# test-time-training/ttt-video-dit

Measured on AMD Instinct MI355X. Metric: DiT+TTT fwd/bwd video-tokens/sec, higher is better.
Workload: dtype bf16

## Files before the change

include/ttt_hip.h:

```cpp
#ifndef TTT_HIP_H
#define TTT_HIP_H

#include <stddef.h>
#include <stdint.h>

#ifdef __cplusplus
extern "C" {
#endif

#define TTT_HIP_ABI_VERSION 5

enum { TTT_DTYPE_BF16 = 0, TTT_DTYPE_F32 = 1 };
enum { TTT_IMPL_AUTO = 0, TTT_IMPL_GENERIC = 1, TTT_IMPL_MFMA = 2 };

typedef struct ttt_dims {
    int32_t B, NH, NC, CS, F, G;
    int32_t act_dtype;
    int32_t impl;
    float   eps;
} ttt_dims;

typedef struct ttt_mlp_fwd_args {
    const void*  XQ;
    const void*  XK;
    const void*  XV;
    const void*  last_eta;
    const float* ttt_norm_weight;
    const float* ttt_norm_bias;
    const float* W1_init;
    const float* b1_init;
    const float* W2_init;
    const float* b2_init;
    float* W1_checkpoints;
    float* b1_checkpoints;
    float* W2_checkpoints;
    float* b2_checkpoints;
    void*  XQW;
} ttt_mlp_fwd_args;

typedef struct ttt_mlp_bwd_args {
    const void*  XQ; const void* XK; const void* XV; const void* last_eta;
    const float* ttt_norm_weight; const float* ttt_norm_bias;
    const float* W1_checkpoints; const float* b1_checkpoints;
    const float* W2_checkpoints; const float* b2_checkpoints;
    const void*  XQW;
    float* W1_init_group; float* b1_init_group; float* W2_init_group; float* b2_init_group;
    void*  x_hat_ln_group;
    float* std_ln_group;
    void*  X2_group;
    void*  Z1_group;
    void*  Z1_bar_group;
    void*  X2_bar_group;
    void*  grad_l_wrt_Z2_group;
    void*  grad_l_wrt_Z1_group;
    void*  x_hat_fused_group;
    void*  grad_x_hat_fused_group;
    void*  grad_output_fused_group;
    float* std_fused_group;
    const float* grad_L_W1_last; const float* grad_L_b1_last;
    const float* grad_L_W2_last; const float* grad_L_b2_last;
    const void*  grad_L_XQW;
    float* grad_L_ttt_norm_weight;
    float* grad_L_ttt_norm_bias;
    float* grad_L_W1_init; float* grad_L_b1_init; float* grad_L_W2_init; float* grad_L_b2_init;
    void*  grad_L_last_eta;
    void*  grad_L_XQ; void* grad_L_XK; void* grad_L_XV;
} ttt_mlp_bwd_args;

typedef struct ttt_linear_fwd_args {
    const void*  XQ; const void* XK; const void* XV; const void* last_eta;
    const float* ttt_norm_weight; const float* ttt_norm_bias;
    const float* W1_init;
    const float* b1_init;
    float* W1_checkpoints;
    float* b1_checkpoints;
    void*  XQW;
} ttt_linear_fwd_args;

typedef struct ttt_linear_bwd_args {
    const void*  XQ; const void* XK; const void* XV; const void* last_eta;
    const float* ttt_norm_weight; const float* ttt_norm_bias;
    const float* W1_checkpoints; const float* b1_checkpoints;
    const float* grad_L_W1_last; const float* grad_L_b1_last;
    const void*  grad_L_XQW;
    float* W1_init_group;
    float* b1_init_group;
    float* grad_L_ttt_norm_weight; float* grad_L_ttt_norm_bias;
    float* grad_L_W1_init; float* grad_L_b1_init;
    void*  grad_L_last_eta;
    void*  grad_L_XQ; void* grad_L_XK; void* grad_L_XV;
} ttt_linear_bwd_args;

size_t ttt_hip_mlp_forward_workspace(const ttt_dims* d);
size_t ttt_hip_mlp_backward_workspace(const ttt_dims* d);
size_t ttt_hip_linear_forward_workspace(const ttt_dims* d);
size_t ttt_hip_linear_backward_workspace(const ttt_dims* d);

int ttt_hip_mlp_forward(const ttt_dims* d, const ttt_mlp_fwd_args* a, void* workspace, size_t workspace_bytes, void* stream);
int ttt_hip_mlp_backward(const ttt_dims* d, const ttt_mlp_bwd_args* a, void* workspace, size_t workspace_bytes, void* stream);
int ttt_hip_mlp_forward_chunk(const ttt_dims* d, const ttt_mlp_fwd_args* a, int step0, int nsteps, float* W1_final, float* b1_final,
                              float* W2_final, float* b2_final, void* workspace, size_t workspace_bytes, void* stream);
int ttt_hip_linear_forward(const ttt_dims* d, const ttt_linear_fwd_args* a, void* workspace, size_t workspace_bytes, void* stream);
int ttt_hip_linear_backward(const ttt_dims* d, const ttt_linear_bwd_args* a, void* workspace, size_t workspace_bytes, void* stream);

int ttt_hip_pre_forward(int B, int L, int NH, int F, const void* XQ_raw, const void* XK_raw, const void* XV_raw,
                        const float* rope , const int32_t* src, const int32_t* pos,
                        const float* ln_w, const float* ln_b , void* XQ, void* XK, void* XV, void* stream);
int ttt_hip_pre_forward_range(int B, int L, int NH, int F, const void* XQ_raw, const void* XK_raw, const void* XV_raw,
                              const float* rope, const int32_t* src, const int32_t* pos, const float* ln_w, const float* ln_b,
                              void* XQ, void* XK, void* XV, int t0, int tn, void* stream);
int ttt_hip_pre_backward_partials(int NH);
int ttt_hip_pre_backward(int B, int L, int NH, int F, const void* XQ_raw, const void* XK_raw, const void* XV_raw,
                         const float* rope, const int32_t* src, const int32_t* pos, const float* ln_w,
                         const void* dXQ, const void* dXK, const void* dXV, void* dXQ_raw, void* dXK_raw, void* dXV_raw,
                         float* dlnw_part, float* dlnb_part , void* stream);
int ttt_hip_pre_backward_ld(int B, int L, int NH, int F, const void* XQ_raw, const void* XK_raw, const void* XV_raw,
                            const float* rope, const int32_t* src, const int32_t* pos, const float* ln_w,
                            const void* dXQ, const void* dXK, const void* dXV, void* dXQ_raw, void* dXK_raw, void* dXV_raw, int64_t ld_out,
                            float* dlnw_part, float* dlnb_part, void* stream);
int ttt_hip_post_partials(int B, int L);
int ttt_hip_post_forward(int B, int L, int NH, int F, float eps, const void* Y, const int32_t* src, const float* w, const float* b,
                         void* out, void* stream);
int ttt_hip_post_forward_range(int B, int L, int NH, int F, float eps, const void* Y, const int32_t* src, const float* w, const float* b,
                               void* out, int t0, int tn, void* stream);
int ttt_hip_post_backward(int B, int L, int NH, int F, float eps, const void* Y, const void* dOut, const int32_t* src, const float* w,
                          void* dY, float* dw_part, float* db_part , void* stream);
int ttt_hip_gate_forward(int B, int L, int D, int n_text, const void* res, const void* y, const float* tanh_text,
                         const float* tanh_video, void* out, void* stream);
int ttt_hip_gate_backward_partials(int D);
int ttt_hip_gate_backward(int B, int L, int D, int n_text, const void* g, const void* y, const float* tanh_text,
                          const float* tanh_video, void* dy, float* dtanh_part , void* stream);

typedef struct ttt_attn_tensor {
    void*   ptr;
    int64_t stride_b, stride_h, stride_s;
} ttt_attn_tensor;
typedef struct ttt_attn_fwd_args {
    ttt_attn_tensor Q, K, V, O;
    float*  LSE;
    int32_t B, NH, S, D;
    float   scale;
} ttt_attn_fwd_args;
typedef struct ttt_attn_bwd_args {
    ttt_attn_tensor Q, K, V, O, dO;
    ttt_attn_tensor dQ, dK, dV;
    const float* LSE;
    float*  Delta;
    int32_t B, NH, S, D;
    float   scale;
} ttt_attn_bwd_args;
int ttt_hip_attn_forward(const ttt_attn_fwd_args* a, void* stream);
int ttt_hip_attn_backward(const ttt_attn_bwd_args* a, void* stream);

int ttt_hip_attn_pre_forward(int B, int S, int NH, int n_text, float eps, const void* q_raw, const void* k_raw,
                             const float* wq, const float* bq, const float* wk, const float* bk,
                             const float* cos_table, const float* sin_table, void* q, void* k, void* stream);
int ttt_hip_attn_pre_partials(int B, int S, int NH);
int ttt_hip_attn_pre_backward(int B, int S, int NH, int n_text, float eps, const void* q_raw, const void* k_raw,
                              const ttt_attn_tensor* dq, const ttt_attn_tensor* dk, const float* wq, const float* wk,
                              const float* cos_table, const float* sin_table, void* dq_raw, void* dk_raw, float* part,
                              void* stream);
int ttt_hip_attn_pre_backward_ld(int B, int S, int NH, int n_text, float eps, const void* q_raw, const void* k_raw,
                                 const ttt_attn_tensor* dq, const ttt_attn_tensor* dk, const float* wq, const float* wk,
                                 const float* cos_table, const float* sin_table, void* dq_raw, void* dk_raw, int64_t ld_out, float* part,
                                 void* stream);

int ttt_hip_adaln_forward(int B, int Lt, int Lv, int D, float eps, const void* vid, const void* text, const float* w, const float* b,
                          const float* shift, const float* scale1p, void* out, void* stream);
int ttt_hip_adaln_backward_partials(void);
int ttt_hip_adaln_backward(int B, int Lt, int Lv, int D, float eps, const void* vid, const void* text, const void* dout,
                           const float* w, const float* b, const float* scale1p, void* dvid, void* dtext, float* part, void* stream);
int ttt_hip_resgate_forward(int B, int Lt, int Lv, int D, const void* vid, const void* text, const void* y, const float* gate,
                            void* ovid, void* otext, void* stream);
int ttt_hip_resgate_backward_partials(int D);
int ttt_hip_resgate_backward(int B, int Lt, int Lv, int D, const void* dvid, const void* dtext, const void* y, const float* gate,
                             void* dy, float* dgate_part, void* stream);

int ttt_hip_resolve_impl(const ttt_dims* d, int is_mlp, int is_backward);

void        ttt_hip_debug_timing(void* device_buffer);
void        ttt_hip_debug_groups_per_chunk(int groups);
int         ttt_hip_debug_option(const char* name, int value);
unsigned    ttt_hip_debug_sweep_error(void);
void        ttt_hip_sweep_error_clear(void);
int         ttt_hip_debug_occupy_cus(int workgroups, int lds_bytes, int microseconds, void* stream);
void        ttt_hip_debug_dump(float* device_buffer);
int         ttt_hip_stream_create_masked(const unsigned* cu_mask, int mask_words, void** stream);
int         ttt_hip_stream_destroy(void* stream);
int         ttt_hip_debug_placement_probe(unsigned* device_out, int workgroups, int lds_bytes, int microseconds, void* stream);

int         ttt_hip_abi_version(void);
const char* ttt_hip_last_error(void);

#ifdef __cplusplus
}
#endif
#endif
```

ttt-video-dit_amd/csrc/attn.h:

```cpp
#pragma once
#include <hip/hip_runtime.h>
#include <stdint.h>
#include "attn_types.h"

namespace ttt {
namespace attn {

struct PreParams {
    const __bf16 *q_raw, *k_raw;
    const float *wq, *bq, *wk, *bk;
    const float *cos, *sin;
    __bf16 *q, *k;
    int B, S, NH, n_text;
    float eps;
};
struct PreBwdParams {
    const __bf16 *q_raw, *k_raw, *dq, *dk;
    long dq_sb, dq_sh, dq_ss, dk_sb, dk_sh, dk_ss;
    const float *wq, *wk, *cos, *sin;
    __bf16 *dq_raw, *dk_raw;
    long ld_out;
    float* part;
    int B, S, NH, n_text;
    float eps;
};
int  pre_blocks(long rows);
void launch_pre_forward(const PreParams& a, hipStream_t s);
void launch_pre_backward(const PreBwdParams& a, hipStream_t s);

void launch_forward(const FwdParams& p, hipStream_t s);
void launch_backward(const BwdParams& p, hipStream_t s);

void launch_dq_v2(const BwdParams& p, hipStream_t s);
void launch_dkdv_v2(const BwdParams& p, hipStream_t s);
void set_debug_attn_variant(int v);

}
}
```

ttt-video-dit_amd/csrc/attn_body.h:

```cpp
#pragma once
#include <math.h>

#include "attn_types.h"
#include "ttt_wave_types.h"

#ifndef TTT_BODY_FN
#if defined(__HIP_DEVICE_COMPILE__) || defined(__HIPCC__)
#define TTT_BODY_FN __device__ __forceinline__
#else
#define TTT_BODY_FN inline
#endif
#endif

namespace ttt {
namespace attnb {
using namespace ttt::wv;
using attn::BwdParams;
using attn::FwdParams;

constexpr int QB = 256, KB = 64;
constexpr int AS = 72;
constexpr int VS = 96;
constexpr int KT_ELEMS = 64 * AS, VT_ELEMS = 64 * VS;
constexpr int FWD_BUF_ELEMS = KT_ELEMS + VT_ELEMS, LDS_FWD = 2 * FWD_BUF_ELEMS * 2;
constexpr int DQ_BUF_ELEMS = 2 * KT_ELEMS, LDS_DQ = 2 * DQ_BUF_ELEMS * 2;
constexpr float LOG2E = 1.4426950408889634f;

#if defined(__HIP_DEVICE_COMPILE__)
#define TTT_PIN_IN_BRANCH(x) asm volatile("" : "+v"(x))
#else
#define TTT_PIN_IN_BRANCH(x) ((void)0)
#endif

TTT_BODY_FN int row_of(int r, int h) { return (r & 3) + 8 * (r >> 2) + 4 * h; }
TTT_BODY_FN f32x16 zero16() {
    f32x16 z;
#pragma unroll
    for (int i = 0; i < 16; ++i) z[i] = 0.f;
    return z;
}
TTT_BODY_FN bf16x8 pack(const f32x16& t, int s) {
    bf16x8 r;
#pragma unroll
    for (int e = 0; e < 8; ++e) r[e] = (__bf16)t[8 * s + e];
    return r;
}
TTT_BODY_FN bf16x8 zero_frag() {
    bf16x8 r;
#pragma unroll
    for (int e = 0; e < 8; ++e) r[e] = (__bf16)0.0f;
    return r;
}
template <class BK>
TTT_BODY_FN bf16x8 row_frag(BK& bk, typename BK::tile_t img, int stride, int row0, int col0, int l) {
    return bk.template ld<bf16x8>(img + ((row0 + (l & 31)) * stride + col0 + 8 * (l >> 5)));
}
template <class BK>
TTT_BODY_FN bf16x8 tr_frag(BK& bk, typename BK::tile_t img, int stride, int r0, int r1, int col0, int l) {
    const int i = l & 15, g1 = (l >> 4) & 1;
    const int off = (i >> 2) * stride + col0 + 16 * g1 + 4 * (i & 3);
    const bf16x4 lo = bk.tr(img + (r0 * stride + off));
    const bf16x4 hi = bk.tr(img + (r1 * stride + off));
    return __builtin_shufflevector(lo, hi, 0, 1, 2, 3, 4, 5, 6, 7);
}
template <class BK>
TTT_BODY_FN bf16x8 tr_frag_pi(BK& bk, typename BK::tile_t img, int stride, int row0, int s, int col0, int l) {
    const int h = l >> 5;
    return tr_frag(bk, img, stride, row0 + 16 * s + 4 * h, row0 + 16 * s + 8 + 4 * h, col0, l);
}

TTT_BODY_FN int swz_g(int r) { return (((r >> 1) & 1) << 2) | ((r >> 2) & 3); }
template <bool SWZ>
TTT_BODY_FN int tile_off(int r, int col) {
    return SWZ ? r * 64 + ((((col >> 3) ^ swz_g(r)) << 3) | (col & 7)) : r * AS + col;
}
template <bool SWZ, class BK>
TTT_BODY_FN bf16x8 row_frag_s(BK& bk, typename BK::tile_t img, int row0, int col0, int l) {
    return bk.template ld<bf16x8>(img + tile_off<SWZ>(row0 + (l & 31), col0 + 8 * (l >> 5)));
}
template <bool SWZ, class BK>
TTT_BODY_FN bf16x8 tr_frag_pi_s(BK& bk, typename BK::tile_t img, int row0, int s, int col0, int l) {
    const int h = l >> 5, i = l & 15, g1 = (l >> 4) & 1;
    const int r0 = row0 + 16 * s + 4 * h + (i >> 2), col = col0 + 16 * g1 + 4 * (i & 3);
    const bf16x4 lo = bk.tr(img + tile_off<SWZ>(r0, col));
    const bf16x4 hi = bk.tr(img + tile_off<SWZ>(r0 + 8, col));
    return __builtin_shufflevector(lo, hi, 0, 1, 2, 3, 4, 5, 6, 7);
}

struct KVStage {
    u32x4 k, v;
};
TTT_BODY_FN u32x4 zero_u4() {
    u32x4 z = {0u, 0u, 0u, 0u};
    return z;
}
TTT_BODY_FN void kv_issue(KVStage& st, const __bf16* Kp, const __bf16* Vp, long k_ss, long v_ss, int kv0, int S, int tid) {
    const int row = tid >> 3, col = (tid & 7) * 8;
    const int key = kv0 + row;
    if (key < S) {
        st.k = *reinterpret_cast<const u32x4*>(Kp + (long)key * k_ss + col);
        st.v = *reinterpret_cast<const u32x4*>(Vp + (long)key * v_ss + col);
    } else {
        st.k = zero_u4();
        st.v = zero_u4();
    }
}
template <class BK>
TTT_BODY_FN void kv_park(BK& bk, const KVStage& st, typename BK::tile_t k_img, typename BK::tile_t v_img, int v_stride, int tid) {
    const int row = tid >> 3, col = (tid & 7) * 8;
    bk.st(k_img + (row * AS + col), st.k);
    bk.st(v_img + (row * v_stride + col), st.v);
}

template <bool SWZ, class BK>
TTT_BODY_FN void kv_park_s(BK& bk, const KVStage& st, typename BK::tile_t k_img, typename BK::tile_t v_img, int tid) {
    const int row = tid >> 3, col = (tid & 7) * 8;
    bk.st(k_img + tile_off<SWZ>(row, col), st.k);
    bk.st(v_img + tile_off<SWZ>(row, col), st.v);
}

TTT_BODY_FN void head_of_block(int b, int nblk, int nbh, int& bh, int& blk) {
    if ((nbh & 7) == 0) {
        const int xcd = b & 7, idx = b >> 3;
        bh = xcd + 8 * (idx / nblk);
        blk = idx % nblk;
    } else {
        bh = b / nblk;
        blk = b % nblk;
    }
}

template <class BK>
TTT_BODY_FN void forward(BK& bk, const FwdParams& p, int bh, int qb) {
    const int tid = bk.thread(), wv = bk.wave(), l = bk.lane(), h = l >> 5, c = l & 31;
    const int bb = bh / p.NH, hh = bh % p.NH;
    const __bf16* Qp = p.Q + (long)bb * p.q_sb + (long)hh * p.q_sh;
    const __bf16* Kp = p.K + (long)bb * p.k_sb + (long)hh * p.k_sh;
    const __bf16* Vp = p.V + (long)bb * p.v_sb + (long)hh * p.v_sh;
    __bf16* Op = p.O + (long)bb * p.o_sb + (long)hh * p.o_sh;

    const int qrow = qb * QB + 32 * wv + c;
    const bool qvalid = qrow < p.S;
    bf16x8 Qf[4];
#pragma unroll
    for (int kk = 0; kk < 4; ++kk)
        Qf[kk] = qvalid ? *reinterpret_cast<const bf16x8*>(Qp + (long)qrow * p.q_ss + 16 * kk + 8 * h) : zero_frag();

    f32x16 O[2] = {zero16(), zero16()};
    float m = -1e30f, lsum = 0.f;
    const float sc = p.scale * LOG2E;
    const int nt = (p.S + KB - 1) / KB;
    KVStage st;

    const typename BK::tile_t lds = bk.lds_base();
    kv_issue(st, Kp, Vp, p.k_ss, p.v_ss, 0, p.S, tid);
    kv_park(bk, st, lds, lds + KT_ELEMS, VS, tid);
    bk.barrier();
    for (int j = 0; j < nt; ++j) {
        const typename BK::tile_t Kt = lds + (j & 1) * FWD_BUF_ELEMS, Vt = Kt + KT_ELEMS;
        const bool more = j + 1 < nt;
        if (more) kv_issue(st, Kp, Vp, p.k_ss, p.v_ss, (j + 1) * KB, p.S, tid);
        f32x16 Sc[2];
#pragma unroll
        for (int kb = 0; kb < 2; ++kb) {
            f32x16 acc = zero16();
#pragma unroll
            for (int kk = 0; kk < 4; ++kk) acc = bk.mma3216(row_frag(bk, Kt, AS, 32 * kb, 16 * kk, l), Qf[kk], acc);
            Sc[kb] = acc;
        }
        if (!more && (p.S & (KB - 1))) {
            const int kv0 = j * KB;
#pragma unroll
            for (int kb = 0; kb < 2; ++kb)
#pragma unroll
                for (int r = 0; r < 16; ++r) {
                    float v = Sc[kb][r];
                    if (kv0 + 32 * kb + row_of(r, h) >= p.S) v = -1e30f;
                    TTT_PIN_IN_BRANCH(v);
                    Sc[kb][r] = v;
                }
        }
        float mt = Sc[0][0];
#pragma unroll
        for (int r = 1; r < 16; ++r) mt = fmaxf(mt, Sc[0][r]);
#pragma unroll
        for (int r = 0; r < 16; ++r) mt = fmaxf(mt, Sc[1][r]);
        mt = fmaxf(mt, bk.xor_read(mt, 32));
        if (bk.any(mt > m)) {
            const float mn = fmaxf(m, mt);
            const float alpha = bk.exp2((m - mn) * sc);
            m = mn;
            lsum *= alpha;
#pragma unroll
            for (int db = 0; db < 2; ++db)
#pragma unroll
                for (int r = 0; r < 16; ++r) O[db][r] *= alpha;
        }
        const float msc = m * sc;
        float ps = 0.f;
#pragma unroll
        for (int kb = 0; kb < 2; ++kb)
#pragma unroll
            for (int r = 0; r < 16; ++r) {
                const float e = bk.exp2(__builtin_fmaf(Sc[kb][r], sc, -msc));
                Sc[kb][r] = e;
                ps += e;
            }
        lsum += ps;
#pragma unroll
        for (int kb = 0; kb < 2; ++kb)
#pragma unroll
            for (int s = 0; s < 2; ++s) {
                const bf16x8 pf = pack(Sc[kb], s);
                O[0] = bk.mma3216(tr_frag_pi(bk, Vt, VS, 32 * kb, s, 0, l), pf, O[0]);
                O[1] = bk.mma3216(tr_frag_pi(bk, Vt, VS, 32 * kb, s, 32, l), pf, O[1]);
            }
        if (more) {
            const typename BK::tile_t Kn = lds + ((j + 1) & 1) * FWD_BUF_ELEMS;
            kv_park(bk, st, Kn, Kn + KT_ELEMS, VS, tid);
        }
        bk.barrier();
    }

    const float ltot = lsum + bk.xor_read(lsum, 32);
    const float inv = 1.0f / ltot;
    if (qvalid) {
        __bf16* orow = Op + (long)qrow * p.o_ss;
#pragma unroll
        for (int db = 0; db < 2; ++db)
#pragma unroll
            for (int g = 0; g < 4; ++g) {
                bf16x4 v;
#pragma unroll
                for (int e = 0; e < 4; ++e) v[e] = (__bf16)(O[db][4 * g + e] * inv);
                *reinterpret_cast<bf16x4*>(orow + 32 * db + 8 * g + 4 * h) = v;
            }
        if (h == 0 && p.LSE) p.LSE[(long)bh * p.S + qrow] = m * p.scale + bk.log(ltot);
    }
}


template <class BK>
TTT_BODY_FN void dq(BK& bk, const BwdParams& p, int bh, int qb) {
    const int tid = bk.thread(), wv = bk.wave(), l = bk.lane(), h = l >> 5, c = l & 31;
    const int bb = bh / p.NH, hh = bh % p.NH;
    const __bf16* Qp = p.Q + (long)bb * p.q_sb + (long)hh * p.q_sh;
    const __bf16* Kp = p.K + (long)bb * p.k_sb + (long)hh * p.k_sh;
    const __bf16* Vp = p.V + (long)bb * p.v_sb + (long)hh * p.v_sh;
    const __bf16* dOp = p.dO + (long)bb * p.do_sb + (long)hh * p.do_sh;

    const int qrow = qb * QB + 32 * wv + c;
    const bool qvalid = qrow < p.S;
    bf16x8 Qf[4], Df[4];
#pragma unroll
    for (int kk = 0; kk < 4; ++kk) {
        Qf[kk] = qvalid ? *reinterpret_cast<const bf16x8*>(Qp + (long)qrow * p.q_ss + 16 * kk + 8 * h) : zero_frag();
        Df[kk] = qvalid ? *reinterpret_cast<const bf16x8*>(dOp + (long)qrow * p.do_ss + 16 * kk + 8 * h) : zero_frag();
    }
    const float lse2 = qvalid ? p.LSE[(long)bh * p.S + qrow] * LOG2E : 1e30f;
// ... 5 lines not shown

    const typename BK::tile_t lds = bk.lds_base();
    kv_issue(st, Kp, Vp, p.k_ss, p.v_ss, 0, p.S, tid);
    kv_park(bk, st, lds, lds + KT_ELEMS, AS, tid);
    bk.barrier();
    for (int j = 0; j < nt; ++j) {
        const typename BK::tile_t Kt = lds + (j & 1) * DQ_BUF_ELEMS, Vt = Kt + KT_ELEMS;
        const bool more = j + 1 < nt;
        if (more) kv_issue(st, Kp, Vp, p.k_ss, p.v_ss, (j + 1) * KB, p.S, tid);
        const bool ragged = !more && (p.S & (KB - 1));
#pragma unroll
        for (int kb = 0; kb < 2; ++kb) {
            f32x16 Sc = zero16(), dP = zero16();
#pragma unroll
            for (int kk = 0; kk < 4; ++kk) {
                Sc = bk.mma3216(row_frag(bk, Kt, AS, 32 * kb, 16 * kk, l), Qf[kk], Sc);
                dP = bk.mma3216(row_frag(bk, Vt, AS, 32 * kb, 16 * kk, l), Df[kk], dP);
            }
            if (ragged) {
#pragma unroll
                for (int r = 0; r < 16; ++r) {
                    float v = Sc[r];
                    if (j * KB + 32 * kb + row_of(r, h) >= p.S) v = -1e30f;
                    TTT_PIN_IN_BRANCH(v);
                    Sc[r] = v;
                }
            }
#pragma unroll
            for (int r = 0; r < 16; ++r) {
                const float pr = bk.exp2(__builtin_fmaf(Sc[r], sc, -lse2));
                dP[r] = pr * (dP[r] - delta);
            }
#pragma unroll
            for (int s = 0; s < 2; ++s) {
                const bf16x8 df = pack(dP, s);
                dQ[0] = bk.mma3216(tr_frag_pi(bk, Kt, AS, 32 * kb, s, 0, l), df, dQ[0]);
                dQ[1] = bk.mma3216(tr_frag_pi(bk, Kt, AS, 32 * kb, s, 32, l), df, dQ[1]);
            }
        }
        if (more) {
            const typename BK::tile_t Kn = lds + ((j + 1) & 1) * DQ_BUF_ELEMS;
            kv_park(bk, st, Kn, Kn + KT_ELEMS, AS, tid);
        }
        bk.barrier();
    }

    if (qvalid) {
        __bf16* row = p.dQ + (long)bb * p.dq_sb + (long)hh * p.dq_sh + (long)qrow * p.dq_ss;
#pragma unroll
        for (int db = 0; db < 2; ++db)
#pragma unroll
            for (int g = 0; g < 4; ++g) {
                bf16x4 v;
#pragma unroll
                for (int e = 0; e < 4; ++e) v[e] = (__bf16)(dQ[db][4 * g + e] * p.scale);
                *reinterpret_cast<bf16x4*>(row + 32 * db + 8 * g + 4 * h) = v;
            }
    }
}

template <int NSUB, bool SWZ = false, class BK>
TTT_BODY_FN void dq_staged(BK& bk, const BwdParams& p, int bh, int qb) {
    const int tid = bk.thread(), wv = bk.wave(), l = bk.lane(), h = l >> 5, c = l & 31;
    const int bb = bh / p.NH, hh = bh % p.NH;
    const __bf16* Qp = p.Q + (long)bb * p.q_sb + (long)hh * p.q_sh;
    const __bf16* Kp = p.K + (long)bb * p.k_sb + (long)hh * p.k_sh;
    const __bf16* Vp = p.V + (long)bb * p.v_sb + (long)hh * p.v_sh;
    const __bf16* dOp = p.dO + (long)bb * p.do_sb + (long)hh * p.do_sh;

    const int qrow = qb * QB + 32 * wv + c;
    const bool qvalid = qrow < p.S;
    bf16x8 Qf[4], Df[4];
#pragma unroll
    for (int kk = 0; kk < 4; ++kk) {
        Qf[kk] = qvalid ? *reinterpret_cast<const bf16x8*>(Qp + (long)qrow * p.q_ss + 16 * kk + 8 * h) : zero_frag();
        Df[kk] = qvalid ? *reinterpret_cast<const bf16x8*>(dOp + (long)qrow * p.do_ss + 16 * kk + 8 * h) : zero_frag();
    }
    const float lse2 = qvalid ? p.LSE[(long)bh * p.S + qrow] * LOG2E : 1e30f;
    const float delta = qvalid ? p.Delta[(long)bh * p.S + qrow] : 0.f;
    const float sc = p.scale * LOG2E;
    f32x16 dQ[2] = {zero16(), zero16()};
    const int nt = (p.S + KB - 1) / KB;
    const int ns = (nt + NSUB - 1) / NSUB;
    constexpr int STAGE_ELEMS = NSUB * DQ_BUF_ELEMS;
    KVStage st;

    const typename BK::tile_t lds = bk.lds_base();
#pragma unroll
    for (int u = 0; u < NSUB; ++u) {
        kv_issue(st, Kp, Vp, p.k_ss, p.v_ss, u * KB, p.S, tid);
        kv_park_s<SWZ>(bk, st, lds + u * DQ_BUF_ELEMS, lds + u * DQ_BUF_ELEMS + KT_ELEMS, tid);
    }
    bk.barrier();
    for (int j = 0; j < ns; ++j) {
        const typename BK::tile_t stage = lds + (j & 1) * STAGE_ELEMS;
        const typename BK::tile_t nxt = lds + ((j + 1) & 1) * STAGE_ELEMS;
        const bool more = j + 1 < ns;
#pragma unroll
        for (int u = 0; u < NSUB; ++u) {
            const int jt = j * NSUB + u;
            if (more) kv_issue(st, Kp, Vp, p.k_ss, p.v_ss, ((j + 1) * NSUB + u) * KB, p.S, tid);
            if (jt < nt) {
            const typename BK::tile_t Kt = stage + u * DQ_BUF_ELEMS, Vt = Kt + KT_ELEMS;
            const bool ragged = jt + 1 == nt && (p.S & (KB - 1));
#pragma unroll
            for (int kb = 0; kb < 2; ++kb) {
                f32x16 Sc = zero16(), dP = zero16();
#pragma unroll
                for (int kk = 0; kk < 4; ++kk) {
                    Sc = bk.mma3216(row_frag_s<SWZ>(bk, Kt, 32 * kb, 16 * kk, l), Qf[kk], Sc);
                    dP = bk.mma3216(row_frag_s<SWZ>(bk, Vt, 32 * kb, 16 * kk, l), Df[kk], dP);
                }
                if (ragged) {
#pragma unroll
                    for (int r = 0; r < 16; ++r) {
                        float v = Sc[r];
                        if (jt * KB + 32 * kb + row_of(r, h) >= p.S) v = -1e30f;
                        TTT_PIN_IN_BRANCH(v);
                        Sc[r] = v;
                    }
                }
#pragma unroll
                for (int r = 0; r < 16; ++r) {
                    const float pr = bk.exp2(__builtin_fmaf(Sc[r], sc, -lse2));
                    dP[r] = pr * (dP[r] - delta);
                }
#pragma unroll
                for (int s = 0; s < 2; ++s) {
                    const bf16x8 df = pack(dP, s);
                    dQ[0] = bk.mma3216(tr_frag_pi_s<SWZ>(bk, Kt, 32 * kb, s, 0, l), df, dQ[0]);
                    dQ[1] = bk.mma3216(tr_frag_pi_s<SWZ>(bk, Kt, 32 * kb, s, 32, l), df, dQ[1]);
                }
            }
            }
            if (more) kv_park_s<SWZ>(bk, st, nxt + u * DQ_BUF_ELEMS, nxt + u * DQ_BUF_ELEMS + KT_ELEMS, tid);
        }
        bk.barrier();
    }

    if (qvalid) {
        __bf16* row = p.dQ + (long)bb * p.dq_sb + (long)hh * p.dq_sh + (long)qrow * p.dq_ss;
#pragma unroll
        for (int db = 0; db < 2; ++db)
#pragma unroll
            for (int g = 0; g < 4; ++g) {
                bf16x4 v;
#pragma unroll
                for (int e = 0; e < 4; ++e) v[e] = (__bf16)(dQ[db][4 * g + e] * p.scale);
                *reinterpret_cast<bf16x4*>(row + 32 * db + 8 * g + 4 * h) = v;
            }
    }
}

template <int NSUB, int NQ, class BK>
TTT_BODY_FN void dq_wide(BK& bk, const BwdParams& p, int bh, int qb) {
    const int tid = bk.thread(), wv = bk.wave(), l = bk.lane(), h = l >> 5, c = l & 31;
    const int bb = bh / p.NH, hh = bh % p.NH;
    const __bf16* Qp = p.Q + (long)bb * p.q_sb + (long)hh * p.q_sh;
    const __bf16* Kp = p.K + (long)bb * p.k_sb + (long)hh * p.k_sh;
    const __bf16* Vp = p.V + (long)bb * p.v_sb + (long)hh * p.v_sh;
    const __bf16* dOp = p.dO + (long)bb * p.do_sb + (long)hh * p.do_sh;

    int qrow[NQ];
    bool qvalid[NQ];
    bf16x8 Qf[NQ][4], Df[NQ][4];
    float lse2[NQ], delta[NQ];
    f32x16 dQ[NQ][2];
#pragma unroll
    for (int qi = 0; qi < NQ; ++qi) {
        qrow[qi] = qb * (QB * NQ) + 32 * NQ * wv + 32 * qi + c;
        qvalid[qi] = qrow[qi] < p.S;
#pragma unroll
        for (int kk = 0; kk < 4; ++kk) {
            Qf[qi][kk] = qvalid[qi] ? *reinterpret_cast<const bf16x8*>(Qp + (long)qrow[qi] * p.q_ss + 16 * kk + 8 * h) : zero_frag();
            Df[qi][kk] = qvalid[qi] ? *reinterpret_cast<const bf16x8*>(dOp + (long)qrow[qi] * p.do_ss + 16 * kk + 8 * h) : zero_frag();
        }
        lse2[qi] = qvalid[qi] ? p.LSE[(long)bh * p.S + qrow[qi]] * LOG2E : 1e30f;
        delta[qi] = qvalid[qi] ? p.Delta[(long)bh * p.S + qrow[qi]] : 0.f;
        dQ[qi][0] = zero16();
        dQ[qi][1] = zero16();
    }
    const float sc = p.scale * LOG2E;
    const int nt = (p.S + KB - 1) / KB;
    const int ns = (nt + NSUB - 1) / NSUB;
    constexpr int STAGE_ELEMS = NSUB * DQ_BUF_ELEMS;
    KVStage st;

    const typename BK::tile_t lds = bk.lds_base();
#pragma unroll
    for (int u = 0; u < NSUB; ++u) {
        kv_issue(st, Kp, Vp, p.k_ss, p.v_ss, u * KB, p.S, tid);
        kv_park_s<false>(bk, st, lds + u * DQ_BUF_ELEMS, lds + u * DQ_BUF_ELEMS + KT_ELEMS, tid);
    }
    bk.barrier();
    for (int j = 0; j < ns; ++j) {
        const typename BK::tile_t stage = lds + (j & 1) * STAGE_ELEMS;
        const typename BK::tile_t nxt = lds + ((j + 1) & 1) * STAGE_ELEMS;
        const bool more = j + 1 < ns;
#pragma unroll
        for (int u = 0; u < NSUB; ++u) {
            const int jt = j * NSUB + u;
            if (more) kv_issue(st, Kp, Vp, p.k_ss, p.v_ss, ((j + 1) * NSUB + u) * KB, p.S, tid);
            if (jt < nt) {
            const typename BK::tile_t Kt = stage + u * DQ_BUF_ELEMS, Vt = Kt + KT_ELEMS;
            const bool ragged = jt + 1 == nt && (p.S & (KB - 1));
#pragma unroll
            for (int kb = 0; kb < 2; ++kb) {
                f32x16 Sc[NQ], dP[NQ];
#pragma unroll
                for (int qi = 0; qi < NQ; ++qi) { Sc[qi] = zero16(); dP[qi] = zero16(); }
#pragma unroll
                for (int kk = 0; kk < 4; ++kk) {
                    const bf16x8 kf = row_frag_s<false>(bk, Kt, 32 * kb, 16 * kk, l), vf = row_frag_s<false>(bk, Vt, 32 * kb, 16 * kk, l);
#pragma unroll
                    for (int qi = 0; qi < NQ; ++qi) {
                        Sc[qi] = bk.mma3216(kf, Qf[qi][kk], Sc[qi]);
                        dP[qi] = bk.mma3216(vf, Df[qi][kk], dP[qi]);
                    }
                }
                if (ragged) {
#pragma unroll
                    for (int qi = 0; qi < NQ; ++qi)
#pragma unroll
                        for (int r = 0; r < 16; ++r) {
                            float v = Sc[qi][r];
                            if (jt * KB + 32 * kb + row_of(r, h) >= p.S) v = -1e30f;
                            TTT_PIN_IN_BRANCH(v);
                            Sc[qi][r] = v;
                        }
                }
#pragma unroll
                for (int qi = 0; qi < NQ; ++qi)
#pragma unroll
                    for (int r = 0; r < 16; ++r) {
                        const float pr = bk.exp2(__builtin_fmaf(Sc[qi][r], sc, -lse2[qi]));
                        dP[qi][r] = pr * (dP[qi][r] - delta[qi]);
                    }
                if constexpr (BK::kPrio) bk.setprio(1);
#pragma unroll
                for (int s = 0; s < 2; ++s) {
                    const bf16x8 k0 = tr_frag_pi_s<false>(bk, Kt, 32 * kb, s, 0, l), k1 = tr_frag_pi_s<false>(bk, Kt, 32 * kb, s, 32, l);
#pragma unroll
                    for (int qi = 0; qi < NQ; ++qi) {
                        const bf16x8 df = pack(dP[qi], s);
                        dQ[qi][0] = bk.mma3216(k0, df, dQ[qi][0]);
                        dQ[qi][1] = bk.mma3216(k1, df, dQ[qi][1]);
                    }
                }
                if constexpr (BK::kPrio) bk.setprio(0);
            }
            }
            if (more) kv_park_s<false>(bk, st, nxt + u * DQ_BUF_ELEMS, nxt + u * DQ_BUF_ELEMS + KT_ELEMS, tid);
        }
        bk.barrier();
    }

#pragma unroll
    for (int qi = 0; qi < NQ; ++qi)
        if (qvalid[qi]) {
            __bf16* row = p.dQ + (long)bb * p.dq_sb + (long)hh * p.dq_sh + (long)qrow[qi] * p.dq_ss;
#pragma unroll
            for (int db = 0; db < 2; ++db)
#pragma unroll
                for (int g = 0; g < 4; ++g) {
                    bf16x4 v;
#pragma unroll
                    for (int e = 0; e < 4; ++e) v[e] = (__bf16)(dQ[qi][db][4 * g + e] * p.scale);
                    *reinterpret_cast<bf16x4*>(row + 32 * db + 8 * g + 4 * h) = v;
                }
        }
}

constexpr int DKV_BUF_ELEMS = 2 * KT_ELEMS + 2 * 64 * 2;
constexpr int LDS_DKV = 2 * DKV_BUF_ELEMS * 2;

struct QStage {
    u32x4 q, d;
    float lse, del;
};
template <bool ACC_INIT>
TTT_BODY_FN void qstage_issue(QStage& st, const BwdParams& p, const __bf16* Qp, const __bf16* dOp, const float* lse, const float* del,
                              float inv_scale, int q0, int tid) {
    if (tid < 512) {
        const int row = tid >> 3, col = (tid & 7) * 8;
        const int q = q0 + row;
        if (q < p.S) {
            st.q = *reinterpret_cast<const u32x4*>(Qp + (long)q * p.q_ss + col);
            st.d = *reinterpret_cast<const u32x4*>(dOp + (long)q * p.do_ss + col);
        } else {
            st.q = zero_u4();
            st.d = zero_u4();
        }
    }
    if (tid < 64) {
        const int qq = q0 + tid;
        if (ACC_INIT) {
            st.lse = qq < p.S ? -lse[qq] * inv_scale : -1e30f;
            st.del = qq < p.S ? -del[qq] : 0.f;
        } else {
            st.lse = qq < p.S ? lse[qq] * LOG2E : 1e30f;
            st.del = qq < p.S ? del[qq] : 0.f;
        }
    }
}
template <class BK>
TTT_BODY_FN void qstage_park(BK& bk, const QStage& st, typename BK::tile_t buf, int tid) {
    if (tid < 512) {
        const int row = tid >> 3, col = (tid & 7) * 8;
        bk.st(buf + (row * AS + col), st.q);
        bk.st(buf + (KT_ELEMS + row * AS + col), st.d);
    }
    if (tid < 64) {
        bk.st(buf + (2 * KT_ELEMS + 2 * tid), st.lse);
        bk.st(buf + (2 * KT_ELEMS + 2 * (64 + tid)), st.del);
    }
}
template <bool SWZ, class BK>
TTT_BODY_FN void qstage_park_s(BK& bk, const QStage& st, typename BK::tile_t buf, int tid) {
    if (tid < 512) {
        const int row = tid >> 3, col = (tid & 7) * 8;
        bk.st(buf + tile_off<SWZ>(row, col), st.q);
        bk.st(buf + (KT_ELEMS + tile_off<SWZ>(row, col)), st.d);
    }
    if (tid < 64) {
        bk.st(buf + (2 * KT_ELEMS + 2 * tid), st.lse);
        bk.st(buf + (2 * KT_ELEMS + 2 * (64 + tid)), st.del);
    }
}
template <class BK>
TTT_BODY_FN f32x16 rows_from_lds(BK& bk, typename BK::tile_t buf, int which, int base, int h) {
    f32x4 v[4];
#pragma unroll
    for (int q = 0; q < 4; ++q) v[q] = bk.template ld<f32x4>(buf + (2 * KT_ELEMS + 2 * (64 * which + base + 8 * q + 4 * h)));
    typedef float f32x8 __attribute__((ext_vector_type(8)));
    const f32x8 lo = __builtin_shufflevector(v[0], v[1], 0, 1, 2, 3, 4, 5, 6, 7);
    const f32x8 hi = __builtin_shufflevector(v[2], v[3], 0, 1, 2, 3, 4, 5, 6, 7);
    return __builtin_shufflevector(lo, hi, 0, 1, 2, 3, 4, 5, 6, 7, 8, 9, 10, 11, 12, 13, 14, 15);
}

template <int NW, bool ACC_INIT, class BK>
TTT_BODY_FN void dkdv(BK& bk, const BwdParams& p, int bh, int kvb) {
    const int tid = bk.thread(), wv = bk.wave(), l = bk.lane(), h = l >> 5, c = l & 31;
    const int bb = bh / p.NH, hh = bh % p.NH;
    const __bf16* Qp = p.Q + (long)bb * p.q_sb + (long)hh * p.q_sh;
    const __bf16* Kp = p.K + (long)bb * p.k_sb + (long)hh * p.k_sh;
    const __bf16* Vp = p.V + (long)bb * p.v_sb + (long)hh * p.v_sh;
    const __bf16* dOp = p.dO + (long)bb * p.do_sb + (long)hh * p.do_sh;
    const float* lse = p.LSE + (long)bh * p.S;
    const float* del = p.Delta + (long)bh * p.S;

    const int key0 = kvb * (32 * NW) + 32 * wv;
    const int krow = key0 + c;
    bf16x8 Kf[4], Vf[4];
#pragma unroll
    for (int kk = 0; kk < 4; ++kk) {
        Kf[kk] = krow < p.S ? *reinterpret_cast<const bf16x8*>(Kp + (long)krow * p.k_ss + 16 * kk + 8 * h) : zero_frag();
        Vf[kk] = krow < p.S ? *reinterpret_cast<const bf16x8*>(Vp + (long)krow * p.v_ss + 16 * kk + 8 * h) : zero_frag();
    }
    f32x16 dK[2] = {zero16(), zero16()}, dV[2] = {zero16(), zero16()};
    const float sc = p.scale * LOG2E, inv_scale = 1.0f / p.scale;

    const int nt = (p.S + 63) / 64;
    const typename BK::tile_t lds = bk.lds_base();
    QStage st;
    qstage_issue<ACC_INIT>(st, p, Qp, dOp, lse, del, inv_scale, 0, tid);
    qstage_park(bk, st, lds, tid);
    bk.barrier();

    for (int j = 0; j < nt; ++j) {
        const typename BK::tile_t buf = lds + (j & 1) * DKV_BUF_ELEMS;
        const typename BK::tile_t Qt = buf, Dt = buf + KT_ELEMS;
        const bool more = j + 1 < nt;
        if (more) qstage_issue<ACC_INIT>(st, p, Qp, dOp, lse, del, inv_scale, (j + 1) * 64, tid);
#pragma unroll
        for (int qb = 0; qb < 2; ++qb) {
            f32x16 Sc, dP;
            if (ACC_INIT) {
                Sc = rows_from_lds(bk, buf, 0, 32 * qb, h);
                dP = rows_from_lds(bk, buf, 1, 32 * qb, h);
            } else {
                Sc = zero16();
                dP = zero16();
            }
#pragma unroll
            for (int kk = 0; kk < 4; ++kk) {
                Sc = bk.mma3216(row_frag(bk, Qt, AS, 32 * qb, 16 * kk, l), Kf[kk], Sc);
                dP = bk.mma3216(row_frag(bk, Dt, AS, 32 * qb, 16 * kk, l), Vf[kk], dP);
            }
            if (ACC_INIT) {
#pragma unroll
                for (int r = 0; r < 16; ++r) {
                    float pr = bk.exp2(Sc[r] * sc);
                    TTT_PIN_IN_BRANCH(pr);
                    Sc[r] = pr;
                    float ds = pr * dP[r];
                    TTT_PIN_IN_BRANCH(ds);
                    dP[r] = ds;
                }
            } else {
                const f32x16 lseR = rows_from_lds(bk, buf, 0, 32 * qb, h);
                const f32x16 delR = rows_from_lds(bk, buf, 1, 32 * qb, h);
#pragma unroll
                for (int r = 0; r < 16; ++r) {
                    const float pr = bk.exp2(__builtin_fmaf(Sc[r], sc, -lseR[r]));
                    Sc[r] = pr;
                    dP[r] = pr * (dP[r] - delR[r]);
                }
            }
#pragma unroll
            for (int s = 0; s < 2; ++s) {
                const bf16x8 pf = pack(Sc, s), df = pack(dP, s);
#pragma unroll
                for (int db = 0; db < 2; ++db) {
                    dV[db] = bk.mma3216(pf, tr_frag_pi(bk, Dt, AS, 32 * qb, s, 32 * db, l), dV[db]);
                    dK[db] = bk.mma3216(df, tr_frag_pi(bk, Qt, AS, 32 * qb, s, 32 * db, l), dK[db]);
                }
            }
        }
        if (more) qstage_park(bk, st, lds + ((j + 1) & 1) * DKV_BUF_ELEMS, tid);
        bk.barrier();
    }

    __bf16* dKp = p.dK + (long)bb * p.dk_sb + (long)hh * p.dk_sh;
    __bf16* dVp = p.dV + (long)bb * p.dv_sb + (long)hh * p.dv_sh;
#pragma unroll
    for (int db = 0; db < 2; ++db)
#pragma unroll
        for (int r = 0; r < 16; ++r) {
            const int key = key0 + row_of(r, h);
            if (key < p.S) {
                dKp[(long)key * p.dk_ss + 32 * db + c] = (__bf16)(dK[db][r] * p.scale);
                dVp[(long)key * p.dv_ss + 32 * db + c] = (__bf16)dV[db][r];
            }
        }
}

template <int NW, bool ACC_INIT, int NSUB, bool SWZ = false, class BK>
TTT_BODY_FN void dkdv_staged(BK& bk, const BwdParams& p, int bh, int kvb) {
    const int tid = bk.thread(), wv = bk.wave(), l = bk.lane(), h = l >> 5, c = l & 31;
    const int bb = bh / p.NH, hh = bh % p.NH;
    const __bf16* Qp = p.Q + (long)bb * p.q_sb + (long)hh * p.q_sh;
    const __bf16* Kp = p.K + (long)bb * p.k_sb + (long)hh * p.k_sh;
    const __bf16* Vp = p.V + (long)bb * p.v_sb + (long)hh * p.v_sh;
    const __bf16* dOp = p.dO + (long)bb * p.do_sb + (long)hh * p.do_sh;
    const float* lse = p.LSE + (long)bh * p.S;
    const float* del = p.Delta + (long)bh * p.S;

    const int key0 = kvb * (32 * NW) + 32 * wv;
    const int krow = key0 + c;
    bf16x8 Kf[4], Vf[4];
#pragma unroll
    for (int kk = 0; kk < 4; ++kk) {
        Kf[kk] = krow < p.S ? *reinterpret_cast<const bf16x8*>(Kp + (long)krow * p.k_ss + 16 * kk + 8 * h) : zero_frag();
        Vf[kk] = krow < p.S ? *reinterpret_cast<const bf16x8*>(Vp + (long)krow * p.v_ss + 16 * kk + 8 * h) : zero_frag();
    }
    f32x16 dK[2] = {zero16(), zero16()}, dV[2] = {zero16(), zero16()};
    const float sc = p.scale * LOG2E, inv_scale = 1.0f / p.scale;

    const int nt = (p.S + 63) / 64;
    const int ns = (nt + NSUB - 1) / NSUB;
    constexpr int STAGE_ELEMS = NSUB * DKV_BUF_ELEMS;
    const typename BK::tile_t lds = bk.lds_base();
    QStage st;
#pragma unroll
    for (int u = 0; u < NSUB; ++u) {
        qstage_issue<ACC_INIT>(st, p, Qp, dOp, lse, del, inv_scale, u * 64, tid);
        qstage_park_s<SWZ>(bk, st, lds + u * DKV_BUF_ELEMS, tid);
    }
    bk.barrier();

    for (int j = 0; j < ns; ++j) {
        const typename BK::tile_t stage = lds + (j & 1) * STAGE_ELEMS;
        const typename BK::tile_t nxt = lds + ((j + 1) & 1) * STAGE_ELEMS;
        const bool more = j + 1 < ns;
#pragma unroll
        for (int u = 0; u < NSUB; ++u) {
        if (more) qstage_issue<ACC_INIT>(st, p, Qp, dOp, lse, del, inv_scale, ((j + 1) * NSUB + u) * 64, tid);
        if (j * NSUB + u < nt) {
        const typename BK::tile_t buf = stage + u * DKV_BUF_ELEMS;
        const typename BK::tile_t Qt = buf, Dt = buf + KT_ELEMS;
#pragma unroll
        for (int qb = 0; qb < 2; ++qb) {
            f32x16 Sc, dP;
            if (ACC_INIT) {
                Sc = rows_from_lds(bk, buf, 0, 32 * qb, h);
                dP = rows_from_lds(bk, buf, 1, 32 * qb, h);
            } else {
                Sc = zero16();
                dP = zero16();
            }
            if constexpr (BK::kPrio) bk.setprio(1);
#pragma unroll
            for (int kk = 0; kk < 4; ++kk) {
                Sc = bk.mma3216(row_frag_s<SWZ>(bk, Qt, 32 * qb, 16 * kk, l), Kf[kk], Sc);
                dP = bk.mma3216(row_frag_s<SWZ>(bk, Dt, 32 * qb, 16 * kk, l), Vf[kk], dP);
            }
            if constexpr (BK::kPrio) bk.setprio(0);
            if (ACC_INIT) {
#pragma unroll
                for (int r = 0; r < 16; ++r) {
                    float pr = bk.exp2(Sc[r] * sc);
                    TTT_PIN_IN_BRANCH(pr);
                    Sc[r] = pr;
                    float ds = pr * dP[r];
                    TTT_PIN_IN_BRANCH(ds);
                    dP[r] = ds;
                }
            } else {
                const f32x16 lseR = rows_from_lds(bk, buf, 0, 32 * qb, h);
                const f32x16 delR = rows_from_lds(bk, buf, 1, 32 * qb, h);
#pragma unroll
                for (int r = 0; r < 16; ++r) {
                    const float pr = bk.exp2(__builtin_fmaf(Sc[r], sc, -lseR[r]));
                    Sc[r] = pr;
                    dP[r] = pr * (dP[r] - delR[r]);
                }
            }
#pragma unroll
            for (int s = 0; s < 2; ++s) {
                const bf16x8 pf = pack(Sc, s), df = pack(dP, s);
#pragma unroll
                for (int db = 0; db < 2; ++db) {
                    dV[db] = bk.mma3216(pf, tr_frag_pi_s<SWZ>(bk, Dt, 32 * qb, s, 32 * db, l), dV[db]);
                    dK[db] = bk.mma3216(df, tr_frag_pi_s<SWZ>(bk, Qt, 32 * qb, s, 32 * db, l), dK[db]);
                }
            }

        }
        }
        if (more) qstage_park_s<SWZ>(bk, st, nxt + u * DKV_BUF_ELEMS, tid);
        }
        bk.barrier();
    }

    __bf16* dKp = p.dK + (long)bb * p.dk_sb + (long)hh * p.dk_sh;
    __bf16* dVp = p.dV + (long)bb * p.dv_sb + (long)hh * p.dv_sh;
#pragma unroll
    for (int db = 0; db < 2; ++db)
#pragma unroll
        for (int r = 0; r < 16; ++r) {
            const int key = key0 + row_of(r, h);
            if (key < p.S) {
                dKp[(long)key * p.dk_ss + 32 * db + c] = (__bf16)(dK[db][r] * p.scale);
                dVp[(long)key * p.dv_ss + 32 * db + c] = (__bf16)dV[db][r];
            }
        }
}

}
}
```

ttt-video-dit_amd/csrc/attn_bwd.hip:

```cpp
#include <hip/hip_runtime.h>
#include <stdlib.h>
#include "../../include/ttt_hip.h"
#include "attn.h"
#include "attn_dev.h"

namespace ttt {
namespace attn {

__global__ __launch_bounds__(256) void attn_delta_kernel(BwdParams p) {
    const long rows = (long)p.B * p.NH * p.S;
    for (long idx = (long)blockIdx.x * blockDim.x + threadIdx.x; idx < rows * 8; idx += (long)gridDim.x * blockDim.x) {
        const long row = idx >> 3;
        const int o = idx & 7;
        const int s = row % p.S;
        const int bh = row / p.S;
        const int b = bh / p.NH, h = bh % p.NH;
        const bf16x8 a = *reinterpret_cast<const bf16x8*>(p.dO + (long)b * p.do_sb + (long)h * p.do_sh + (long)s * p.do_ss + 8 * o);
        const bf16x8 c = *reinterpret_cast<const bf16x8*>(p.O + (long)b * p.o_sb + (long)h * p.o_sh + (long)s * p.o_ss + 8 * o);
        float acc = 0.f;
#pragma unroll
        for (int e = 0; e < 8; ++e) acc += (float)a[e] * (float)c[e];
        acc += __shfl_xor(acc, 1, 64);
        acc += __shfl_xor(acc, 2, 64);
        acc += __shfl_xor(acc, 4, 64);
        if (o == 0) p.Delta[row] = acc;
    }
}

void launch_backward(const BwdParams& p, hipStream_t s) {
    const long rows = (long)p.B * p.NH * p.S;
    const int dgrid = (int)((rows * 8 + 255) / 256 < 65536 ? (rows * 8 + 255) / 256 : 65536);
    hipLaunchKernelGGL(attn_delta_kernel, dim3(dgrid), dim3(256), 0, s, p);
    launch_dkdv_v2(p, s);
    launch_dq_v2(p, s);
}

}
}
```

ttt-video-dit_amd/csrc/attn_fwd.hip:

```cpp
#include <hip/hip_runtime.h>
#include "../../include/ttt_hip.h"
#include "attn.h"
#include "attn_dev.h"
#include "once_per_device.h"

namespace ttt {
namespace attn {

constexpr int QB = 256;
constexpr int KB = 64;
constexpr int NTF = 512;
constexpr int VS = 96;
constexpr int KT_ELEMS = ATILE, VT_ELEMS = 64 * VS, BUF_ELEMS = KT_ELEMS + VT_ELEMS;
constexpr int LDS_FWD = 2 * BUF_ELEMS * 2;

struct KVStage {
    uint4 k, v;
};

__device__ __forceinline__ void stage_issue(KVStage& st, const __bf16* Kp, const __bf16* Vp, long k_ss, long v_ss, int kv0, int S, int tid) {
    const int row = tid >> 3, col = (tid & 7) * 8;
    const int key = kv0 + row;
    if (key < S) {
        st.k = *reinterpret_cast<const uint4*>(Kp + (long)key * k_ss + col);
        st.v = *reinterpret_cast<const uint4*>(Vp + (long)key * v_ss + col);
    } else {
        st.k = make_uint4(0, 0, 0, 0);
        st.v = make_uint4(0, 0, 0, 0);
    }
}
__device__ __forceinline__ void stage_park(const KVStage& st, __bf16* Kt, __bf16* Vt, int tid) {
    const int row = tid >> 3, col = (tid & 7) * 8;
    *reinterpret_cast<uint4*>(Kt + row * AS + col) = st.k;
    *reinterpret_cast<uint4*>(Vt + row * VS + col) = st.v;
}

__global__ __launch_bounds__(NTF) void attn_fwd_kernel(FwdParams p) {
    extern __shared__ __attribute__((aligned(16))) char smem[];
    __bf16* lds = reinterpret_cast<__bf16*>(smem);

    const int tid = threadIdx.x;
    const int wv = __builtin_amdgcn_readfirstlane(tid >> 6);
    const int l = tid & 63, h = l >> 5, c = l & 31;

    const int nqb = (p.S + QB - 1) / QB;
    int bh, qb;
    {
        const int nbh = p.B * p.NH;
        const int b = blockIdx.x;
        if ((nbh & 7) == 0) {
            const int xcd = b & 7, idx = b >> 3;
            bh = xcd + 8 * (idx / nqb);
            qb = idx % nqb;
        } else {
            bh = b / nqb;
            qb = b % nqb;
        }
    }
    const int bb = bh / p.NH, hh = bh % p.NH;
    const __bf16* Qp = p.Q + (long)bb * p.q_sb + (long)hh * p.q_sh;
    const __bf16* Kp = p.K + (long)bb * p.k_sb + (long)hh * p.k_sh;
    const __bf16* Vp = p.V + (long)bb * p.v_sb + (long)hh * p.v_sh;
    __bf16* Op = p.O + (long)bb * p.o_sb + (long)hh * p.o_sh;

    const int q0 = qb * QB + 32 * wv;
    const int qrow = q0 + c;
    const bool qvalid = qrow < p.S;

    bf16x8 Qf[4];
#pragma unroll
    for (int kk = 0; kk < 4; ++kk) {
        if (qvalid) Qf[kk] = *reinterpret_cast<const bf16x8*>(Qp + (long)qrow * p.q_ss + 16 * kk + 8 * h);
        else {
#pragma unroll
            for (int e = 0; e < 8; ++e) Qf[kk][e] = (__bf16)0.0f;
        }
    }

    f32x16 O[2] = {zero16(), zero16()};
    float m = -1e30f, lsum = 0.f;
    const float sc = p.scale * 1.4426950408889634f;

    const int nt = (p.S + KB - 1) / KB;
    KVStage st;
    stage_issue(st, Kp, Vp, p.k_ss, p.v_ss, 0, p.S, tid);
    stage_park(st, lds, lds + KT_ELEMS, tid);
    __syncthreads();

    for (int j = 0; j < nt; ++j) {
        const __bf16* Kt = lds + (j & 1) * BUF_ELEMS;
        const __bf16* Vt = Kt + KT_ELEMS;
        const bool more = j + 1 < nt;
        if (more) stage_issue(st, Kp, Vp, p.k_ss, p.v_ss, (j + 1) * KB, p.S, tid);

        f32x16 Sc[2];
#pragma unroll
        for (int kb = 0; kb < 2; ++kb) {
            f32x16 acc = zero16();
#pragma unroll
            for (int kk = 0; kk < 4; ++kk) acc = mma(row_frag(Kt, AS, 32 * kb, 16 * kk, l), Qf[kk], acc);
            Sc[kb] = acc;
        }
        if (!more && (p.S & (KB - 1))) {
            const int kv0 = j * KB;
#pragma unroll
            for (int kb = 0; kb < 2; ++kb)
#pragma unroll
                for (int r = 0; r < 16; ++r)
                    if (kv0 + 32 * kb + row_of(r, h) >= p.S) Sc[kb][r] = -1e30f;
        }
        float mt = Sc[0][0];
#pragma unroll
        for (int r = 1; r < 16; ++r) mt = fmaxf(mt, Sc[0][r]);
#pragma unroll
        for (int r = 0; r < 16; ++r) mt = fmaxf(mt, Sc[1][r]);
        mt = fmaxf(mt, half_swap(mt));
        if (__builtin_amdgcn_ballot_w64(mt > m) != 0) {
            const float mn = fmaxf(m, mt);
            const float alpha = __builtin_amdgcn_exp2f((m - mn) * sc);
            m = mn;
            lsum *= alpha;
#pragma unroll
            for (int db = 0; db < 2; ++db)
#pragma unroll
                for (int r = 0; r < 16; ++r) O[db][r] *= alpha;
        }
        const float msc = m * sc;
        float ps = 0.f;
#pragma unroll
        for (int kb = 0; kb < 2; ++kb)
#pragma unroll
            for (int r = 0; r < 16; ++r) {
                const float e = __builtin_amdgcn_exp2f(__builtin_fmaf(Sc[kb][r], sc, -msc));
                Sc[kb][r] = e;
                ps += e;
            }
        lsum += ps;
#pragma unroll
        for (int kb = 0; kb < 2; ++kb)
#pragma unroll
            for (int s = 0; s < 2; ++s) {
                const bf16x8 pf = pack(Sc[kb], s);
                O[0] = mma(tr_frag_pi(Vt, VS, 32 * kb, s, 0, l), pf, O[0]);
                O[1] = mma(tr_frag_pi(Vt, VS, 32 * kb, s, 32, l), pf, O[1]);
            }
        if (more) {
            __bf16* Kn = lds + ((j + 1) & 1) * BUF_ELEMS;
            stage_park(st, Kn, Kn + KT_ELEMS, tid);
        }
        __syncthreads();
    }

    const float ltot = lsum + half_swap(lsum);
    const float inv = 1.0f / ltot;
    if (qvalid) {
        __bf16* orow = Op + (long)qrow * p.o_ss;
#pragma unroll
        for (int db = 0; db < 2; ++db)
#pragma unroll
            for (int g = 0; g < 4; ++g) {
                bf16x4 v;
#pragma unroll
                for (int e = 0; e < 4; ++e) v[e] = (__bf16)(O[db][4 * g + e] * inv);
                *reinterpret_cast<bf16x4*>(orow + 32 * db + 8 * g + 4 * h) = v;
            }
        if (h == 0 && p.LSE) p.LSE[(long)bh * p.S + qrow] = m * p.scale + __logf(ltot);
    }
}

void launch_forward(const FwdParams& p, hipStream_t s) {
    static ttt::OncePerDevice attr;
    attr.run([&] {
        (void)hipFuncSetAttribute((const void*)attn_fwd_kernel, hipFuncAttributeMaxDynamicSharedMemorySize, LDS_FWD);
    });
    const int nqb = (p.S + QB - 1) / QB;
    hipLaunchKernelGGL(attn_fwd_kernel, dim3(p.B * p.NH * nqb), dim3(NTF), LDS_FWD, s, p);
}

}
}
```

ttt-video-dit_amd/csrc/attn_pre.hip:

```cpp
#include <hip/hip_runtime.h>
#include <stdint.h>
#include "../../include/ttt_hip.h"
#include "attn.h"
#include "ttt_dpp.h"

namespace ttt {
namespace attn {

typedef __bf16 bf16x8 __attribute__((ext_vector_type(8)));
typedef float f32x4 __attribute__((ext_vector_type(4)));

__device__ __forceinline__ void ld8(const __bf16* p, float (&o)[8]) {
    const bf16x8 a = *reinterpret_cast<const bf16x8*>(p);
#pragma unroll
    for (int j = 0; j < 8; ++j) o[j] = (float)a[j];
}
__device__ __forceinline__ void st8(__bf16* p, const float (&v)[8]) {
    bf16x8 a;
#pragma unroll
    for (int j = 0; j < 8; ++j) a[j] = (__bf16)v[j];
    *reinterpret_cast<bf16x8*>(p) = a;
}
__device__ __forceinline__ void ldf8(const float* p, float (&o)[8]) {
    const f32x4 a = *reinterpret_cast<const f32x4*>(p), b = *reinterpret_cast<const f32x4*>(p + 4);
    o[0] = a[0]; o[1] = a[1]; o[2] = a[2]; o[3] = a[3]; o[4] = b[0]; o[5] = b[1]; o[6] = b[2]; o[7] = b[3];
}
__device__ __forceinline__ float rb(float x) { return (float)(__bf16)x; }

__device__ __forceinline__ void ln_rope(const float (&x)[8], const float (&w)[8], const float (&b)[8], float eps,
                                        const float* cosr, const float* sinr, float (&out)[8], float (&xh)[8], float& rstd) {
    float s = 0.f;
#pragma unroll
    for (int j = 0; j < 8; ++j) s += x[j];
    const float mean = sum8(s) * (1.0f / 64.0f);
    float vs = 0.f;
#pragma unroll
    for (int j = 0; j < 8; ++j) { xh[j] = x[j] - mean; vs += xh[j] * xh[j]; }
    rstd = 1.0f / sqrtf(sum8(vs) * (1.0f / 64.0f) + eps);
#pragma unroll
    for (int j = 0; j < 8; ++j) { xh[j] *= rstd; out[j] = rb(xh[j] * w[j] + b[j]); }
    if (cosr) {
        float c8[8], s8[8];
        ldf8(cosr, c8);
        ldf8(sinr, s8);
#pragma unroll
        for (int q = 0; q < 4; ++q) {
            const float a = out[2 * q], bb = out[2 * q + 1];
            out[2 * q] = rb(rb(a * rb(c8[2 * q])) + rb(-bb * rb(s8[2 * q])));
            out[2 * q + 1] = rb(rb(bb * rb(c8[2 * q + 1])) + rb(a * rb(s8[2 * q + 1])));
        }
    }
}

__global__ __launch_bounds__(256) void attn_pre_fwd_kernel(PreParams a) {
    const long total = (long)a.B * a.S * a.NH * 8;
    const int o = threadIdx.x & 7;
    float wq[8], bq[8], wk[8], bk[8];
    ldf8(a.wq + 8 * o, wq); ldf8(a.bq + 8 * o, bq); ldf8(a.wk + 8 * o, wk); ldf8(a.bk + 8 * o, bk);
    for (long idx = (long)blockIdx.x * blockDim.x + threadIdx.x; idx < total; idx += (long)gridDim.x * blockDim.x) {
        const int s = ((idx >> 3) / a.NH) % a.S;
        const int pos = s - a.n_text;
        const float* cosr = pos >= 0 ? a.cos + (long)pos * 64 + 8 * o : nullptr;
        const float* sinr = pos >= 0 ? a.sin + (long)pos * 64 + 8 * o : nullptr;
        float x[8], y[8], xh[8], rstd;
        ld8(a.q_raw + idx * 8, x);
        ln_rope(x, wq, bq, a.eps, cosr, sinr, y, xh, rstd);
        st8(a.q + idx * 8, y);
        ld8(a.k_raw + idx * 8, x);
        ln_rope(x, wk, bk, a.eps, cosr, sinr, y, xh, rstd);
        st8(a.k + idx * 8, y);
    }
}

__device__ __forceinline__ void ln_rope_bwd(const float (&x)[8], const float (&w)[8], float eps, const float* cosr, const float* sinr,
                                            float (&g)[8], float (&dx)[8], float (&dw)[8], float (&db)[8]) {
    if (cosr) {
        float c8[8], s8[8];
        ldf8(cosr, c8);
        ldf8(sinr, s8);
#pragma unroll
        for (int q = 0; q < 4; ++q) {
            const float ga = g[2 * q], gb = g[2 * q + 1];
            g[2 * q] = ga * rb(c8[2 * q]) + gb * rb(s8[2 * q + 1]);
            g[2 * q + 1] = gb * rb(c8[2 * q + 1]) - ga * rb(s8[2 * q]);
        }
    }
    float s = 0.f;
#pragma unroll
    for (int j = 0; j < 8; ++j) s += x[j];
    const float mean = sum8(s) * (1.0f / 64.0f);
    float vs = 0.f, xh[8];
#pragma unroll
    for (int j = 0; j < 8; ++j) { xh[j] = x[j] - mean; vs += xh[j] * xh[j]; }
    const float rstd = 1.0f / sqrtf(sum8(vs) * (1.0f / 64.0f) + eps);
    float s1 = 0.f, s2 = 0.f;
#pragma unroll
    for (int j = 0; j < 8; ++j) {
        xh[j] *= rstd;
        dw[j] += g[j] * xh[j];
        db[j] += g[j];
        g[j] *= w[j];
        s1 += g[j];
        s2 += g[j] * xh[j];
    }
    s1 = sum8(s1) * (1.0f / 64.0f);
    s2 = sum8(s2) * (1.0f / 64.0f);
#pragma unroll
    for (int j = 0; j < 8; ++j) dx[j] = (g[j] - s1 - xh[j] * s2) * rstd;
}

__global__ __launch_bounds__(256) void attn_pre_bwd_kernel(PreBwdParams a) {
    __shared__ float red[4][256][8 + 1];
    const long total = (long)a.B * a.S * a.NH * 8;
    const int o = threadIdx.x & 7;
    float wq[8], wk[8], dwq[8], dbq[8], dwk[8], dbk[8];
    ldf8(a.wq + 8 * o, wq); ldf8(a.wk + 8 * o, wk);
#pragma unroll
    for (int j = 0; j < 8; ++j) { dwq[j] = 0.f; dbq[j] = 0.f; dwk[j] = 0.f; dbk[j] = 0.f; }
    for (long idx = (long)blockIdx.x * blockDim.x + threadIdx.x; idx < total; idx += (long)gridDim.x * blockDim.x) {
        const long row = idx >> 3;
        const int hd = row % a.NH;
        const long tok = row / a.NH;
        const int s = tok % a.S;
        const int b = tok / a.S;
        const int pos = s - a.n_text;
        const float* cosr = pos >= 0 ? a.cos + (long)pos * 64 + 8 * o : nullptr;
        const float* sinr = pos >= 0 ? a.sin + (long)pos * 64 + 8 * o : nullptr;
        float x[8], g[8], dx[8];
        ld8(a.q_raw + idx * 8, x);
        ld8(a.dq + (long)b * a.dq_sb + (long)hd * a.dq_sh + (long)s * a.dq_ss + 8 * o, g);
        ln_rope_bwd(x, wq, a.eps, cosr, sinr, g, dx, dwq, dbq);
        const long raw_off = tok * a.ld_out + hd * 64 + 8 * o;
        st8(a.dq_raw + raw_off, dx);
        ld8(a.k_raw + idx * 8, x);
        ld8(a.dk + (long)b * a.dk_sb + (long)hd * a.dk_sh + (long)s * a.dk_ss + 8 * o, g);
        ln_rope_bwd(x, wk, a.eps, cosr, sinr, g, dx, dwk, dbk);
        st8(a.dk_raw + raw_off, dx);
    }
#pragma unroll
    for (int j = 0; j < 8; ++j) {
        red[0][threadIdx.x][j] = dwq[j]; red[1][threadIdx.x][j] = dbq[j];
        red[2][threadIdx.x][j] = dwk[j]; red[3][threadIdx.x][j] = dbk[j];
    }
    __syncthreads();
    {
        const int which = threadIdx.x >> 6, f = threadIdx.x & 63;
        const int oo = f >> 3, j = f & 7;
        float acc = 0.f;
        for (int t = oo; t < 256; t += 8) acc += red[which][t][j];
        a.part[((long)blockIdx.x * 4 + which) * 64 + f] = acc;
    }
}

int pre_blocks(long rows) {
    const long g = (rows * 8 + 255) / 256;
    return (int)(g < 2048 ? g : 2048);
}
void launch_pre_forward(const PreParams& a, hipStream_t s) {
    const long g = ((long)a.B * a.S * a.NH * 8 + 255) / 256;
    hipLaunchKernelGGL(attn_pre_fwd_kernel, dim3((int)(g < 8192 ? g : 8192)), dim3(256), 0, s, a);
}
void launch_pre_backward(const PreBwdParams& a, hipStream_t s) {
    hipLaunchKernelGGL(attn_pre_bwd_kernel, dim3(pre_blocks((long)a.B * a.S * a.NH)), dim3(256), 0, s, a);
}

}
}
```

ttt-video-dit_amd/csrc/attn_types.h:

```cpp
#pragma once
#include <stdint.h>

namespace ttt {
namespace attn {

struct FwdParams {
    const __bf16 *Q, *K, *V;
    __bf16* O;
    float* LSE;
    long q_sb, q_sh, q_ss, k_sb, k_sh, k_ss, v_sb, v_sh, v_ss, o_sb, o_sh, o_ss;
    int B, NH, S;
    float scale;
};
struct BwdParams {
    const __bf16 *Q, *K, *V, *O, *dO;
    const float* LSE;
    float* Delta;
    __bf16 *dQ, *dK, *dV;
    long q_sb, q_sh, q_ss, k_sb, k_sh, k_ss, v_sb, v_sh, v_ss, o_sb, o_sh, o_ss, do_sb, do_sh, do_ss;
    long dq_sb, dq_sh, dq_ss, dk_sb, dk_sh, dk_ss, dv_sb, dv_sh, dv_ss;
    int B, NH, S;
    float scale;
};

}
}
```

ttt-video-dit_amd/csrc/attn_v2.hip:

```cpp
#include <hip/hip_runtime.h>
#include <stdlib.h>
#include "../../include/ttt_hip.h"
#include "attn.h"
#include "attn_body.h"
#include "once_per_device.h"

namespace ttt {
namespace attn {

template <int VAR>
struct AttnDeviceWave {
    static constexpr bool kPrio = VAR != 0;
    __device__ __forceinline__ void setprio(int v) const { if (v) __builtin_amdgcn_s_setprio(1); else __builtin_amdgcn_s_setprio(0); }
    typedef __bf16* tile_t;
    typedef __attribute__((address_space(3))) wv::bf16x4 lds_b4;
    tile_t base;
    __device__ __forceinline__ int lane() const { return threadIdx.x & 63; }
    __device__ __forceinline__ int wave() const { return __builtin_amdgcn_readfirstlane(threadIdx.x >> 6); }
    __device__ __forceinline__ int thread() const { return threadIdx.x; }
    __device__ __forceinline__ void barrier() const { __syncthreads(); }
    __device__ __forceinline__ float exp2(float x) const { return __builtin_amdgcn_exp2f(x); }
    __device__ __forceinline__ float log(float x) const { return __logf(x); }
    __device__ __forceinline__ tile_t lds_base() const { return base; }
    template <class T> __device__ __forceinline__ T ld(const __bf16* p) const { return *reinterpret_cast<const T*>(p); }
    template <class T> __device__ __forceinline__ void st(__bf16* p, T v) const { *reinterpret_cast<T*>(p) = v; }
    __device__ __forceinline__ wv::bf16x4 tr(const __bf16* p) const { return __builtin_amdgcn_ds_read_tr16_b64_v4bf16((lds_b4*)p); }
    __device__ __forceinline__ wv::f32x16 mma3216(wv::bf16x8 a, wv::bf16x8 b, wv::f32x16 c) const {
        return __builtin_amdgcn_mfma_f32_32x32x16_bf16(a, b, c, 0, 0, 0);
    }
    __device__ __forceinline__ float xor_read(float v, int mask) const { return __shfl_xor(v, mask, 64); }
    __device__ __forceinline__ bool any(bool b) const { return __builtin_amdgcn_ballot_w64(b) != 0; }
};

template <int NW, bool ACC_INIT, int MINW, int NSUB, int VAR>
__global__ __launch_bounds__(64 * NW, MINW) void attn_dkdv2s_kernel(BwdParams p) {
    extern __shared__ __attribute__((aligned(16))) char smem[];
    int bh, kvb;
    attnb::head_of_block(blockIdx.x, (p.S + 32 * NW - 1) / (32 * NW), p.B * p.NH, bh, kvb);
    AttnDeviceWave<VAR> bk{reinterpret_cast<__bf16*>(smem)};
    attnb::dkdv_staged<NW, ACC_INIT, NSUB, false>(bk, p, bh, kvb);
}
template <int NSUB, int VAR>
__global__ __launch_bounds__(512, 2) void attn_dq_wide_kernel(BwdParams p) {
    extern __shared__ __attribute__((aligned(16))) char smem[];
    int bh, qb;
    attnb::head_of_block(blockIdx.x, (p.S + 2 * attnb::QB - 1) / (2 * attnb::QB), p.B * p.NH, bh, qb);
    AttnDeviceWave<VAR> bk{reinterpret_cast<__bf16*>(smem)};
    attnb::dq_wide<NSUB, 2>(bk, p, bh, qb);
}

static int g_attn_variant = 1;
void set_debug_attn_variant(int v) { g_attn_variant = v; }

template <int VAR>
static void launch_dq_var(const BwdParams& p, hipStream_t s) {
    constexpr int NSUB = 1;
    static ttt::OncePerDevice attr;
    attr.run([&] {
        (void)hipFuncSetAttribute((const void*)attn_dq_wide_kernel<NSUB, VAR>, hipFuncAttributeMaxDynamicSharedMemorySize, NSUB * attnb::LDS_DQ);
    });
    const int nb = (p.S + 2 * attnb::QB - 1) / (2 * attnb::QB);
    hipLaunchKernelGGL((attn_dq_wide_kernel<NSUB, VAR>), dim3(p.B * p.NH * nb), dim3(512), NSUB * attnb::LDS_DQ, s, p);
}
void launch_dq_v2(const BwdParams& p, hipStream_t s) {
    if (g_attn_variant) launch_dq_var<1>(p, s);
    else launch_dq_var<0>(p, s);
}

template <int VAR>
static void launch_dkdv_var(const BwdParams& p, hipStream_t s) {
    constexpr int NW = 12, NSUB = 2;
    static_assert(NSUB * attnb::LDS_DKV <= 160 * 1024, "LDS budget");
    static ttt::OncePerDevice attr;
    attr.run([&] {
        (void)hipFuncSetAttribute((const void*)attn_dkdv2s_kernel<NW, true, 3, NSUB, VAR>, hipFuncAttributeMaxDynamicSharedMemorySize, NSUB * attnb::LDS_DKV);
    });
    const int nb = (p.S + 32 * NW - 1) / (32 * NW);
    hipLaunchKernelGGL((attn_dkdv2s_kernel<NW, true, 3, NSUB, VAR>), dim3(p.B * p.NH * nb), dim3(64 * NW), NSUB * attnb::LDS_DKV, s, p);
}
void launch_dkdv_v2(const BwdParams& p, hipStream_t s) {
    if (g_attn_variant) launch_dkdv_var<1>(p, s);
    else launch_dkdv_var<0>(p, s);
}

}
}
```

ttt-video-dit_amd/csrc/capi.hip:

```cpp
#include <hip/hip_runtime.h>
#include <stdio.h>
#include <string.h>
#include "../../include/ttt_hip.h"
#include "ttt_generic.h"
#include "ttt_mfma.h"
#include "ttt_prepost.h"
#include "attn.h"
#include "ttt_mfma_int.h"

static thread_local char g_err[512] = "";

static int fail(const char* fmt, const char* what = "") {
    snprintf(g_err, sizeof(g_err), fmt, what);
    return -1;
}

static int check_dims(const ttt_dims* d) {
    if (!d) return fail("ttt_hip: null dims");
    if (d->B <= 0 || d->NH <= 0 || d->NC <= 0 || d->CS <= 0 || d->F <= 0 || d->G <= 0)
        return fail("ttt_hip: non-positive dimension");
    if (d->act_dtype != TTT_DTYPE_BF16 && d->act_dtype != TTT_DTYPE_F32) return fail("ttt_hip: bad act_dtype");
    if (d->impl < TTT_IMPL_AUTO || d->impl > TTT_IMPL_MFMA) return fail("ttt_hip: bad impl");
    if (!(d->eps >= 0.f)) return fail("ttt_hip: bad eps");
    return 0;
// ... 194 lines not shown
    if (wsb < ws_bytes(d, false, true) || (ws_bytes(d, false, true) && !ws)) return fail("ttt_hip: linear_backward: workspace too small");
    if (r == TTT_IMPL_MFMA) ttt::mfma::linear_backward(d, a, ws, (hipStream_t)stream);
    else ttt::generic::linear_backward(d, a, ws, (hipStream_t)stream);
    return post_launch("linear_backward");
}

static int check_pp(int B, int L, int NH, int F) {
    if (B <= 0 || L <= 0 || NH <= 0) return fail("ttt_hip: non-positive dimension");
    if (F != 64) return fail("ttt_hip: fused pre/post kernels need head_dim 64");
    if (NH * 8 > 512) return fail("ttt_hip: too many heads for the post kernels (NH * 64 <= 4096 features)");
    if ((long long)B * L >= (1ll << 31) / 4) return fail("ttt_hip: B * L too large for the pre / post kernels' 32-bit token arithmetic");
    return 0;
}

int ttt_hip_pre_forward(int B, int L, int NH, int F, const void* XQ_raw, const void* XK_raw, const void* XV_raw,
                        const float* rope, const int32_t* src, const int32_t* pos, const float* ln_w, const float* ln_b,
                        void* XQ, void* XK, void* XV, void* stream) {
    return ttt_hip_pre_forward_range(B, L, NH, F, XQ_raw, XK_raw, XV_raw, rope, src, pos, ln_w, ln_b, XQ, XK, XV, 0, L, stream);
}
int ttt_hip_pre_forward_range(int B, int L, int NH, int F, const void* XQ_raw, const void* XK_raw, const void* XV_raw,
                              const float* rope, const int32_t* src, const int32_t* pos, const float* ln_w, const float* ln_b,
                              void* XQ, void* XK, void* XV, int t0, int tn, void* stream) {
    if (check_pp(B, L, NH, F)) return -1;
    if (!XQ_raw || !XK_raw || !XV_raw || !ln_w || !ln_b || !XQ || !XK || !XV) return fail("ttt_hip: pre_forward: null pointer");
    if (pos && !rope) return fail("ttt_hip: pre_forward: positions without a rotation table");
    if (t0 < 0 || tn <= 0 || t0 + tn > L) return fail("ttt_hip: pre_forward: the range of scan positions must lie inside the sequence");
    ttt::prepost::PreArgs a = {(const __bf16*)XQ_raw, (const __bf16*)XK_raw, (const __bf16*)XV_raw, rope, src, pos, ln_w, ln_b,
                               (__bf16*)XQ, (__bf16*)XK, (__bf16*)XV, B, L, NH, t0, tn};
    ttt::prepost::pre_forward(a, (hipStream_t)stream);
    return post_launch("pre_forward");
}
int ttt_hip_pre_backward_partials(int NH) { return ttt::prepost::pre_backward_partials(NH); }
int ttt_hip_pre_backward(int B, int L, int NH, int F, const void* XQ_raw, const void* XK_raw, const void* XV_raw,
                         const float* rope, const int32_t* src, const int32_t* pos, const float* ln_w,
                         const void* dXQ, const void* dXK, const void* dXV, void* dXQ_raw, void* dXK_raw, void* dXV_raw,
                         float* dlnw_part, float* dlnb_part, void* stream) {
    return ttt_hip_pre_backward_ld(B, L, NH, F, XQ_raw, XK_raw, XV_raw, rope, src, pos, ln_w, dXQ, dXK, dXV, dXQ_raw, dXK_raw, dXV_raw,
                                   (int64_t)NH * F, dlnw_part, dlnb_part, stream);
}
int ttt_hip_pre_backward_ld(int B, int L, int NH, int F, const void* XQ_raw, const void* XK_raw, const void* XV_raw,
                            const float* rope, const int32_t* src, const int32_t* pos, const float* ln_w,
                            const void* dXQ, const void* dXK, const void* dXV, void* dXQ_raw, void* dXK_raw, void* dXV_raw, int64_t ld_out,
                            float* dlnw_part, float* dlnb_part, void* stream) {
    if (check_pp(B, L, NH, F)) return -1;
    if (ld_out < (int64_t)NH * F || (ld_out & 7) || ((uintptr_t)dXQ_raw & 15) || ((uintptr_t)dXK_raw & 15) || ((uintptr_t)dXV_raw & 15))
        return fail("ttt_hip: pre_backward: the raw gradients' row stride must be >= NH*F and a multiple of 8 elements, their bases 16-byte aligned");
    if (!XQ_raw || !XK_raw || !XV_raw || !ln_w || !dXQ || !dXK || !dXV || !dXQ_raw || !dXK_raw || !dXV_raw || !dlnw_part || !dlnb_part)
        return fail("ttt_hip: pre_backward: null pointer");
    ttt::prepost::PreBwdArgs a = {(const __bf16*)XQ_raw, (const __bf16*)XK_raw, (const __bf16*)XV_raw, rope, src, pos, ln_w,
                                  (const __bf16*)dXQ, (const __bf16*)dXK, (const __bf16*)dXV,
                                  (__bf16*)dXQ_raw, (__bf16*)dXK_raw, (__bf16*)dXV_raw, dlnw_part, dlnb_part, B, L, NH, (long)ld_out};
    ttt::prepost::pre_backward(a, (hipStream_t)stream);
    return post_launch("pre_backward");
}
int ttt_hip_post_partials(int B, int L) { return ttt::prepost::post_blocks(B, L); }
int ttt_hip_post_forward(int B, int L, int NH, int F, float eps, const void* Y, const int32_t* src, const float* w, const float* b,
                         void* out, void* stream) {
    return ttt_hip_post_forward_range(B, L, NH, F, eps, Y, src, w, b, out, 0, L, stream);
}
int ttt_hip_post_forward_range(int B, int L, int NH, int F, float eps, const void* Y, const int32_t* src, const float* w, const float* b,
                               void* out, int t0, int tn, void* stream) {
    if (check_pp(B, L, NH, F)) return -1;
    if (!Y || !w || !b || !out) return fail("ttt_hip: post_forward: null pointer");
    if (t0 < 0 || tn <= 0 || t0 + tn > L) return fail("ttt_hip: post_forward: the range of scan positions must lie inside the sequence");
    ttt::prepost::PostArgs a = {(const __bf16*)Y, src, w, b, (__bf16*)out, B, L, NH, eps, t0, tn};
    ttt::prepost::post_forward(a, (hipStream_t)stream);
    return post_launch("post_forward");
}
int ttt_hip_post_backward(int B, int L, int NH, int F, float eps, const void* Y, const void* dOut, const int32_t* src, const float* w,
                          void* dY, float* dw_part, float* db_part, void* stream) {
    if (check_pp(B, L, NH, F)) return -1;
    if (!Y || !dOut || !w || !dY || !dw_part || !db_part) return fail("ttt_hip: post_backward: null pointer");
    ttt::prepost::PostBwdArgs a = {(const __bf16*)Y, (const __bf16*)dOut, src, w, (__bf16*)dY, dw_part, db_part, B, L, NH, eps};
    ttt::prepost::post_backward(a, (hipStream_t)stream);
    return post_launch("post_backward");
}
int ttt_hip_gate_forward(int B, int L, int D, int n_text, const void* res, const void* y, const float* tanh_text,
                         const float* tanh_video, void* out, void* stream) {
    if (B <= 0 || L <= 0 || D <= 0 || D % 8) return fail("ttt_hip: gate_forward: bad dimensions");
    if (!res || !y || !tanh_text || !tanh_video || !out) return fail("ttt_hip: gate_forward: null pointer");
    ttt::prepost::GateArgs a = {(const __bf16*)res, (const __bf16*)y, tanh_text, tanh_video, (__bf16*)out, B, L, D, n_text};
    ttt::prepost::gate_forward(a, (hipStream_t)stream);
    return post_launch("gate_forward");
}
int ttt_hip_gate_backward_partials(int D) { return ttt::prepost::gate_backward_partials(D); }
int ttt_hip_gate_backward(int B, int L, int D, int n_text, const void* g, const void* y, const float* tanh_text,
                          const float* tanh_video, void* dy, float* dtanh_part, void* stream) {
    if (B <= 0 || L <= 0 || D <= 0 || D % 8) return fail("ttt_hip: gate_backward: bad dimensions");
    if (!g || !y || !tanh_text || !tanh_video || !dy || !dtanh_part) return fail("ttt_hip: gate_backward: null pointer");
    ttt::prepost::GateBwdArgs a = {(const __bf16*)g, (const __bf16*)y, tanh_text, tanh_video, (__bf16*)dy, dtanh_part, B, L, D, n_text};
    ttt::prepost::gate_backward(a, (hipStream_t)stream);
    return post_launch("gate_backward");
}


static int check_attn_tensor(const ttt_attn_tensor& t, const char* name) {
    if (!t.ptr) return fail("ttt_hip: attention: null tensor %s", name);
    if (((uintptr_t)t.ptr & 15) || (t.stride_b & 7) || (t.stride_h & 7) || (t.stride_s & 7))
        return fail("ttt_hip: attention: tensor %s must be 16-byte aligned with strides that are multiples of 8 elements", name);
    return 0;
}

int ttt_hip_attn_forward(const ttt_attn_fwd_args* a, void* stream) {
    if (!a) return fail("ttt_hip: null args");
    if (a->D != 64) return fail("ttt_hip: attention: head_dim must be 64");
    if (a->B <= 0 || a->NH <= 0 || a->S <= 0) return fail("ttt_hip: attention: non-positive dimension");
    if (check_attn_tensor(a->Q, "Q") || check_attn_tensor(a->K, "K") || check_attn_tensor(a->V, "V") || check_attn_tensor(a->O, "O")) return -1;
    ttt::attn::FwdParams p = {};
    p.Q = (const __bf16*)a->Q.ptr; p.K = (const __bf16*)a->K.ptr; p.V = (const __bf16*)a->V.ptr; p.O = (__bf16*)a->O.ptr;
    p.LSE = a->LSE;
    p.q_sb = a->Q.stride_b; p.q_sh = a->Q.stride_h; p.q_ss = a->Q.stride_s;
    p.k_sb = a->K.stride_b; p.k_sh = a->K.stride_h; p.k_ss = a->K.stride_s;
    p.v_sb = a->V.stride_b; p.v_sh = a->V.stride_h; p.v_ss = a->V.stride_s;
    p.o_sb = a->O.stride_b; p.o_sh = a->O.stride_h; p.o_ss = a->O.stride_s;
    p.B = a->B; p.NH = a->NH; p.S = a->S; p.scale = a->scale;
    ttt::attn::launch_forward(p, (hipStream_t)stream);
    return post_launch("attn_forward");
}

int ttt_hip_attn_backward(const ttt_attn_bwd_args* a, void* stream) {
    if (!a) return fail("ttt_hip: null args");
    if (a->D != 64) return fail("ttt_hip: attention: head_dim must be 64");
    if (a->B <= 0 || a->NH <= 0 || a->S <= 0) return fail("ttt_hip: attention: non-positive dimension");
    if (!a->LSE || !a->Delta) return fail("ttt_hip: attention backward: null LSE / Delta");
    if (check_attn_tensor(a->Q, "Q") || check_attn_tensor(a->K, "K") || check_attn_tensor(a->V, "V") || check_attn_tensor(a->O, "O") ||
        check_attn_tensor(a->dO, "dO") || check_attn_tensor(a->dQ, "dQ") || check_attn_tensor(a->dK, "dK") || check_attn_tensor(a->dV, "dV")) return -1;
    ttt::attn::BwdParams p = {};
    p.Q = (const __bf16*)a->Q.ptr; p.K = (const __bf16*)a->K.ptr; p.V = (const __bf16*)a->V.ptr; p.O = (const __bf16*)a->O.ptr;
    p.dO = (const __bf16*)a->dO.ptr; p.dQ = (__bf16*)a->dQ.ptr; p.dK = (__bf16*)a->dK.ptr; p.dV = (__bf16*)a->dV.ptr;
    p.LSE = a->LSE; p.Delta = a->Delta;
    p.q_sb = a->Q.stride_b; p.q_sh = a->Q.stride_h; p.q_ss = a->Q.stride_s;
    p.k_sb = a->K.stride_b; p.k_sh = a->K.stride_h; p.k_ss = a->K.stride_s;
    p.v_sb = a->V.stride_b; p.v_sh = a->V.stride_h; p.v_ss = a->V.stride_s;
    p.o_sb = a->O.stride_b; p.o_sh = a->O.stride_h; p.o_ss = a->O.stride_s;
    p.do_sb = a->dO.stride_b; p.do_sh = a->dO.stride_h; p.do_ss = a->dO.stride_s;
    p.dq_sb = a->dQ.stride_b; p.dq_sh = a->dQ.stride_h; p.dq_ss = a->dQ.stride_s;
    p.dk_sb = a->dK.stride_b; p.dk_sh = a->dK.stride_h; p.dk_ss = a->dK.stride_s;
    p.dv_sb = a->dV.stride_b; p.dv_sh = a->dV.stride_h; p.dv_ss = a->dV.stride_s;
    p.B = a->B; p.NH = a->NH; p.S = a->S; p.scale = a->scale;
    ttt::attn::launch_backward(p, (hipStream_t)stream);
    return post_launch("attn_backward");
}


int ttt_hip_attn_pre_partials(int B, int S, int NH) { return ttt::attn::pre_blocks((long)B * S * NH); }

int ttt_hip_attn_pre_forward(int B, int S, int NH, int n_text, float eps, const void* q_raw, const void* k_raw,
                             const float* wq, const float* bq, const float* wk, const float* bk,
                             const float* cos_table, const float* sin_table, void* q, void* k, void* stream) {
    if (B <= 0 || S <= 0 || NH <= 0 || n_text < 0) return fail("ttt_hip: attn_pre: bad dimension");
    if (!q_raw || !k_raw || !wq || !bq || !wk || !bk || !q || !k) return fail("ttt_hip: attn_pre_forward: null pointer");
    if (n_text < S && (!cos_table || !sin_table)) return fail("ttt_hip: attn_pre_forward: null rope table");
    ttt::attn::PreParams p = {(const __bf16*)q_raw, (const __bf16*)k_raw, wq, bq, wk, bk, cos_table, sin_table,
                              (__bf16*)q, (__bf16*)k, B, S, NH, n_text, eps};
    ttt::attn::launch_pre_forward(p, (hipStream_t)stream);
    return post_launch("attn_pre_forward");
}

int ttt_hip_attn_pre_backward(int B, int S, int NH, int n_text, float eps, const void* q_raw, const void* k_raw,
                              const ttt_attn_tensor* dq, const ttt_attn_tensor* dk, const float* wq, const float* wk,
                              const float* cos_table, const float* sin_table, void* dq_raw, void* dk_raw, float* part,
                              void* stream) {
    return ttt_hip_attn_pre_backward_ld(B, S, NH, n_text, eps, q_raw, k_raw, dq, dk, wq, wk, cos_table, sin_table, dq_raw, dk_raw,
                                        (int64_t)NH * 64, part, stream);
}
int ttt_hip_attn_pre_backward_ld(int B, int S, int NH, int n_text, float eps, const void* q_raw, const void* k_raw,
                                 const ttt_attn_tensor* dq, const ttt_attn_tensor* dk, const float* wq, const float* wk,
                                 const float* cos_table, const float* sin_table, void* dq_raw, void* dk_raw, int64_t ld_out, float* part,
                                 void* stream) {
    if (ld_out < (int64_t)NH * 64 || (ld_out & 7) || ((uintptr_t)dq_raw & 15) || ((uintptr_t)dk_raw & 15))
        return fail("ttt_hip: attn_pre_backward: the raw gradients' row stride must be >= NH*64 and a multiple of 8 elements, their bases 16-byte aligned");
    if (B <= 0 || S <= 0 || NH <= 0 || n_text < 0) return fail("ttt_hip: attn_pre: bad dimension");
    if (!q_raw || !k_raw || !dq || !dk || !wq || !wk || !dq_raw || !dk_raw || !part) return fail("ttt_hip: attn_pre_backward: null pointer");
    if (n_text < S && (!cos_table || !sin_table)) return fail("ttt_hip: attn_pre_backward: null rope table");
    if (check_attn_tensor(*dq, "dq") || check_attn_tensor(*dk, "dk")) return -1;
    ttt::attn::PreBwdParams p = {};
    p.q_raw = (const __bf16*)q_raw; p.k_raw = (const __bf16*)k_raw; p.dq = (const __bf16*)dq->ptr; p.dk = (const __bf16*)dk->ptr;
    p.dq_sb = dq->stride_b; p.dq_sh = dq->stride_h; p.dq_ss = dq->stride_s;
    p.dk_sb = dk->stride_b; p.dk_sh = dk->stride_h; p.dk_ss = dk->stride_s;
    p.wq = wq; p.wk = wk; p.cos = cos_table; p.sin = sin_table;
    p.dq_raw = (__bf16*)dq_raw; p.dk_raw = (__bf16*)dk_raw; p.part = part; p.ld_out = (long)ld_out;
    p.B = B; p.S = S; p.NH = NH; p.n_text = n_text; p.eps = eps;
    ttt::attn::launch_pre_backward(p, (hipStream_t)stream);
    return post_launch("attn_pre_backward");
}


static int check_glue_dims(int B, int Lt, int Lv, int D) {
    if (B <= 0 || Lt < 0 || Lv < 0 || Lt + Lv <= 0 || D <= 0 || (D & 7)) return fail("ttt_hip: glue kernels: bad dimension (D must be a multiple of 8)");
    if (D > 8 * 512) return fail("ttt_hip: glue kernels: D too large for one block per token (D / 8 <= 512 threads)");
    return 0;
}
int ttt_hip_adaln_backward_partials(void) { return ttt::prepost::adaln_backward_partials(); }
int ttt_hip_adaln_forward(int B, int Lt, int Lv, int D, float eps, const void* vid, const void* text, const float* w, const float* b,
                          const float* shift, const float* scale1p, void* out, void* stream) {
    if (check_glue_dims(B, Lt, Lv, D)) return -1;
    if ((Lv && !vid) || (Lt && !text) || !w || !b || !shift || !scale1p || !out) return fail("ttt_hip: adaln_forward: null pointer");
    ttt::prepost::AdaLNArgs a = {(const __bf16*)vid, (const __bf16*)text, w, b, shift, scale1p, (__bf16*)out, B, Lt, Lv, D, eps};
    ttt::prepost::adaln_forward(a, (hipStream_t)stream);
    return post_launch("adaln_forward");
}
int ttt_hip_adaln_backward(int B, int Lt, int Lv, int D, float eps, const void* vid, const void* text, const void* dout,
                           const float* w, const float* b, const float* scale1p, void* dvid, void* dtext, float* part, void* stream) {
    if (check_glue_dims(B, Lt, Lv, D)) return -1;
    if ((Lv && (!vid || !dvid)) || (Lt && (!text || !dtext)) || !dout || !w || !b || !scale1p || !part) return fail("ttt_hip: adaln_backward: null pointer");
    ttt::prepost::AdaLNBwdArgs a = {(const __bf16*)vid, (const __bf16*)text, (const __bf16*)dout, w, b, scale1p,
                                    (__bf16*)dvid, (__bf16*)dtext, part, B, Lt, Lv, D, 0, eps};
    ttt::prepost::adaln_backward(a, (hipStream_t)stream);
    return post_launch("adaln_backward");
}
int ttt_hip_resgate_backward_partials(int D) { return ttt::prepost::resgate_backward_partials(D); }
int ttt_hip_resgate_forward(int B, int Lt, int Lv, int D, const void* vid, const void* text, const void* y, const float* gate,
                            void* ovid, void* otext, void* stream) {
    if (check_glue_dims(B, Lt, Lv, D)) return -1;
    if ((Lv && (!vid || !ovid)) || (Lt && (!text || !otext)) || !y || !gate) return fail("ttt_hip: resgate_forward: null pointer");
    ttt::prepost::ResGateArgs a = {(const __bf16*)vid, (const __bf16*)text, (const __bf16*)y, gate, (__bf16*)ovid, (__bf16*)otext, B, Lt, Lv, D};
    ttt::prepost::resgate_forward(a, (hipStream_t)stream);
    return post_launch("resgate_forward");
}
int ttt_hip_resgate_backward(int B, int Lt, int Lv, int D, const void* dvid, const void* dtext, const void* y, const float* gate,
                             void* dy, float* dgate_part, void* stream) {
    if (check_glue_dims(B, Lt, Lv, D)) return -1;
    if ((Lv && !dvid) || (Lt && !dtext) || !y || !gate || !dy || !dgate_part) return fail("ttt_hip: resgate_backward: null pointer");
    ttt::prepost::ResGateBwdArgs a = {(const __bf16*)dvid, (const __bf16*)dtext, (const __bf16*)y, gate, (__bf16*)dy, dgate_part, B, Lt, Lv, D};
    ttt::prepost::resgate_backward(a, (hipStream_t)stream);
    return post_launch("resgate_backward");
}

}
```

ttt-video-dit_amd/test_time_training/__init__.py:

```python
from __future__ import annotations

import ctypes
import os
from typing import Optional

import torch

_HERE = os.path.dirname(os.path.abspath(__file__))
_LIB_PATH = os.path.join(os.path.dirname(_HERE), "lib", "libttt_hip.so")

IMPL_AUTO, IMPL_GENERIC, IMPL_MFMA = 0, 1, 2
_IMPL_NAMES = {"auto": IMPL_AUTO, "generic": IMPL_GENERIC, "mfma": IMPL_MFMA}

_state = {"impl": IMPL_AUTO, "eps": 1e-8}


class _Dims(ctypes.Structure):
    _fields_ = [(n, ctypes.c_int32) for n in ("B", "NH", "NC", "CS", "F", "G", "act_dtype", "impl")] + [("eps", ctypes.c_float)]


def _ptr_struct(name, fields):
    return type(name, (ctypes.Structure,), {"_fields_": [(f, ctypes.c_void_p) for f in fields]})


MLP_FWD_FIELDS = ("XQ", "XK", "XV", "last_eta", "ttt_norm_weight", "ttt_norm_bias", "W1_init", "b1_init", "W2_init",
                  "b2_init", "W1_checkpoints", "b1_checkpoints", "W2_checkpoints", "b2_checkpoints", "XQW")
MLP_BWD_FIELDS = ("XQ", "XK", "XV", "last_eta", "ttt_norm_weight", "ttt_norm_bias", "W1_checkpoints", "b1_checkpoints",
                  "W2_checkpoints", "b2_checkpoints", "XQW", "W1_init_group", "b1_init_group", "W2_init_group",
                  "b2_init_group", "x_hat_ln_group", "std_ln_group", "X2_group", "Z1_group", "Z1_bar_group", "X2_bar_group",
                  "grad_l_wrt_Z2_group", "grad_l_wrt_Z1_group", "x_hat_fused_group", "grad_x_hat_fused_group",
                  "grad_output_fused_group", "std_fused_group", "grad_L_W1_last", "grad_L_b1_last", "grad_L_W2_last",
                  "grad_L_b2_last", "grad_L_XQW", "grad_L_ttt_norm_weight", "grad_L_ttt_norm_bias", "grad_L_W1_init",
                  "grad_L_b1_init", "grad_L_W2_init", "grad_L_b2_init", "grad_L_last_eta", "grad_L_XQ", "grad_L_XK", "grad_L_XV")
LIN_FWD_FIELDS = ("XQ", "XK", "XV", "last_eta", "ttt_norm_weight", "ttt_norm_bias", "W1_init", "b1_init",
                  "W1_checkpoints", "b1_checkpoints", "XQW")
LIN_BWD_FIELDS = ("XQ", "XK", "XV", "last_eta", "ttt_norm_weight", "ttt_norm_bias", "W1_checkpoints", "b1_checkpoints",
                  "grad_L_W1_last", "grad_L_b1_last", "grad_L_XQW", "W1_init_group", "b1_init_group",
                  "grad_L_ttt_norm_weight", "grad_L_ttt_norm_bias", "grad_L_W1_init", "grad_L_b1_init", "grad_L_last_eta",
                  "grad_L_XQ", "grad_L_XK", "grad_L_XV")

_MlpFwd = _ptr_struct("_MlpFwd", MLP_FWD_FIELDS)
_MlpBwd = _ptr_struct("_MlpBwd", MLP_BWD_FIELDS)
_LinFwd = _ptr_struct("_LinFwd", LIN_FWD_FIELDS)
_LinBwd = _ptr_struct("_LinBwd", LIN_BWD_FIELDS)

ABI_VERSION = 5

EXPORTED_SYMBOLS = (
    "ttt_hip_mlp_forward_workspace", "ttt_hip_mlp_backward_workspace", "ttt_hip_linear_forward_workspace",
    "ttt_hip_linear_backward_workspace", "ttt_hip_mlp_forward", "ttt_hip_mlp_forward_chunk", "ttt_hip_mlp_backward", "ttt_hip_linear_forward",
    "ttt_hip_linear_backward", "ttt_hip_resolve_impl", "ttt_hip_abi_version", "ttt_hip_last_error",
    "ttt_hip_debug_timing", "ttt_hip_debug_groups_per_chunk", "ttt_hip_debug_dump", "ttt_hip_debug_option", "ttt_hip_debug_sweep_error", "ttt_hip_sweep_error_clear", "ttt_hip_debug_occupy_cus",
    "ttt_hip_stream_create_masked", "ttt_hip_stream_destroy", "ttt_hip_debug_placement_probe",
    "ttt_hip_pre_forward", "ttt_hip_pre_forward_range", "ttt_hip_post_forward_range", "ttt_hip_pre_backward_partials", "ttt_hip_pre_backward", "ttt_hip_pre_backward_ld", "ttt_hip_post_partials",
    "ttt_hip_post_forward", "ttt_hip_post_backward", "ttt_hip_gate_forward", "ttt_hip_gate_backward_partials",
    "ttt_hip_gate_backward", "ttt_hip_attn_forward", "ttt_hip_attn_backward",
    "ttt_hip_attn_pre_forward", "ttt_hip_attn_pre_partials", "ttt_hip_attn_pre_backward", "ttt_hip_attn_pre_backward_ld",
    "ttt_hip_adaln_forward", "ttt_hip_adaln_backward_partials", "ttt_hip_adaln_backward",
    "ttt_hip_resgate_forward", "ttt_hip_resgate_backward_partials", "ttt_hip_resgate_backward",
)

_lib: Optional[ctypes.CDLL] = None


def library_path() -> str:
    return _LIB_PATH


def load_library() -> ctypes.CDLL:
    global _lib
    if _lib is not None:
        return _lib
    if not os.path.exists(_LIB_PATH):
        raise RuntimeError(
            f"test_time_training: HIP library not found at {_LIB_PATH}; build it with "
            f"`python -c 'import __graft_entry__ as g; g.build()'` (there is no CPU fallback)")
    lib = ctypes.CDLL(_LIB_PATH)
    for n in ("mlp_forward", "mlp_backward", "linear_forward", "linear_backward"):
        getattr(lib, f"ttt_hip_{n}_workspace").restype = ctypes.c_size_t
        getattr(lib, f"ttt_hip_{n}_workspace").argtypes = [ctypes.c_void_p]
        getattr(lib, f"ttt_hip_{n}").restype = ctypes.c_int
        getattr(lib, f"ttt_hip_{n}").argtypes = [ctypes.c_void_p, ctypes.c_void_p, ctypes.c_void_p, ctypes.c_size_t, ctypes.c_void_p]
    lib.ttt_hip_resolve_impl.restype = ctypes.c_int
    lib.ttt_hip_resolve_impl.argtypes = [ctypes.c_void_p, ctypes.c_int, ctypes.c_int]
    lib.ttt_hip_abi_version.restype = ctypes.c_int
    lib.ttt_hip_last_error.restype = ctypes.c_char_p
    if lib.ttt_hip_abi_version() != ABI_VERSION:
        raise RuntimeError(f"test_time_training: libttt_hip.so ABI version {lib.ttt_hip_abi_version()}, this binding needs {ABI_VERSION}: rebuild (csrc/build.sh)")
    _lib = lib
    return lib


def debug_timing(buf: Optional[torch.Tensor]) -> None:
    lib = load_library()
    lib.ttt_hip_debug_timing.argtypes = [ctypes.c_void_p]
    lib.ttt_hip_debug_timing(buf.data_ptr() if buf is not None else None)


def debug_groups_per_chunk(groups: int) -> None:
    lib = load_library()
    lib.ttt_hip_debug_groups_per_chunk.argtypes = [ctypes.c_int]
    lib.ttt_hip_debug_groups_per_chunk(int(groups))


def debug_option(name: str, value: int) -> None:
    lib = load_library()
    lib.ttt_hip_debug_option.argtypes = [ctypes.c_char_p, ctypes.c_int]
    lib.ttt_hip_debug_option.restype = ctypes.c_int
    if lib.ttt_hip_debug_option(name.encode(), int(value)) != 0:
        raise ValueError(f"unknown debug option {name!r}")


def sweep_error() -> int:
    lib = load_library()
    lib.ttt_hip_debug_sweep_error.restype = ctypes.c_uint
    return int(lib.ttt_hip_debug_sweep_error())


def debug_occupy_cus(workgroups: int, lds_bytes: int, microseconds: int, stream=None) -> None:
    lib = load_library()
    st = (stream or torch.cuda.current_stream()).cuda_stream
    lib.ttt_hip_debug_occupy_cus.restype = ctypes.c_int
    if lib.ttt_hip_debug_occupy_cus(int(workgroups), int(lds_bytes), int(microseconds), ctypes.c_void_p(st)) != 0:
        raise RuntimeError("ttt_hip_debug_occupy_cus: bad arguments or launch failure")


def masked_stream(cu_mask_words) -> "torch.cuda.ExternalStream":
    lib = load_library()
    words = [int(w) & 0xFFFFFFFF for w in cu_mask_words]
    arr = (ctypes.c_uint * len(words))(*words)
    out = ctypes.c_void_p()
    lib.ttt_hip_stream_create_masked.restype = ctypes.c_int
    if lib.ttt_hip_stream_create_masked(arr, len(words), ctypes.byref(out)) != 0:
        lib.ttt_hip_last_error.restype = ctypes.c_char_p
        raise RuntimeError(lib.ttt_hip_last_error().decode())
    return torch.cuda.ExternalStream(out.value)


def placement_probe(workgroups: int, stream=None, lds_bytes: int = 150 * 1024, microseconds: int = 200):
    lib = load_library()
    st = stream or torch.cuda.current_stream()
    out = torch.zeros(workgroups, dtype=torch.int32, device="cuda")
    lib.ttt_hip_debug_placement_probe.restype = ctypes.c_int
    with torch.cuda.stream(st):
        rc = lib.ttt_hip_debug_placement_probe(ctypes.c_void_p(out.data_ptr()), int(workgroups), int(lds_bytes), int(microseconds), ctypes.c_void_p(st.cuda_stream))
    if rc != 0:
        raise RuntimeError("ttt_hip_debug_placement_probe: bad arguments or launch failure")
    st.synchronize()
    w = out.cpu().tolist()
    return [((v >> 16) & 0xF, (v >> 13) & 0x7, (v >> 12) & 0x1, (v >> 8) & 0xF) for v in w]


def sweep_error_clear() -> None:
    load_library().ttt_hip_sweep_error_clear()


def sweep_fast_count() -> int:
    lib = load_library()
    lib.ttt_hip_debug_option.argtypes = [ctypes.c_char_p, ctypes.c_int]
    lib.ttt_hip_debug_option.restype = ctypes.c_int
    return -2 - int(lib.ttt_hip_debug_option(b"sweep_fast_count", 0))


def debug_dump(buf: Optional[torch.Tensor]) -> None:
    lib = load_library()
    lib.ttt_hip_debug_dump.argtypes = [ctypes.c_void_p]
    lib.ttt_hip_debug_dump(buf.data_ptr() if buf is not None else None)


def set_impl(name: str) -> None:
    _state["impl"] = _IMPL_NAMES[name]


def get_impl() -> str:
    return {v: k for k, v in _IMPL_NAMES.items()}[_state["impl"]]


def set_ln_eps(eps: float) -> None:
    _state["eps"] = float(eps)


def get_ln_eps() -> float:
    return _state["eps"]


def _check(t: torch.Tensor, name: str, shape, dtype) -> None:
    if not isinstance(t, torch.Tensor):
        raise TypeError(f"{name}: expected a torch.Tensor")
    if not t.is_cuda:
        raise RuntimeError(f"{name}: tensor must live on a HIP device (got {t.device}); there is no CPU path")
    if t.dtype != dtype:
        raise RuntimeError(f"{name}: expected dtype {dtype}, got {t.dtype}")
    if shape is not None and tuple(t.shape) != tuple(shape):
        raise RuntimeError(f"{name}: expected shape {tuple(shape)}, got {tuple(t.shape)}")
    if not t.is_contiguous():
        raise RuntimeError(f"{name}: tensor must be contiguous")


def _check5(XQ) -> None:
    if not isinstance(XQ, torch.Tensor) or XQ.ndim != 5:
        raise RuntimeError("XQ: expected a 5-D tensor [B, NH, NC, CS, F]")


def _dims(B, NH, NC, CS, F, G, act_dtype) -> _Dims:
    if act_dtype == torch.bfloat16:
        code = 0
    elif act_dtype == torch.float32:
        code = 1
    else:
        raise RuntimeError(f"activations must be bfloat16 or float32, got {act_dtype}")
# ... 239 lines not shown


def pre_forward(XQ_raw, XK_raw, XV_raw, rope, src, pos, ln_w, ln_b, XQ, XK, XV, NH, n_pos=None, t0=0, tn=None):
    B, L, D = XQ_raw.shape
    _req_maps(rope, src, pos, L, D // NH, n_pos)
    for t, n in ((XQ_raw, "XQ_raw"), (XK_raw, "XK_raw"), (XV_raw, "XV_raw"), (XQ, "XQ"), (XK, "XK"), (XV, "XV")):
        _req(t, n, torch.bfloat16)
    for t, n in ((ln_w, "ln_w"), (ln_b, "ln_b")):
        _req(t, n, torch.float32)
    _call("ttt_hip_pre_forward_range", B, L, NH, D // NH, _p(XQ_raw), _p(XK_raw), _p(XV_raw), _p(rope), _p(src), _p(pos), _p(ln_w), _p(ln_b),
          _p(XQ), _p(XK), _p(XV), int(t0), int(L - t0 if tn is None else tn), device=XQ_raw.device)


def pre_backward_partials(NH):
    return load_library().ttt_hip_pre_backward_partials(int(NH))


def _req_rows(t, name, shape, ld):
    if not isinstance(t, torch.Tensor) or not t.is_cuda or t.dtype != torch.bfloat16 or tuple(t.shape) != tuple(shape) \
            or t.stride(2) != 1 or t.stride(1) != ld or (shape[0] > 1 and t.stride(0) != shape[1] * ld) or t.data_ptr() % 16:
        raise RuntimeError(f"{name}: expected a bf16 {tuple(shape)} tensor on a HIP device with token rows {ld} elements apart")


def pre_backward(XQ_raw, XK_raw, XV_raw, rope, src, pos, ln_w, dXQ, dXK, dXV, dXQ_raw, dXK_raw, dXV_raw, dlnw_part, dlnb_part, NH, ld_out=None):
    B, L, D = XQ_raw.shape
    for t, n in ((XQ_raw, "XQ_raw"), (XK_raw, "XK_raw"), (XV_raw, "XV_raw"), (dXQ, "dXQ"), (dXK, "dXK"), (dXV, "dXV")):
        _req(t, n, torch.bfloat16)
    for t, n in ((dXQ_raw, "dXQ_raw"), (dXK_raw, "dXK_raw"), (dXV_raw, "dXV_raw")):
        if ld_out is None:
            _req(t, n, torch.bfloat16)
        else:
            _req_rows(t, n, (B, L, D), int(ld_out))
    for t, n in ((ln_w, "ln_w"), (dlnw_part, "dlnw_part"), (dlnb_part, "dlnb_part")):
        _req(t, n, torch.float32)
    _call("ttt_hip_pre_backward_ld", B, L, NH, D // NH, _p(XQ_raw), _p(XK_raw), _p(XV_raw), _p(rope), _p(src), _p(pos), _p(ln_w),
          _p(dXQ), _p(dXK), _p(dXV), _p(dXQ_raw), _p(dXK_raw), _p(dXV_raw), ctypes.c_int64(D if ld_out is None else int(ld_out)),
          _p(dlnw_part), _p(dlnb_part), device=XQ_raw.device)


def post_partials(B, L):
    return load_library().ttt_hip_post_partials(int(B), int(L))


def post_forward(Y, src, w, b, out, eps, t0=0, tn=None):
    B, NH, L, F = Y.shape
    _req(Y, "Y", torch.bfloat16); _req(out, "out", torch.bfloat16); _req(w, "w", torch.float32); _req(b, "b", torch.float32)
    _call("ttt_hip_post_forward_range", B, L, NH, F, ctypes.c_float(eps), _p(Y), _p(src), _p(w), _p(b), _p(out),
          int(t0), int(L - t0 if tn is None else tn), device=Y.device)


def post_backward(Y, dOut, src, w, dY, dw_part, db_part, eps):
    B, NH, L, F = Y.shape
    _req(Y, "Y", torch.bfloat16); _req(dOut, "dOut", torch.bfloat16); _req(dY, "dY", torch.bfloat16)
    _req(w, "w", torch.float32); _req(dw_part, "dw_part", torch.float32); _req(db_part, "db_part", torch.float32)
    _call("ttt_hip_post_backward", B, L, NH, F, ctypes.c_float(eps), _p(Y), _p(dOut), _p(src), _p(w), _p(dY), _p(dw_part), _p(db_part),
          device=Y.device)


def gate_forward(res, y, tanh_text, tanh_video, out, n_text):
    B, L, D = res.shape
    _req(res, "res", torch.bfloat16); _req(y, "y", torch.bfloat16); _req(out, "out", torch.bfloat16)
    _req(tanh_text, "tanh_text", torch.float32); _req(tanh_video, "tanh_video", torch.float32)
    _call("ttt_hip_gate_forward", B, L, D, int(n_text), _p(res), _p(y), _p(tanh_text), _p(tanh_video), _p(out), device=res.device)


def gate_backward_partials(D):
    return load_library().ttt_hip_gate_backward_partials(int(D))


def gate_backward(g, y, tanh_text, tanh_video, dy, dtanh_part, n_text):
    B, L, D = g.shape
    _req(g, "g", torch.bfloat16); _req(y, "y", torch.bfloat16); _req(dy, "dy", torch.bfloat16)
    _req(tanh_text, "tanh_text", torch.float32); _req(tanh_video, "tanh_video", torch.float32); _req(dtanh_part, "dtanh_part", torch.float32)
    _call("ttt_hip_gate_backward", B, L, D, int(n_text), _p(g), _p(y), _p(tanh_text), _p(tanh_video), _p(dy), _p(dtanh_part), device=g.device)


class _AttnTensor(ctypes.Structure):
    _fields_ = [("ptr", ctypes.c_void_p), ("stride_b", ctypes.c_int64), ("stride_h", ctypes.c_int64), ("stride_s", ctypes.c_int64)]


class _AttnFwd(ctypes.Structure):
    _fields_ = [("Q", _AttnTensor), ("K", _AttnTensor), ("V", _AttnTensor), ("O", _AttnTensor), ("LSE", ctypes.c_void_p),
                ("B", ctypes.c_int32), ("NH", ctypes.c_int32), ("S", ctypes.c_int32), ("D", ctypes.c_int32), ("scale", ctypes.c_float)]


class _AttnBwd(ctypes.Structure):
    _fields_ = [(n, _AttnTensor) for n in ("Q", "K", "V", "O", "dO", "dQ", "dK", "dV")] + [
        ("LSE", ctypes.c_void_p), ("Delta", ctypes.c_void_p),
        ("B", ctypes.c_int32), ("NH", ctypes.c_int32), ("S", ctypes.c_int32), ("D", ctypes.c_int32), ("scale", ctypes.c_float)]


def _attn_tensor(t, name, shape):
    if not isinstance(t, torch.Tensor) or not t.is_cuda or t.dtype != torch.bfloat16:
        raise RuntimeError(f"{name}: expected a bfloat16 tensor on a HIP device (there is no CPU path)")
    if tuple(t.shape) != tuple(shape):
        raise RuntimeError(f"{name}: expected shape {tuple(shape)}, got {tuple(t.shape)}")
    if t.stride(3) != 1:
        raise RuntimeError(f"{name}: the head dimension must be contiguous")
    return _AttnTensor(t.data_ptr(), t.stride(0), t.stride(1), t.stride(2))


def attn_forward(q, k, v, out, lse, scale):
    B, NH, S, D = q.shape
    a = _AttnFwd(_attn_tensor(q, "q", (B, NH, S, D)), _attn_tensor(k, "k", (B, NH, S, D)), _attn_tensor(v, "v", (B, NH, S, D)),
                 _attn_tensor(out, "out", (B, NH, S, D)), lse.data_ptr() if lse is not None else None, B, NH, S, D, float(scale))
    if lse is not None:
        _req(lse, "lse", torch.float32)
    _call("ttt_hip_attn_forward", ctypes.byref(a), device=q.device)


def attn_backward(q, k, v, out, dout, lse, delta, dq, dk, dv, scale):
    B, NH, S, D = q.shape
    sh = (B, NH, S, D)
    _req(lse, "lse", torch.float32); _req(delta, "delta", torch.float32)
    a = _AttnBwd(_attn_tensor(q, "q", sh), _attn_tensor(k, "k", sh), _attn_tensor(v, "v", sh), _attn_tensor(out, "out", sh),
                 _attn_tensor(dout, "dout", sh), _attn_tensor(dq, "dq", sh), _attn_tensor(dk, "dk", sh), _attn_tensor(dv, "dv", sh),
                 lse.data_ptr(), delta.data_ptr(), B, NH, S, D, float(scale))
    _call("ttt_hip_attn_backward", ctypes.byref(a), device=q.device)


def attn_pre_forward(q_raw, k_raw, wq, bq, wk, bk, cos, sin, q, k, NH, n_text, eps):
    B, S, D = q_raw.shape
    for t, n in ((q_raw, "q_raw"), (k_raw, "k_raw"), (q, "q"), (k, "k")):
        _req(t, n, torch.bfloat16)
    for t, n in ((wq, "wq"), (bq, "bq"), (wk, "wk"), (bk, "bk"), (cos, "cos"), (sin, "sin")):
        _req(t, n, torch.float32)
    if D != NH * 64 or cos.shape[-1] != 64 or cos.shape[0] < S - n_text:
        raise RuntimeError("attn_pre_forward: head_dim must be 64 and the rope tables must cover the video tokens")
    _call("ttt_hip_attn_pre_forward", B, S, NH, int(n_text), ctypes.c_float(eps), _p(q_raw), _p(k_raw), _p(wq), _p(bq), _p(wk), _p(bk),
          _p(cos), _p(sin), _p(q), _p(k), device=q_raw.device)


def attn_pre_partials(B, S, NH):
    return load_library().ttt_hip_attn_pre_partials(int(B), int(S), int(NH))


def attn_pre_backward(q_raw, k_raw, dq, dk, wq, wk, cos, sin, dq_raw, dk_raw, part, NH, n_text, eps, ld_out=None):
    B, S, D = q_raw.shape
    for t, n in ((q_raw, "q_raw"), (k_raw, "k_raw")):
        _req(t, n, torch.bfloat16)
    for t, n in ((dq_raw, "dq_raw"), (dk_raw, "dk_raw")):
        if ld_out is None:
            _req(t, n, torch.bfloat16)
        else:
            _req_rows(t, n, (B, S, D), int(ld_out))
    for t, n in ((wq, "wq"), (wk, "wk"), (cos, "cos"), (sin, "sin"), (part, "part")):
        _req(t, n, torch.float32)
    tq, tk = _attn_tensor(dq, "dq", (B, NH, S, 64)), _attn_tensor(dk, "dk", (B, NH, S, 64))
    _call("ttt_hip_attn_pre_backward_ld", B, S, NH, int(n_text), ctypes.c_float(eps), _p(q_raw), _p(k_raw), ctypes.byref(tq), ctypes.byref(tk),
          _p(wq), _p(wk), _p(cos), _p(sin), _p(dq_raw), _p(dk_raw), ctypes.c_int64(D if ld_out is None else int(ld_out)), _p(part),
          device=q_raw.device)


def adaln_forward(vid, text, w, b, shift, scale1p, out, eps):
    B, Lv, D = vid.shape
    Lt = text.shape[1]
    for t, n in ((vid, "vid"), (text, "text"), (out, "out")):
        _req(t, n, torch.bfloat16)
    for t, n in ((w, "w"), (b, "b"), (shift, "shift"), (scale1p, "scale1p")):
        _req(t, n, torch.float32)
    if tuple(out.shape) != (B, Lt + Lv, D) or tuple(shift.shape) != (B, 2, D) or tuple(scale1p.shape) != (B, 2, D):
        raise RuntimeError("adaln_forward: out must be [B, Lt+Lv, D], shift / scale1p [B, 2, D]")
    _call("ttt_hip_adaln_forward", B, Lt, Lv, D, ctypes.c_float(eps), _p(vid), _p(text), _p(w), _p(b), _p(shift), _p(scale1p), _p(out),
          device=vid.device)


def adaln_backward_partials():
    return load_library().ttt_hip_adaln_backward_partials()


def adaln_backward(vid, text, dout, w, b, scale1p, dvid, dtext, part, eps):
    B, Lv, D = vid.shape
    Lt = text.shape[1]
    for t, n in ((vid, "vid"), (text, "text"), (dout, "dout"), (dvid, "dvid"), (dtext, "dtext")):
        _req(t, n, torch.bfloat16)
    for t, n in ((w, "w"), (b, "b"), (scale1p, "scale1p"), (part, "part")):
        _req(t, n, torch.float32)
    _call("ttt_hip_adaln_backward", B, Lt, Lv, D, ctypes.c_float(eps), _p(vid), _p(text), _p(dout), _p(w), _p(b), _p(scale1p),
          _p(dvid), _p(dtext), _p(part), device=vid.device)


def resgate_forward(vid, text, y, gate, ovid, otext):
    B, Lv, D = vid.shape
    Lt = text.shape[1]
    for t, n in ((vid, "vid"), (text, "text"), (y, "y"), (ovid, "ovid"), (otext, "otext")):
        _req(t, n, torch.bfloat16)
    _req(gate, "gate", torch.float32)
    if tuple(y.shape) != (B, Lt + Lv, D) or tuple(gate.shape) != (B, 2, D):
        raise RuntimeError("resgate_forward: y must be [B, Lt+Lv, D], gate [B, 2, D]")
    _call("ttt_hip_resgate_forward", B, Lt, Lv, D, _p(vid), _p(text), _p(y), _p(gate), _p(ovid), _p(otext), device=vid.device)


def resgate_backward_partials(D):
    return load_library().ttt_hip_resgate_backward_partials(int(D))


def resgate_backward(dvid, dtext, y, gate, dy, dgate_part):
    B, Lv, D = dvid.shape
    Lt = dtext.shape[1]
    for t, n in ((dvid, "dvid"), (dtext, "dtext"), (y, "y"), (dy, "dy")):
        _req(t, n, torch.bfloat16)
    _req(gate, "gate", torch.float32); _req(dgate_part, "dgate_part", torch.float32)
    _call("ttt_hip_resgate_backward", B, Lt, Lv, D, _p(dvid), _p(dtext), _p(y), _p(gate), _p(dy), _p(dgate_part), device=dvid.device)
```

ttt-video-dit_amd/ttt_amd/models/cogvideo/attention.py:

```python
from __future__ import annotations

import math

import torch
import torch.nn.functional as F

from ttt_amd.infra.remat_cache import kernel_result


def _ext():
    import test_time_training
    return test_time_training


class SegmentAttention(torch.autograd.Function):
    @staticmethod
    def forward(ctx, q, k, v):
        ext = _ext()
        B, NH, S, D = q.shape
        scale = 1.0 / math.sqrt(D)
        out = torch.empty(B, S, NH, D, device=q.device, dtype=q.dtype).transpose(1, 2)
        lse = torch.empty(B, NH, S, device=q.device, dtype=torch.float32)
        ext.attn_forward(q, k, v, out, lse, scale)
        ctx.save_for_backward(q, k, v, out, lse)
        ctx.scale = scale
        return out

    @staticmethod
    def backward(ctx, dout):
        ext = _ext()
        q, k, v, out, lse = ctx.saved_tensors
        B, NH, S, D = q.shape
        if dout.stride(3) != 1:
            dout = dout.contiguous()
        mk = lambda: torch.empty(B, S, NH, D, device=q.device, dtype=q.dtype).transpose(1, 2)
        dq, dk, dv = mk(), mk(), mk()
        delta = torch.empty(B, NH, S, device=q.device, dtype=torch.float32)
        ext.attn_backward(q, k, v, out, dout, lse, delta, dq, dk, dv, ctx.scale)
        return dq, dk, dv


def segment_attention(q: torch.Tensor, k: torch.Tensor, v: torch.Tensor) -> torch.Tensor:
    if q.is_cuda:
        if q.dtype != torch.bfloat16 or q.shape[-1] != 64:
            raise RuntimeError("segment_attention: the HIP kernels need bf16 activations and head_dim 64 "
                               f"(got {q.dtype}, head_dim {q.shape[-1]}); no fallback on a GPU")
        fix = lambda t: t if t.stride(3) == 1 else t.contiguous()
        return SegmentAttention.apply(fix(q), fix(k), fix(v))
    return F.scaled_dot_product_attention(q, k, v, attn_mask=None, dropout_p=0.0, is_causal=False)


class AttnPre(torch.autograd.Function):

    @staticmethod
    def forward(ctx, q_raw, k_raw, wq, bq, wk, bk, cos, sin, NH, n_text, eps):
        ext = _ext()
        B, S, D = q_raw.shape
        qr, kr = q_raw.contiguous(), k_raw.contiguous()
        f32 = lambda t: t.detach().to(torch.float32).contiguous()
        wq32, bq32, wk32, bk32 = f32(wq), f32(bq), f32(wk), f32(bk)
        q, k = torch.empty_like(qr), torch.empty_like(kr)
        ext.attn_pre_forward(qr, kr, wq32, bq32, wk32, bk32, cos, sin, q, k, NH, n_text, float(eps))
        ctx.save_for_backward(qr, kr, wq32, wk32, cos, sin)
        ctx.meta = (NH, n_text, float(eps), wq.dtype)
        view = lambda t: t.view(B, S, NH, D // NH).transpose(1, 2)
        return view(q), view(k)

    @staticmethod
    def backward(ctx, dq, dk):
        ext = _ext()
        qr, kr, wq32, wk32, cos, sin = ctx.saved_tensors
        NH, n_text, eps, pdt = ctx.meta
        B, S, D = qr.shape
        fix = lambda t: t if t.stride(3) == 1 else t.contiguous()
        dq, dk = fix(dq), fix(dk)
        dq_raw, dk_raw = torch.empty_like(qr), torch.empty_like(kr)
        P = ext.attn_pre_partials(B, S, NH)
        part = torch.empty(P, 4, 64, device=qr.device, dtype=torch.float32)
        ext.attn_pre_backward(qr, kr, dq, dk, wq32, wk32, cos, sin, dq_raw, dk_raw, part, NH, n_text, eps)
        g = part.sum(0).to(pdt)
        return dq_raw, dk_raw, g[0], g[1], g[2], g[3], None, None, None, None, None


def attn_pre_available(x: torch.Tensor, head_dim: int) -> bool:
    return x.is_cuda and x.dtype == torch.bfloat16 and head_dim == 64


class FusedSegmentAttention(torch.autograd.Function):

    @staticmethod
    def forward(ctx, q_raw, k_raw, v, wq, bq, wk, bk, cos, sin, NH, n_text, eps):
        ext = _ext()
        B, S, D = q_raw.shape
        Dh = D // NH
        qr, kr = q_raw.contiguous(), k_raw.contiguous()
        v = v if v.stride(3) == 1 else v.contiguous()
        f32 = lambda t: t.detach().to(torch.float32).contiguous()
        p32 = (f32(wq), f32(bq), f32(wk), f32(bk))
        scale = 1.0 / math.sqrt(Dh)

        def run():
            q, k = torch.empty_like(qr), torch.empty_like(kr)
            ext.attn_pre_forward(qr, kr, *p32, cos, sin, q, k, NH, n_text, float(eps))
            view = lambda t: t.view(B, S, NH, Dh).transpose(1, 2)
            out = torch.empty(B, S, NH, Dh, device=qr.device, dtype=qr.dtype).transpose(1, 2)
            lse = torch.empty(B, NH, S, device=qr.device, dtype=torch.float32)
            ext.attn_forward(view(q), view(k), v, out, lse, scale)
            return out, lse

        out, lse = kernel_result("attn", run)
        ctx.save_for_backward(qr, kr, v, out, lse, *p32, cos, sin)
        ctx.meta = (NH, n_text, float(eps), scale, wq.dtype)
        return out

    @staticmethod
    def backward(ctx, dout):
        ext = _ext()
        qr, kr, v, out, lse, wq32, bq32, wk32, bk32, cos, sin = ctx.saved_tensors
        NH, n_text, eps, scale, pdt = ctx.meta
        B, S, D = qr.shape
        Dh = D // NH
        q, k = torch.empty_like(qr), torch.empty_like(kr)
        ext.attn_pre_forward(qr, kr, wq32, bq32, wk32, bk32, cos, sin, q, k, NH, n_text, eps)
        view = lambda t: t.view(B, S, NH, Dh).transpose(1, 2)
        if dout.stride(3) != 1:
            dout = dout.contiguous()
        mk = lambda: torch.empty(B, S, NH, Dh, device=qr.device, dtype=qr.dtype).transpose(1, 2)
        dq, dk = mk(), mk()
        from ttt_amd.models.ssm.fused import qkv_grad_blocks
        dq_raw, dk_raw, dv_blk = qkv_grad_blocks(qr)
        dv = dv_blk.view(B, S, NH, Dh).transpose(1, 2)
        delta = torch.empty(B, NH, S, device=qr.device, dtype=torch.float32)
        ext.attn_backward(view(q), view(k), v, out, dout, lse, delta, dq, dk, dv, scale)
        del q, k
        P = ext.attn_pre_partials(B, S, NH)
        part = torch.empty(P, 4, 64, device=qr.device, dtype=torch.float32)
        ext.attn_pre_backward(qr, kr, dq, dk, wq32, wk32, cos, sin, dq_raw, dk_raw, part, NH, n_text, eps, ld_out=dq_raw.stride(1))
        g = part.sum(0).to(pdt)
        return dq_raw, dk_raw, dv, g[0], g[1], g[2], g[3], None, None, None, None, None
```

ttt-video-dit_amd/ttt_amd/models/cogvideo/dit.py:

```python
from __future__ import annotations

import contextlib

import torch
import torch.nn.functional as F
from torch import nn
from torch.utils.checkpoint import checkpoint

from ttt_amd.infra import remat_cache
from ttt_amd.infra.fused_linear import linear3
from ttt_amd.models.cogvideo.attention import FusedSegmentAttention, attn_pre_available, segment_attention
from ttt_amd.models.cogvideo.utils import (Rotary3DPositionEmbedding, SequenceMetadata, modulate,
                                           timestep_embedding, unpatchify)
from ttt_amd.models.configs import ModelConfig
from ttt_amd.models.ssm.fused import FusedAdaLN, FusedGate, FusedResGate, fused_available
from ttt_amd.models.ssm.ttt_layer import TTTWrapper


def _ckpt(fn, enabled: bool):
    if not enabled:
        return fn
    return lambda *a: checkpoint(fn, *a, use_reentrant=False, context_fn=lambda: (remat_cache.suspended(), remat_cache.suspended()))


class GeluLinear(torch.autograd.Function):

    @staticmethod
    def forward(ctx, z, weight, bias):
        ctx.save_for_backward(z, weight)
        ctx.has_bias = bias is not None
        return remat_cache.kernel_result("fc2", lambda: (F.linear(F.gelu(z, approximate="tanh"), weight, bias),))[0]

    @staticmethod
    def backward(ctx, dy):
        z, weight = ctx.saved_tensors
        need_z, need_w, need_b = ctx.needs_input_grad
        dw = db = dz = None
        dy2 = dy.reshape(-1, dy.shape[-1])
        if need_w:
            h = F.gelu(z, approximate="tanh")
            dw = dy2.t().mm(h.reshape(-1, h.shape[-1]))
            del h
        if need_b and ctx.has_bias:
            db = dy2.sum(0)
        if need_z:
            dz = torch.ops.aten.gelu_backward(dy.matmul(weight), z, approximate="tanh")
        return dz, dw, db


def _segment_geometry(meta: SequenceMetadata, n_video: int, attn_length: int, prefix: int):
    tl, tpf = meta.text_length, meta.tokens_per_frame
    rng = [(i * attn_length * tpf, min((prefix + (i + 1) * attn_length) * tpf, n_video)) for i in range(meta.num_chunks)]
    shared = prefix * tpf
    assert 0 < prefix < attn_length and rng[-1][1] == n_video and all(hi - lo > shared for lo, hi in rng), \
        "segments must tile the video, consecutive ones sharing `prefix` frames"
    return tl, rng, shared


class SegmentSplit(torch.autograd.Function):

    @staticmethod
    def forward(ctx, x, n_text, tl, rng, shared):
        ctx.geo = (n_text, tl, rng, shared, x.shape)
        return tuple(torch.cat((x[:, i * tl:(i + 1) * tl], x[:, n_text + lo:n_text + hi]), dim=1) for i, (lo, hi) in enumerate(rng))

    @staticmethod
    def backward(ctx, *gs):
        n_text, tl, rng, shared, shape = ctx.geo
        ref = next(g for g in gs if g is not None)
        gs = [g if g is not None else ref.new_zeros(shape[0], tl + hi - lo, shape[2]) for g, (lo, hi) in zip(gs, rng)]
        dx = ref.new_empty(shape)
        for i, (lo, hi) in enumerate(rng):
            dx[:, i * tl:(i + 1) * tl] = gs[i][:, :tl]
            dx[:, n_text + lo:n_text + hi] = gs[i][:, tl:]
        for i in range(1, len(rng)):
            lo = rng[i][0]
            torch.add(gs[i - 1][:, -shared:], gs[i][:, tl:tl + shared], out=dx[:, n_text + lo:n_text + lo + shared])
        return dx, None, None, None, None


class SegmentMerge(torch.autograd.Function):

    @staticmethod
    def forward(ctx, n_text, tl, rng, shared, *outs):
        ctx.geo = (n_text, tl, rng, shared)
        b, _, d = outs[0].shape
        out = outs[0].new_empty(b, n_text + rng[-1][1], d)
        for i, (lo, hi) in enumerate(rng):
            out[:, i * tl:(i + 1) * tl] = outs[i][:, :tl]
            out[:, n_text + lo:n_text + hi] = outs[i][:, tl:]
        for i in range(1, len(rng)):
            lo = rng[i][0]
            blk = out[:, n_text + lo:n_text + lo + shared]
            torch.add(outs[i - 1][:, -shared:], outs[i][:, tl:tl + shared], out=blk)
            blk.div_(2)
        return out

    @staticmethod
    def backward(ctx, g):
        n_text, tl, rng, shared = ctx.geo
        gs = [torch.cat((g[:, i * tl:(i + 1) * tl], g[:, n_text + lo:n_text + hi]), dim=1) for i, (lo, hi) in enumerate(rng)]
        for i in range(1, len(rng)):
            gs[i - 1][:, -shared:].div_(2)
            gs[i][:, tl:tl + shared].div_(2)
        return (None, None, None, None, *gs)


class PatchEmbedding(nn.Module):

    def __init__(self, config: ModelConfig):
        super().__init__()
        train = config.adapter_method == "sft"
        self.vid_proj = nn.Conv2d(config.in_channels, config.model_dim, config.patch_size, config.patch_size, bias=True).requires_grad_(train)
        self.text_proj = nn.Linear(config.text_dim, config.model_dim, bias=True).requires_grad_(train)

    def forward(self, video, text_encoding):
        b, t, c, H, W = video.shape
        conv = self.vid_proj
        ph, pw = conv.kernel_size
        if conv.stride == conv.kernel_size and conv.padding == (0, 0) and H % ph == 0 and W % pw == 0:
            h, w = H // ph, W // pw
            patches = video.reshape(b * t, c, h, ph, w, pw).permute(0, 2, 4, 1, 3, 5).reshape(b, t * h * w, c * ph * pw)
            x = F.linear(patches, conv.weight.reshape(conv.out_channels, -1), conv.bias)
        else:
            x = conv(video.flatten(0, 1))
            x = x.flatten(2).transpose(1, 2).reshape(b, -1, x.shape[1])
        return self.text_proj(text_encoding).contiguous(), x.contiguous()


class MLP(nn.Module):

    def __init__(self, config: ModelConfig):
        super().__init__()
        train = config.adapter_method == "sft"
        self.do_remat = config.remat_mlp
        self.requires_grad = train
        self.layer1 = nn.Linear(config.model_dim, 4 * config.model_dim, bias=True).requires_grad_(train)
        self.layer2 = nn.Linear(4 * config.model_dim, config.model_dim, bias=True).requires_grad_(train)
        self.tp_mesh = None

    def _run(self, x):
        z = self.layer1(x)
        w2 = self.layer2.weight
        if z.is_cuda and type(w2) in (torch.Tensor, nn.Parameter) and torch.is_grad_enabled():
            return GeluLinear.apply(z, w2, self.layer2.bias)
        return self.layer2(F.gelu(z, approximate="tanh"))

    def forward(self, x):
        return _ckpt(self._run, self.do_remat)(x)


class SSMGating(nn.Module):

    def __init__(self, config):
        super().__init__()
        self.gating_alpha = nn.Parameter(torch.ones(config.model_dim) * config.gating_alpha_init)

    def forward(self, x):
        return torch.tanh(self.gating_alpha) * x


class SeqModelingBlock(nn.Module):

    def __init__(self, config: ModelConfig):
        super().__init__()
        train = config.adapter_method in ("sft", "qkvo")
        assert config.adapter_method in ("sft", "qkvo", "none"), f"Invalid adapter method: {config.adapter_method}"
        self.do_attn_remat = config.remat_attention
        self.do_forward_ssm_remat = config.remat_forward_ssm
        self.do_reverse_ssm_remat = config.remat_reverse_ssm
        self.num_heads = config.num_heads
        self.head_dim = config.model_dim // config.num_heads
        self.prefix_temporal_length = config.prefix_temporal_length
        self.attn_length = config.attn_length

        self.q_norm = nn.LayerNorm(self.head_dim, eps=config.layer_norm_eps).requires_grad_(train)
        self.k_norm = nn.LayerNorm(self.head_dim, eps=config.layer_norm_eps).requires_grad_(train)
        self.rotary = Rotary3DPositionEmbedding(config.latent_height, config.latent_width, config.compressed_num_frames,
                                                self.head_dim, config.theta)
        D = config.model_dim
        self.q = nn.Linear(D, D, bias=True)
        self.k = nn.Linear(D, D, bias=True)
        self.v = nn.Linear(D, D, bias=True)
        self.o = nn.Linear(D, D, bias=True)
        self.ssm = TTTWrapper(config)
        self.forward_ssm_gating_video = SSMGating(config)
        self.forward_ssm_gating_text = SSMGating(config)
        self.backward_ssm_gating_video = SSMGating(config)
        self.backward_ssm_gating_text = SSMGating(config)

    def _segment(self, emb, n_text):
        b, s, _ = emb.shape
        heads = lambda t: t.view(b, s, self.num_heads, self.head_dim).transpose(1, 2)
        if attn_pre_available(emb, self.head_dim):
            cos, sin = self.rotary.tables_f32()
            q, k, v = linear3(self.q, self.k, self.v, emb)
            a = FusedSegmentAttention.apply(q, k, heads(v),
                                            self.q_norm.weight, self.q_norm.bias, self.k_norm.weight, self.k_norm.bias, cos, sin,
                                            self.num_heads, n_text, self.q_norm.eps)
            return self.o(a.transpose(1, 2).reshape(b, s, -1))
        else:
            q, k, v = (heads(t) for t in linear3(self.q, self.k, self.v, emb))
            q, k = self.q_norm(q), self.k_norm(k)
            q = torch.cat((q[:, :, :n_text], self.rotary(q[:, :, n_text:])), dim=2)
            k = torch.cat((k[:, :, :n_text], self.rotary(k[:, :, n_text:])), dim=2)
        a = segment_attention(q, k, v)
        return self.o(a.transpose(1, 2).reshape(b, s, -1))

    def _attn_forward(self, vid_emb, text_emb, seq_metadata: SequenceMetadata, cat=None):
        tl, tpf = seq_metadata.text_length, seq_metadata.tokens_per_frame
        if seq_metadata.num_chunks == 1:
            return self._segment(cat if cat is not None else torch.cat((text_emb, vid_emb), dim=1), tl)
        x = cat if cat is not None else torch.cat((text_emb, vid_emb), dim=1)
        n_text = text_emb.shape[1]
        tl, rng, shared = _segment_geometry(seq_metadata, vid_emb.shape[1], self.attn_length, self.prefix_temporal_length)
        segs = SegmentSplit.apply(x, n_text, tl, rng, shared)
        return SegmentMerge.apply(n_text, tl, rng, shared, *(self._segment(seg, tl) for seg in segs))

    def _gate(self, text_gate, video_gate, residual, ssm_output, n_text):
        if fused_available(residual, 64) and residual.shape[-1] % 8 == 0:
            return FusedGate.apply(residual, ssm_output, text_gate.gating_alpha, video_gate.gating_alpha, n_text)
        return residual + torch.cat((text_gate(ssm_output[:, :n_text]), video_gate(ssm_output[:, n_text:])), dim=1)

    def _ssm_forward(self, emb, seq_metadata: SequenceMetadata):
        n_text = seq_metadata.seq_text_length
        fwd = _ckpt(self.ssm, self.do_forward_ssm_remat)
        rev = _ckpt(self.ssm, self.do_reverse_ssm_remat)
        emb = self._gate(self.forward_ssm_gating_text, self.forward_ssm_gating_video, emb, fwd(emb, seq_metadata, False), n_text)
        y = rev(emb, seq_metadata, True)
        return self._gate(self.backward_ssm_gating_text, self.backward_ssm_gating_video, emb, y, n_text)

    def _segment_heads(self, emb, n_text, h0, h1):
        b, s, _ = emb.shape
        nh, Fh = h1 - h0, self.head_dim
        sl = slice(h0 * Fh, h1 * Fh)
        lin = lambda m: F.linear(emb, m.weight[sl], m.bias[sl])
        heads = lambda t: t.view(b, s, nh, Fh).transpose(1, 2)
        if attn_pre_available(emb, Fh):
            cos, sin = self.rotary.tables_f32()
            a = FusedSegmentAttention.apply(lin(self.q), lin(self.k), heads(lin(self.v)), self.q_norm.weight, self.q_norm.bias,
                                            self.k_norm.weight, self.k_norm.bias, cos, sin, nh, n_text, self.q_norm.eps)
        else:
            q, k, v = heads(lin(self.q)), heads(lin(self.k)), heads(lin(self.v))
            q, k = self.q_norm(q), self.k_norm(k)
            q = torch.cat((q[:, :, :n_text], self.rotary(q[:, :, n_text:])), dim=2)
            k = torch.cat((k[:, :, :n_text], self.rotary(k[:, :, n_text:])), dim=2)
            a = segment_attention(q, k, v)
        return a.transpose(1, 2).reshape(b, s, -1)

    def _attn_heads(self, vid_emb, text_emb, seq_metadata: SequenceMetadata, h0, h1):
        tl, tpf = seq_metadata.text_length, seq_metadata.tokens_per_frame
        if seq_metadata.num_chunks == 1:
            return self._segment_heads(torch.cat((text_emb, vid_emb), dim=1), tl, h0, h1)
        d = (h1 - h0) * self.head_dim
        out_vid = vid_emb.new_zeros(*vid_emb.shape[:2], d)
        out_txt = text_emb.new_zeros(*text_emb.shape[:2], d)
        count = torch.zeros_like(vid_emb[..., :1])
        for i in range(seq_metadata.num_chunks):
            lo = i * self.attn_length * tpf
            hi = (self.prefix_temporal_length + (i + 1) * self.attn_length) * tpf
            o = self._segment_heads(torch.cat((text_emb[:, i * tl:(i + 1) * tl], vid_emb[:, lo:hi]), dim=1), tl, h0, h1)
            out_txt[:, i * tl:(i + 1) * tl] = o[:, :tl]
            out_vid[:, lo:hi] += o[:, tl:]
            count[:, lo:hi] += 1
        return torch.cat((out_txt, out_vid / count), dim=1)

    def forward_sp(self, vid_loc, text_loc, seq_metadata: SequenceMetadata, sp):
        n_text = seq_metadata.seq_text_length
        n_vid = seq_metadata.num_frames * seq_metadata.tokens_per_frame
        h0, h1 = sp.head_range(self.num_heads)
        a = self._attn_heads(sp.gather_tokens(vid_loc, n_vid), sp.gather_tokens(text_loc, n_text), seq_metadata, h0, h1)
        text_loc, vid_loc = self.o(sp.heads_to_tokens(a[:, :n_text])), self.o(sp.heads_to_tokens(a[:, n_text:]))
        ttt = self.ssm.ttt
        for g_text, g_vid, reverse in ((self.forward_ssm_gating_text, self.forward_ssm_gating_video, False),
                                       (self.backward_ssm_gating_text, self.backward_ssm_gating_video, True)):
            full = torch.cat((sp.gather_tokens(text_loc, n_text), sp.gather_tokens(vid_loc, n_vid)), dim=1)
            y = self.ssm.forward_heads(full, seq_metadata, reverse, h0, h1)
            y_text = ttt.wo(ttt.post_norm(sp.heads_to_tokens(y[:, :n_text])))
            y_vid = ttt.wo(ttt.post_norm(sp.heads_to_tokens(y[:, n_text:])))
            text_loc, vid_loc = text_loc + g_text(y_text), vid_loc + g_vid(y_vid)
        return vid_loc, text_loc

    def forward_cat(self, x, seq_metadata: SequenceMetadata):
        n_text = seq_metadata.seq_text_length
        x = _ckpt(self._attn_forward, self.do_attn_remat)(x[:, n_text:], x[:, :n_text], seq_metadata, x)
        return self._ssm_forward(x, seq_metadata)

    def forward(self, vid_emb, text_emb, seq_metadata: SequenceMetadata):
        x = _ckpt(self._attn_forward, self.do_attn_remat)(vid_emb, text_emb, seq_metadata)
        x = self._ssm_forward(x, seq_metadata)
        n_text = seq_metadata.seq_text_length
        return x[:, n_text:], x[:, :n_text]


class TransformerLayer(nn.Module):

    def __init__(self, config):
        super().__init__()
        train = config.adapter_method == "sft"
        self.remat_seq_modeling_block = config.remat_seq_modeling_block
        self.tp_mesh = None
        self.use_fused_glue = True
        D = config.model_dim
        self.pre_seq_layernorm = nn.LayerNorm(D, eps=config.layer_norm_eps).requires_grad_(train)
        self.pre_seq_adaLN_modulation = nn.Sequential(nn.SiLU(), nn.Linear(config.time_embed_dim, 6 * D, bias=True).requires_grad_(train))
        self.seq_modeling_block = SeqModelingBlock(config)
        self.pre_mlp_layernorm = nn.LayerNorm(D, eps=config.layer_norm_eps).requires_grad_(train)
        self.pre_mlp_adaLN_modulation = nn.Sequential(nn.SiLU(), nn.Linear(config.time_embed_dim, 6 * D, bias=True).requires_grad_(train))
        self.mlp = MLP(config)

    def _forward_fused(self, vid_emb, text_emb, seq_metadata: SequenceMetadata):
        t = seq_metadata.t_emb
        ln1, ln2 = self.pre_seq_layernorm, self.pre_mlp_layernorm
        sh_v, sc_v, g_v, sh_t, sc_t, g_t = self.pre_seq_adaLN_modulation(t).chunk(6, dim=1)
        x = FusedAdaLN.apply(vid_emb, text_emb, ln1.weight, ln1.bias, sh_v, sc_v, sh_t, sc_t, ln1.eps)
        y = _ckpt(self.seq_modeling_block.forward_cat, self.remat_seq_modeling_block)(x, seq_metadata)
        vid_emb, text_emb = FusedResGate.apply(vid_emb, text_emb, y, g_v, g_t)
        sh_v, sc_v, g_v, sh_t, sc_t, g_t = self.pre_mlp_adaLN_modulation(t).chunk(6, dim=1)
        x = FusedAdaLN.apply(vid_emb, text_emb, ln2.weight, ln2.bias, sh_v, sc_v, sh_t, sc_t, ln2.eps)
        y = self.mlp(x)
        return FusedResGate.apply(vid_emb, text_emb, y, g_v, g_t)

    def forward_sp(self, vid_emb, text_emb, seq_metadata: SequenceMetadata, sp):
        t = seq_metadata.t_emb
        if self.use_fused_glue and fused_available(vid_emb, 64) and vid_emb.shape[-1] % 8 == 0 and vid_emb.shape[-1] <= 4096:
            ln1, ln2, nt = self.pre_seq_layernorm, self.pre_mlp_layernorm, text_emb.shape[1]
            sh_v, sc_v, g_v, sh_t, sc_t, g_t = self.pre_seq_adaLN_modulation(t).chunk(6, dim=1)
            x = FusedAdaLN.apply(vid_emb, text_emb, ln1.weight, ln1.bias, sh_v, sc_v, sh_t, sc_t, ln1.eps)
            v_out, t_out = self.seq_modeling_block.forward_sp(x[:, nt:], x[:, :nt], seq_metadata, sp)
            vid_emb, text_emb = FusedResGate.apply(vid_emb, text_emb, torch.cat((t_out, v_out), dim=1), g_v, g_t)
            sh_v, sc_v, g_v, sh_t, sc_t, g_t = self.pre_mlp_adaLN_modulation(t).chunk(6, dim=1)
            x = FusedAdaLN.apply(vid_emb, text_emb, ln2.weight, ln2.bias, sh_v, sc_v, sh_t, sc_t, ln2.eps)
            return FusedResGate.apply(vid_emb, text_emb, self.mlp(x), g_v, g_t)
        sh_v, sc_v, g_v, sh_t, sc_t, g_t = self.pre_seq_adaLN_modulation(t).chunk(6, dim=1)
        v_out, t_out = self.seq_modeling_block.forward_sp(modulate(self.pre_seq_layernorm(vid_emb), sh_v, sc_v),
                                                          modulate(self.pre_seq_layernorm(text_emb), sh_t, sc_t), seq_metadata, sp)
        vid_emb = vid_emb + g_v.unsqueeze(1) * v_out
        text_emb = text_emb + g_t.unsqueeze(1) * t_out
        sh_v, sc_v, g_v, sh_t, sc_t, g_t = self.pre_mlp_adaLN_modulation(t).chunk(6, dim=1)
        vid_emb = vid_emb + g_v.unsqueeze(1) * self.mlp(modulate(self.pre_mlp_layernorm(vid_emb), sh_v, sc_v))
        text_emb = text_emb + g_t.unsqueeze(1) * self.mlp(modulate(self.pre_mlp_layernorm(text_emb), sh_t, sc_t))
        return vid_emb, text_emb

    def forward(self, vid_emb, text_emb, seq_metadata: SequenceMetadata, sp=None):
        if sp is not None:
            return self.forward_sp(vid_emb, text_emb, seq_metadata, sp)
        if self.use_fused_glue and fused_available(vid_emb, 64) and vid_emb.shape[-1] % 8 == 0 and vid_emb.shape[-1] <= 4096:
            return self._forward_fused(vid_emb, text_emb, seq_metadata)
        n_text = seq_metadata.seq_text_length
        t = seq_metadata.t_emb
        sh_v, sc_v, g_v, sh_t, sc_t, g_t = self.pre_seq_adaLN_modulation(t).chunk(6, dim=1)
        block = _ckpt(self.seq_modeling_block, self.remat_seq_modeling_block)
        v_out, t_out = block(modulate(self.pre_seq_layernorm(vid_emb), sh_v, sc_v),
                             modulate(self.pre_seq_layernorm(text_emb), sh_t, sc_t), seq_metadata)
        vid_emb = vid_emb + g_v.unsqueeze(1) * v_out
        text_emb = text_emb + g_t.unsqueeze(1) * t_out

        sh_v, sc_v, g_v, sh_t, sc_t, g_t = self.pre_mlp_adaLN_modulation(t).chunk(6, dim=1)
        x = torch.cat((modulate(self.pre_mlp_layernorm(text_emb), sh_t, sc_t),
                       modulate(self.pre_mlp_layernorm(vid_emb), sh_v, sc_v)), dim=1)
        y = self.mlp(x)
        vid_emb = vid_emb + g_v.unsqueeze(1) * y[:, n_text:]
        text_emb = text_emb + g_t.unsqueeze(1) * y[:, :n_text]
        return vid_emb, text_emb


class FinalLayer(nn.Module):

# ... 92 lines not shown
```

Before: 8602.

## Run segmented attention directly on full-sequence QKV with in-kernel segment addressing

```diff
diff --git a/include/ttt_hip.h b/include/ttt_hip.h
--- a/include/ttt_hip.h
+++ b/include/ttt_hip.h
@@ -165,6 +165,48 @@
                                  const float* cos_table, const float* sin_table, void* dq_raw, void* dk_raw, int64_t ld_out, float* part,
                                  void* stream);
 
+typedef struct ttt_attn_rows {
+    void*   ptr0;
+    void*   ptr1;
+    int64_t stride_b, stride_h, stride_s;
+    int32_t n_split;
+    int32_t reserved;
+} ttt_attn_rows;
+typedef struct ttt_attn_seg_fwd_args {
+    ttt_attn_tensor Q, K;
+    ttt_attn_rows   V, O;
+    ttt_attn_tensor O_side[2];
+    int32_t side_lo[2], side_hi[2];
+    float*  LSE;
+    int32_t B, NH, S, D;
+    float   scale;
+} ttt_attn_seg_fwd_args;
+typedef struct ttt_attn_seg_bwd_args {
+    ttt_attn_tensor Q, K;
+    ttt_attn_rows   V, O, dO;
+    ttt_attn_tensor O_side[2];
+    int32_t side_lo[2], side_hi[2];
+    int32_t half_lo[2], half_hi[2];
+    ttt_attn_tensor dQ, dK;
+    ttt_attn_rows   dV;
+    int32_t acc_lo, acc_hi;
+    const float* LSE;
+    float*  Delta;
+    int32_t B, NH, S, D;
+    float   scale;
+} ttt_attn_seg_bwd_args;
+int ttt_hip_attn_forward_seg(const ttt_attn_seg_fwd_args* a, void* stream);
+int ttt_hip_attn_backward_seg(const ttt_attn_seg_bwd_args* a, void* stream);
+int ttt_hip_attn_average(int B, int n, int d, const void* a, const void* b, int64_t ab_stride_b, int64_t ab_stride_s,
+                         void* out, int64_t out_stride_b, int64_t out_stride_s, void* stream);
+int ttt_hip_attn_pre_forward_seg(int B, int S, int NH, int n_text, float eps, const ttt_attn_rows* q_raw, const ttt_attn_rows* k_raw,
+                                 const float* wq, const float* bq, const float* wk, const float* bk,
+                                 const float* cos_table, const float* sin_table, void* q, void* k, void* stream);
+int ttt_hip_attn_pre_backward_seg(int B, int S, int NH, int n_text, float eps, const ttt_attn_rows* q_raw, const ttt_attn_rows* k_raw,
+                                  const ttt_attn_tensor* dq, const ttt_attn_tensor* dk, const float* wq, const float* wk,
+                                  const float* cos_table, const float* sin_table, const ttt_attn_rows* dq_raw, const ttt_attn_rows* dk_raw,
+                                  int acc_lo, int acc_hi, float* part, void* stream);
+
 int ttt_hip_adaln_forward(int B, int Lt, int Lv, int D, float eps, const void* vid, const void* text, const float* w, const float* b,
                           const float* shift, const float* scale1p, void* out, void* stream);
 int ttt_hip_adaln_backward_partials(void);
diff --git a/ttt-video-dit_amd/csrc/attn.h b/ttt-video-dit_amd/csrc/attn.h
--- a/ttt-video-dit_amd/csrc/attn.h
+++ b/ttt-video-dit_amd/csrc/attn.h
@@ -13,6 +13,9 @@
     __bf16 *q, *k;
     int B, S, NH, n_text;
     float eps;
+    long q_dlo, k_dlo;
+    long in_sb, in_ss;
+    int n_split;
 };
 struct PreBwdParams {
     const __bf16 *q_raw, *k_raw, *dq, *dk;
@@ -23,6 +26,9 @@
     float* part;
     int B, S, NH, n_text;
     float eps;
+    long q_dlo, k_dlo, dq_raw_dlo, dk_raw_dlo;
+    long in_sb, in_ss, out_sb;
+    int n_split, acc_lo, acc_hi;
 };
 int  pre_blocks(long rows);
 void launch_pre_forward(const PreParams& a, hipStream_t s);
@@ -30,9 +36,18 @@
 
 void launch_forward(const FwdParams& p, hipStream_t s);
 void launch_backward(const BwdParams& p, hipStream_t s);
+void launch_forward_seg(const SegFwdParams& p, hipStream_t s);
+void launch_backward_seg(const SegBwdParams& p, hipStream_t s);
+struct AvgParams {
+    const __bf16 *a, *b;
+    __bf16* out;
+    long a_sb, a_ss, o_sb, o_ss;
+    int B, n, d;
+};
+void launch_average(const AvgParams& p, hipStream_t s);
 
-void launch_dq_v2(const BwdParams& p, hipStream_t s);
-void launch_dkdv_v2(const BwdParams& p, hipStream_t s);
+void launch_dq_v2(const SegBwdParams& p, hipStream_t s);
+void launch_dkdv_v2(const SegBwdParams& p, hipStream_t s);
 void set_debug_attn_variant(int v);
 
 }
diff --git a/ttt-video-dit_amd/csrc/attn_body.h b/ttt-video-dit_amd/csrc/attn_body.h
--- a/ttt-video-dit_amd/csrc/attn_body.h
+++ b/ttt-video-dit_amd/csrc/attn_body.h
@@ -105,6 +105,53 @@
         st.v = zero_u4();
     }
 }
+TTT_BODY_FN long pick_rows(long dlo, int n_split, int row0, int n, int row) {
+    long d = row0 >= n_split ? 0 : dlo;
+    if (row0 < n_split && row0 + n > n_split) {
+        d = row < n_split ? dlo : 0;
+        TTT_PIN_IN_BRANCH(d);
+    }
+    return d;
+}
+template <class P>
+TTT_BODY_FN const __bf16* v_rows(const P& p, const __bf16* Vp, long off, int row0, int n, int row) {
+    if constexpr (P::kSeg) return Vp + pick_rows(p.x.v_dlo, p.x.n_split, row0, n, row);
+    else return Vp;
+}
+template <class P>
+TTT_BODY_FN const __bf16* do_rows(const P& p, const __bf16* dOp, long off, int row0, int n, int row) {
+    if constexpr (P::kSeg) return dOp + pick_rows(p.x.do_dlo, p.x.n_split, row0, n, row);
+    else return dOp;
+}
+template <class P>
+TTT_BODY_FN bool half_tile(const P& p, int row0, int n) {
+    if constexpr (P::kSeg) return (row0 < p.x.h0_hi && row0 + n > p.x.h0_lo) || (row0 < p.x.h1_hi && row0 + n > p.x.h1_lo);
+    else return false;
+}
+template <class P>
+TTT_BODY_FN bool half_row(const P& p, int row) {
+    if constexpr (P::kSeg) return (row >= p.x.h0_lo && row < p.x.h0_hi) || (row >= p.x.h1_lo && row < p.x.h1_hi);
+    else return false;
+}
+TTT_BODY_FN bf16x8 halve8(bf16x8 a) {
+#pragma unroll
+    for (int e = 0; e < 8; ++e) a[e] = (__bf16)((float)a[e] * 0.5f);
+    return a;
+}
+TTT_BODY_FN u32x4 halve8(u32x4 a) { return __builtin_bit_cast(u32x4, halve8(__builtin_bit_cast(bf16x8, a))); }
+template <class P>
+TTT_BODY_FN void kv_issue_p(KVStage& st, const P& p, const __bf16* Kp, const __bf16* Vp, long v_off, int kv0, int tid) {
+    const int row = tid >> 3, col = (tid & 7) * 8;
+    const int key = kv0 + row;
+    if (key < p.S) {
+        st.k = *reinterpret_cast<const u32x4*>(Kp + (long)key * p.k_ss + col);
+        st.v = *reinterpret_cast<const u32x4*>(v_rows(p, Vp, v_off, kv0, KB, key) + (long)key * p.v_ss + col);
+    } else {
+        st.k = zero_u4();
+        st.v = zero_u4();
+    }
+}
+
 template <class BK>
 TTT_BODY_FN void kv_park(BK& bk, const KVStage& st, typename BK::tile_t k_img, typename BK::tile_t v_img, int v_stride, int tid) {
     const int row = tid >> 3, col = (tid & 7) * 8;
@@ -416,14 +463,15 @@
     }
 }
 
-template <int NSUB, int NQ, class BK>
-TTT_BODY_FN void dq_wide(BK& bk, const BwdParams& p, int bh, int qb) {
+template <int NSUB, int NQ, class BK, class P = BwdParams>
+TTT_BODY_FN void dq_wide(BK& bk, const P& p, int bh, int qb) {
     const int tid = bk.thread(), wv = bk.wave(), l = bk.lane(), h = l >> 5, c = l & 31;
     const int bb = bh / p.NH, hh = bh % p.NH;
     const __bf16* Qp = p.Q + (long)bb * p.q_sb + (long)hh * p.q_sh;
     const __bf16* Kp = p.K + (long)bb * p.k_sb + (long)hh * p.k_sh;
     const __bf16* Vp = p.V + (long)bb * p.v_sb + (long)hh * p.v_sh;
     const __bf16* dOp = p.dO + (long)bb * p.do_sb + (long)hh * p.do_sh;
+    const long v_off = (long)bb * p.v_sb + (long)hh * p.v_sh, do_off = (long)bb * p.do_sb + (long)hh * p.do_sh;
 
     int qrow[NQ];
     bool qvalid[NQ];
@@ -437,7 +485,12 @@
 #pragma unroll
         for (int kk = 0; kk < 4; ++kk) {
             Qf[qi][kk] = qvalid[qi] ? *reinterpret_cast<const bf16x8*>(Qp + (long)qrow[qi] * p.q_ss + 16 * kk + 8 * h) : zero_frag();
-            Df[qi][kk] = qvalid[qi] ? *reinterpret_cast<const bf16x8*>(dOp + (long)qrow[qi] * p.do_ss + 16 * kk + 8 * h) : zero_frag();
+            Df[qi][kk] = qvalid[qi] ? *reinterpret_cast<const bf16x8*>(do_rows(p, dOp, do_off, qb * (QB * NQ) + 32 * NQ * wv + 32 * qi, 32, qrow[qi]) + (long)qrow[qi] * p.do_ss + 16 * kk + 8 * h) : zero_frag();
+        }
+        if (half_tile(p, qb * (QB * NQ) + 32 * NQ * wv + 32 * qi, 32)) {
+            const bool hv = half_row(p, qrow[qi]);
+#pragma unroll
+            for (int kk = 0; kk < 4; ++kk) Df[qi][kk] = hv ? halve8(Df[qi][kk]) : Df[qi][kk];
         }
         lse2[qi] = qvalid[qi] ? p.LSE[(long)bh * p.S + qrow[qi]] * LOG2E : 1e30f;
         delta[qi] = qvalid[qi] ? p.Delta[(long)bh * p.S + qrow[qi]] : 0.f;
@@ -453,7 +506,7 @@
     const typename BK::tile_t lds = bk.lds_base();
 #pragma unroll
     for (int u = 0; u < NSUB; ++u) {
-        kv_issue(st, Kp, Vp, p.k_ss, p.v_ss, u * KB, p.S, tid);
+        kv_issue_p(st, p, Kp, Vp, v_off, u * KB, tid);
         kv_park_s<false>(bk, st, lds + u * DQ_BUF_ELEMS, lds + u * DQ_BUF_ELEMS + KT_ELEMS, tid);
     }
     bk.barrier();
@@ -464,7 +517,7 @@
 #pragma unroll
         for (int u = 0; u < NSUB; ++u) {
             const int jt = j * NSUB + u;
-            if (more) kv_issue(st, Kp, Vp, p.k_ss, p.v_ss, ((j + 1) * NSUB + u) * KB, p.S, tid);
+            if (more) kv_issue_p(st, p, Kp, Vp, v_off, ((j + 1) * NSUB + u) * KB, tid);
             if (jt < nt) {
             const typename BK::tile_t Kt = stage + u * DQ_BUF_ELEMS, Vt = Kt + KT_ELEMS;
             const bool ragged = jt + 1 == nt && (p.S & (KB - 1));
@@ -542,15 +595,21 @@
     u32x4 q, d;
     float lse, del;
 };
-template <bool ACC_INIT>
-TTT_BODY_FN void qstage_issue(QStage& st, const BwdParams& p, const __bf16* Qp, const __bf16* dOp, const float* lse, const float* del,
-                              float inv_scale, int q0, int tid) {
+template <bool ACC_INIT, class P>
+TTT_BODY_FN void qstage_issue(QStage& st, const P& p, const __bf16* Qp, const __bf16* dOp, const float* lse, const float* del,
+                              float inv_scale, int q0, int tid, long do_off = 0) {
     if (tid < 512) {
         const int row = tid >> 3, col = (tid & 7) * 8;
         const int q = q0 + row;
         if (q < p.S) {
             st.q = *reinterpret_cast<const u32x4*>(Qp + (long)q * p.q_ss + col);
-            st.d = *reinterpret_cast<const u32x4*>(dOp + (long)q * p.do_ss + col);
+            st.d = *reinterpret_cast<const u32x4*>(do_rows(p, dOp, do_off, q0, 64, q) + (long)q * p.do_ss + col);
+            if (half_tile(p, q0, 64)) {
+                if (half_row(p, q)) st.d = halve8(st.d);
+                unsigned t = st.d[0];
+                TTT_PIN_IN_BRANCH(t);
+                st.d[0] = t;
+            }
         } else {
             st.q = zero_u4();
             st.d = zero_u4();
@@ -699,8 +758,8 @@
         }
 }
 
-template <int NW, bool ACC_INIT, int NSUB, bool SWZ = false, class BK>
-TTT_BODY_FN void dkdv_staged(BK& bk, const BwdParams& p, int bh, int kvb) {
+template <int NW, bool ACC_INIT, int NSUB, bool SWZ = false, class BK, class P = BwdParams>
+TTT_BODY_FN void dkdv_staged(BK& bk, const P& p, int bh, int kvb) {
     const int tid = bk.thread(), wv = bk.wave(), l = bk.lane(), h = l >> 5, c = l & 31;
     const int bb = bh / p.NH, hh = bh % p.NH;
     const __bf16* Qp = p.Q + (long)bb * p.q_sb + (long)hh * p.q_sh;
@@ -709,6 +768,7 @@
     const __bf16* dOp = p.dO + (long)bb * p.do_sb + (long)hh * p.do_sh;
     const float* lse = p.LSE + (long)bh * p.S;
     const float* del = p.Delta + (long)bh * p.S;
+    const long v_off = (long)bb * p.v_sb + (long)hh * p.v_sh, do_off = (long)bb * p.do_sb + (long)hh * p.do_sh;
 
     const int key0 = kvb * (32 * NW) + 32 * wv;
     const int krow = key0 + c;
@@ -716,7 +776,7 @@
 #pragma unroll
     for (int kk = 0; kk < 4; ++kk) {
         Kf[kk] = krow < p.S ? *reinterpret_cast<const bf16x8*>(Kp + (long)krow * p.k_ss + 16 * kk + 8 * h) : zero_frag();
-        Vf[kk] = krow < p.S ? *reinterpret_cast<const bf16x8*>(Vp + (long)krow * p.v_ss + 16 * kk + 8 * h) : zero_frag();
+        Vf[kk] = krow < p.S ? *reinterpret_cast<const bf16x8*>(v_rows(p, Vp, v_off, key0, 32, krow) + (long)krow * p.v_ss + 16 * kk + 8 * h) : zero_frag();
     }
     f32x16 dK[2] = {zero16(), zero16()}, dV[2] = {zero16(), zero16()};
     const float sc = p.scale * LOG2E, inv_scale = 1.0f / p.scale;
@@ -728,7 +788,7 @@
     QStage st;
 #pragma unroll
     for (int u = 0; u < NSUB; ++u) {
-        qstage_issue<ACC_INIT>(st, p, Qp, dOp, lse, del, inv_scale, u * 64, tid);
+        qstage_issue<ACC_INIT>(st, p, Qp, dOp, lse, del, inv_scale, u * 64, tid, do_off);
         qstage_park_s<SWZ>(bk, st, lds + u * DKV_BUF_ELEMS, tid);
     }
     bk.barrier();
@@ -739,7 +799,7 @@
         const bool more = j + 1 < ns;
 #pragma unroll
         for (int u = 0; u < NSUB; ++u) {
-        if (more) qstage_issue<ACC_INIT>(st, p, Qp, dOp, lse, del, inv_scale, ((j + 1) * NSUB + u) * 64, tid);
+        if (more) qstage_issue<ACC_INIT>(st, p, Qp, dOp, lse, del, inv_scale, ((j + 1) * NSUB + u) * 64, tid, do_off);
         if (j * NSUB + u < nt) {
         const typename BK::tile_t buf = stage + u * DKV_BUF_ELEMS;
         const typename BK::tile_t Qt = buf, Dt = buf + KT_ELEMS;
@@ -799,6 +859,23 @@
 
     __bf16* dKp = p.dK + (long)bb * p.dk_sb + (long)hh * p.dk_sh;
     __bf16* dVp = p.dV + (long)bb * p.dv_sb + (long)hh * p.dv_sh;
+    if constexpr (P::kSeg) {
+        const bool acc_any = key0 < p.x.acc_hi && key0 + 32 > p.x.acc_lo;
+#pragma unroll
+        for (int db = 0; db < 2; ++db)
+#pragma unroll
+            for (int r = 0; r < 16; ++r) {
+                const int key = key0 + row_of(r, h);
+                if (key < p.S) {
+                    dKp[(long)key * p.dk_ss + 32 * db + c] = (__bf16)(dK[db][r] * p.scale);
+                    __bf16* dst = dVp + pick_rows(p.x.dv_dlo, p.x.n_split, key0, 32, key) + (long)key * p.dv_ss + 32 * db + c;
+                    __bf16 val = (__bf16)dV[db][r];
+                    if (acc_any && key >= p.x.acc_lo && key < p.x.acc_hi) val = (__bf16)((float)*dst + (float)val);
+                    *dst = val;
+                }
+            }
+        return;
+    }
 #pragma unroll
     for (int db = 0; db < 2; ++db)
 #pragma unroll
diff --git a/ttt-video-dit_amd/csrc/attn_bwd.hip b/ttt-video-dit_amd/csrc/attn_bwd.hip
--- a/ttt-video-dit_amd/csrc/attn_bwd.hip
+++ b/ttt-video-dit_amd/csrc/attn_bwd.hip
@@ -7,19 +7,27 @@
 namespace ttt {
 namespace attn {
 
-__global__ __launch_bounds__(256) void attn_delta_kernel(BwdParams p) {
+__global__ __launch_bounds__(256) void attn_delta_kernel(SegBwdParams p) {
     const long rows = (long)p.B * p.NH * p.S;
+    const int n_split = p.x.n_split, s0_lo = p.x.s0_lo, s0_hi = p.x.s0_hi, s1_lo = p.x.s1_lo, s1_hi = p.x.s1_hi;
+    const int h0_lo = p.x.h0_lo, h0_hi = p.x.h0_hi, h1_lo = p.x.h1_lo, h1_hi = p.x.h1_hi;
     for (long idx = (long)blockIdx.x * blockDim.x + threadIdx.x; idx < rows * 8; idx += (long)gridDim.x * blockDim.x) {
         const long row = idx >> 3;
         const int o = idx & 7;
         const int s = row % p.S;
         const int bh = row / p.S;
         const int b = bh / p.NH, h = bh % p.NH;
-        const bf16x8 a = *reinterpret_cast<const bf16x8*>(p.dO + (long)b * p.do_sb + (long)h * p.do_sh + (long)s * p.do_ss + 8 * o);
-        const bf16x8 c = *reinterpret_cast<const bf16x8*>(p.O + (long)b * p.o_sb + (long)h * p.o_sh + (long)s * p.o_ss + 8 * o);
+        const long dod = s < n_split ? p.x.do_dlo : 0;
+        const bool side0 = s >= s0_lo && s < s0_hi, side1 = s >= s1_lo && s < s1_hi;
+        const long od = side0 ? p.x.os0_d : side1 ? p.x.os1_d : s < n_split ? p.x.o_dlo : 0;
+        const bool side = side0 || side1;
+        const long o_off = (long)b * (side ? p.x.os_sb : p.o_sb) + (long)h * (side ? p.x.os_sh : p.o_sh) + (long)s * (side ? p.x.os_ss : p.o_ss);
+        const bf16x8 a = *reinterpret_cast<const bf16x8*>(p.dO + dod + (long)b * p.do_sb + (long)h * p.do_sh + (long)s * p.do_ss + 8 * o);
+        const bf16x8 c = *reinterpret_cast<const bf16x8*>(p.O + od + o_off + 8 * o);
+        const bool hv = (s >= h0_lo && s < h0_hi) || (s >= h1_lo && s < h1_hi);
         float acc = 0.f;
 #pragma unroll
-        for (int e = 0; e < 8; ++e) acc += (float)a[e] * (float)c[e];
+        for (int e = 0; e < 8; ++e) acc += (hv ? (float)(__bf16)((float)a[e] * 0.5f) : (float)a[e]) * (float)c[e];
         acc += __shfl_xor(acc, 1, 64);
         acc += __shfl_xor(acc, 2, 64);
         acc += __shfl_xor(acc, 4, 64);
@@ -27,13 +35,38 @@
     }
 }
 
-void launch_backward(const BwdParams& p, hipStream_t s) {
+__global__ __launch_bounds__(256) void attn_avg_kernel(AvgParams p) {
+    const int per = p.d >> 3;
+    const long total = (long)p.B * p.n * per;
+    for (long idx = (long)blockIdx.x * blockDim.x + threadIdx.x; idx < total; idx += (long)gridDim.x * blockDim.x) {
+        const int o = idx % per;
+        const long r = idx / per;
+        const int s = r % p.n, b = r / p.n;
+        const long ao = (long)b * p.a_sb + (long)s * p.a_ss + 8 * o;
+        const bf16x8 x = *reinterpret_cast<const bf16x8*>(p.a + ao), y = *reinterpret_cast<const bf16x8*>(p.b + ao);
+        bf16x8 z;
+#pragma unroll
+        for (int e = 0; e < 8; ++e) z[e] = (__bf16)((float)(__bf16)((float)x[e] + (float)y[e]) * 0.5f);
+        *reinterpret_cast<bf16x8*>(p.out + (long)b * p.o_sb + (long)s * p.o_ss + 8 * o) = z;
+    }
+}
+void launch_average(const AvgParams& p, hipStream_t s) {
+    const long g = ((long)p.B * p.n * (p.d >> 3) + 255) / 256;
+    hipLaunchKernelGGL(attn_avg_kernel, dim3((int)(g < 65536 ? g : 65536)), dim3(256), 0, s, p);
+}
+
+void launch_backward_seg(const SegBwdParams& p, hipStream_t s) {
     const long rows = (long)p.B * p.NH * p.S;
     const int dgrid = (int)((rows * 8 + 255) / 256 < 65536 ? (rows * 8 + 255) / 256 : 65536);
     hipLaunchKernelGGL(attn_delta_kernel, dim3(dgrid), dim3(256), 0, s, p);
     launch_dkdv_v2(p, s);
     launch_dq_v2(p, s);
 }
+void launch_backward(const BwdParams& p, hipStream_t s) {
+    SegBwdParams q = {};
+    static_cast<BwdParams&>(q) = p;
+    launch_backward_seg(q, s);
+}
 
 }
 }
diff --git a/ttt-video-dit_amd/csrc/attn_fwd.hip b/ttt-video-dit_amd/csrc/attn_fwd.hip
--- a/ttt-video-dit_amd/csrc/attn_fwd.hip
+++ b/ttt-video-dit_amd/csrc/attn_fwd.hip
@@ -18,10 +18,17 @@
     uint4 k, v;
 };
 
-__device__ __forceinline__ void stage_issue(KVStage& st, const __bf16* Kp, const __bf16* Vp, long k_ss, long v_ss, int kv0, int S, int tid) {
+__device__ __forceinline__ void stage_issue(KVStage& st, const __bf16* Kp, const __bf16* Vp, long v_dlo, int n_split, long k_ss, long v_ss,
+                                            int kv0, int S, int tid) {
     const int row = tid >> 3, col = (tid & 7) * 8;
     const int key = kv0 + row;
     if (key < S) {
+        long d = kv0 >= n_split ? 0 : v_dlo;
+        if (kv0 < n_split && kv0 + KB > n_split) {
+            d = key < n_split ? v_dlo : 0;
+            asm volatile("" : "+v"(d));
+        }
+        Vp += d;
         st.k = *reinterpret_cast<const uint4*>(Kp + (long)key * k_ss + col);
         st.v = *reinterpret_cast<const uint4*>(Vp + (long)key * v_ss + col);
     } else {
@@ -35,7 +42,7 @@
     *reinterpret_cast<uint4*>(Vt + row * VS + col) = st.v;
 }
 
-__global__ __launch_bounds__(NTF) void attn_fwd_kernel(FwdParams p) {
+__global__ __launch_bounds__(NTF) void attn_fwd_kernel(SegFwdParams p) {
     extern __shared__ __attribute__((aligned(16))) char smem[];
     __bf16* lds = reinterpret_cast<__bf16*>(smem);
 
@@ -83,7 +90,7 @@
 
     const int nt = (p.S + KB - 1) / KB;
     KVStage st;
-    stage_issue(st, Kp, Vp, p.k_ss, p.v_ss, 0, p.S, tid);
+    stage_issue(st, Kp, Vp, p.x.v_dlo, p.x.n_split, p.k_ss, p.v_ss, 0, p.S, tid);
     stage_park(st, lds, lds + KT_ELEMS, tid);
     __syncthreads();
 
@@ -91,7 +98,7 @@
         const __bf16* Kt = lds + (j & 1) * BUF_ELEMS;
         const __bf16* Vt = Kt + KT_ELEMS;
         const bool more = j + 1 < nt;
-        if (more) stage_issue(st, Kp, Vp, p.k_ss, p.v_ss, (j + 1) * KB, p.S, tid);
+        if (more) stage_issue(st, Kp, Vp, p.x.v_dlo, p.x.n_split, p.k_ss, p.v_ss, (j + 1) * KB, p.S, tid);
 
         f32x16 Sc[2];
 #pragma unroll
@@ -154,7 +161,12 @@
     const float ltot = lsum + half_swap(lsum);
     const float inv = 1.0f / ltot;
     if (qvalid) {
-        __bf16* orow = Op + (long)qrow * p.o_ss;
+        const SegExt& x = p.x;
+        long ooff;
+        if (qrow >= x.s0_lo && qrow < x.s0_hi) ooff = x.os0_d + (long)bb * x.os_sb + (long)hh * x.os_sh + (long)qrow * x.os_ss;
+        else if (qrow >= x.s1_lo && qrow < x.s1_hi) ooff = x.os1_d + (long)bb * x.os_sb + (long)hh * x.os_sh + (long)qrow * x.os_ss;
+        else ooff = (qrow < x.n_split ? x.o_dlo : 0) + (long)bb * p.o_sb + (long)hh * p.o_sh + (long)qrow * p.o_ss;
+        __bf16* orow = p.O + ooff;
 #pragma unroll
         for (int db = 0; db < 2; ++db)
 #pragma unroll
@@ -168,7 +180,7 @@
     }
 }
 
-void launch_forward(const FwdParams& p, hipStream_t s) {
+void launch_forward_seg(const SegFwdParams& p, hipStream_t s) {
     static ttt::OncePerDevice attr;
     attr.run([&] {
         (void)hipFuncSetAttribute((const void*)attn_fwd_kernel, hipFuncAttributeMaxDynamicSharedMemorySize, LDS_FWD);
@@ -176,6 +188,11 @@
     const int nqb = (p.S + QB - 1) / QB;
     hipLaunchKernelGGL(attn_fwd_kernel, dim3(p.B * p.NH * nqb), dim3(NTF), LDS_FWD, s, p);
 }
+void launch_forward(const FwdParams& p, hipStream_t s) {
+    SegFwdParams q = {};
+    static_cast<FwdParams&>(q) = p;
+    launch_forward_seg(q, s);
+}
 
 }
 }
diff --git a/ttt-video-dit_amd/csrc/attn_pre.hip b/ttt-video-dit_amd/csrc/attn_pre.hip
--- a/ttt-video-dit_amd/csrc/attn_pre.hip
+++ b/ttt-video-dit_amd/csrc/attn_pre.hip
@@ -19,6 +19,17 @@
     bf16x8 a;
 #pragma unroll
     for (int j = 0; j < 8; ++j) a[j] = (__bf16)v[j];
+    *reinterpret_cast<bf16x8*>(p) = a;
+}
+__device__ __forceinline__ void st8_acc(__bf16* p, const float (&v)[8], bool acc) {
+    bf16x8 a;
+#pragma unroll
+    for (int j = 0; j < 8; ++j) a[j] = (__bf16)v[j];
+    if (acc) {
+        const bf16x8 prev = *reinterpret_cast<const bf16x8*>(p);
+#pragma unroll
+        for (int j = 0; j < 8; ++j) a[j] = (__bf16)((float)prev[j] + (float)a[j]);
+    }
     *reinterpret_cast<bf16x8*>(p) = a;
 }
 __device__ __forceinline__ void ldf8(const float* p, float (&o)[8]) {
@@ -58,15 +69,20 @@
     float wq[8], bq[8], wk[8], bk[8];
     ldf8(a.wq + 8 * o, wq); ldf8(a.bq + 8 * o, bq); ldf8(a.wk + 8 * o, wk); ldf8(a.bk + 8 * o, bk);
     for (long idx = (long)blockIdx.x * blockDim.x + threadIdx.x; idx < total; idx += (long)gridDim.x * blockDim.x) {
-        const int s = ((idx >> 3) / a.NH) % a.S;
+        const long row = idx >> 3;
+        const int hd = row % a.NH;
+        const long tok = row / a.NH;
+        const int s = tok % a.S;
+        const int b = tok / a.S;
         const int pos = s - a.n_text;
         const float* cosr = pos >= 0 ? a.cos + (long)pos * 64 + 8 * o : nullptr;
         const float* sinr = pos >= 0 ? a.sin + (long)pos * 64 + 8 * o : nullptr;
+        const long in_off = (long)b * a.in_sb + (long)s * a.in_ss + hd * 64 + 8 * o;
         float x[8], y[8], xh[8], rstd;
-        ld8(a.q_raw + idx * 8, x);
+        ld8(a.q_raw + (s < a.n_split ? a.q_dlo : 0) + in_off, x);
         ln_rope(x, wq, bq, a.eps, cosr, sinr, y, xh, rstd);
         st8(a.q + idx * 8, y);
-        ld8(a.k_raw + idx * 8, x);
+        ld8(a.k_raw + (s < a.n_split ? a.k_dlo : 0) + in_off, x);
         ln_rope(x, wk, bk, a.eps, cosr, sinr, y, xh, rstd);
         st8(a.k + idx * 8, y);
     }
@@ -127,15 +143,18 @@
         const float* cosr = pos >= 0 ? a.cos + (long)pos * 64 + 8 * o : nullptr;
         const float* sinr = pos >= 0 ? a.sin + (long)pos * 64 + 8 * o : nullptr;
         float x[8], g[8], dx[8];
-        ld8(a.q_raw + idx * 8, x);
+        const bool lo = s < a.n_split;
+        const bool acc = s >= a.acc_lo && s < a.acc_hi;
+        const long in_off = (long)b * a.in_sb + (long)s * a.in_ss + hd * 64 + 8 * o;
+        const long raw_off = (long)b * a.out_sb + (long)s * a.ld_out + hd * 64 + 8 * o;
+        ld8(a.q_raw + (lo ? a.q_dlo : 0) + in_off, x);
         ld8(a.dq + (long)b * a.dq_sb + (long)hd * a.dq_sh + (long)s * a.dq_ss + 8 * o, g);
         ln_rope_bwd(x, wq, a.eps, cosr, sinr, g, dx, dwq, dbq);
-        const long raw_off = tok * a.ld_out + hd * 64 + 8 * o;
-        st8(a.dq_raw + raw_off, dx);
-        ld8(a.k_raw + idx * 8, x);
+        st8_acc(a.dq_raw + (lo ? a.dq_raw_dlo : 0) + raw_off, dx, acc);
+        ld8(a.k_raw + (lo ? a.k_dlo : 0) + in_off, x);
         ld8(a.dk + (long)b * a.dk_sb + (long)hd * a.dk_sh + (long)s * a.dk_ss + 8 * o, g);
         ln_rope_bwd(x, wk, a.eps, cosr, sinr, g, dx, dwk, dbk);
-        st8(a.dk_raw + raw_off, dx);
+        st8_acc(a.dk_raw + (lo ? a.dk_raw_dlo : 0) + raw_off, dx, acc);
     }
 #pragma unroll
     for (int j = 0; j < 8; ++j) {
diff --git a/ttt-video-dit_amd/csrc/attn_types.h b/ttt-video-dit_amd/csrc/attn_types.h
--- a/ttt-video-dit_amd/csrc/attn_types.h
+++ b/ttt-video-dit_amd/csrc/attn_types.h
@@ -11,6 +11,7 @@
     long q_sb, q_sh, q_ss, k_sb, k_sh, k_ss, v_sb, v_sh, v_ss, o_sb, o_sh, o_ss;
     int B, NH, S;
     float scale;
+    static constexpr bool kSeg = false;
 };
 struct BwdParams {
     const __bf16 *Q, *K, *V, *O, *dO;
@@ -21,6 +22,25 @@
     long dq_sb, dq_sh, dq_ss, dk_sb, dk_sh, dk_ss, dv_sb, dv_sh, dv_ss;
     int B, NH, S;
     float scale;
+    static constexpr bool kSeg = false;
+};
+
+struct SegExt {
+    long v_dlo, o_dlo, do_dlo, dv_dlo;
+    long os0_d, os1_d;
+    long os_sb, os_sh, os_ss;
+    int n_split;
+    int s0_lo, s0_hi, s1_lo, s1_hi;
+    int h0_lo, h0_hi, h1_lo, h1_hi;
+    int acc_lo, acc_hi;
+};
+struct SegFwdParams : FwdParams {
+    static constexpr bool kSeg = true;
+    SegExt x;
+};
+struct SegBwdParams : BwdParams {
+    static constexpr bool kSeg = true;
+    SegExt x;
 };
 
 }
diff --git a/ttt-video-dit_amd/csrc/attn_v2.hip b/ttt-video-dit_amd/csrc/attn_v2.hip
--- a/ttt-video-dit_amd/csrc/attn_v2.hip
+++ b/ttt-video-dit_amd/csrc/attn_v2.hip
@@ -33,7 +33,7 @@
 };
 
 template <int NW, bool ACC_INIT, int MINW, int NSUB, int VAR>
-__global__ __launch_bounds__(64 * NW, MINW) void attn_dkdv2s_kernel(BwdParams p) {
+__global__ __launch_bounds__(64 * NW, MINW) void attn_dkdv2s_kernel(SegBwdParams p) {
     extern __shared__ __attribute__((aligned(16))) char smem[];
     int bh, kvb;
     attnb::head_of_block(blockIdx.x, (p.S + 32 * NW - 1) / (32 * NW), p.B * p.NH, bh, kvb);
@@ -41,7 +41,7 @@
     attnb::dkdv_staged<NW, ACC_INIT, NSUB, false>(bk, p, bh, kvb);
 }
 template <int NSUB, int VAR>
-__global__ __launch_bounds__(512, 2) void attn_dq_wide_kernel(BwdParams p) {
+__global__ __launch_bounds__(512, 2) void attn_dq_wide_kernel(SegBwdParams p) {
     extern __shared__ __attribute__((aligned(16))) char smem[];
     int bh, qb;
     attnb::head_of_block(blockIdx.x, (p.S + 2 * attnb::QB - 1) / (2 * attnb::QB), p.B * p.NH, bh, qb);
@@ -53,7 +53,7 @@
 void set_debug_attn_variant(int v) { g_attn_variant = v; }
 
 template <int VAR>
-static void launch_dq_var(const BwdParams& p, hipStream_t s) {
+static void launch_dq_var(const SegBwdParams& p, hipStream_t s) {
     constexpr int NSUB = 1;
     static ttt::OncePerDevice attr;
     attr.run([&] {
@@ -62,13 +62,13 @@
     const int nb = (p.S + 2 * attnb::QB - 1) / (2 * attnb::QB);
     hipLaunchKernelGGL((attn_dq_wide_kernel<NSUB, VAR>), dim3(p.B * p.NH * nb), dim3(512), NSUB * attnb::LDS_DQ, s, p);
 }
-void launch_dq_v2(const BwdParams& p, hipStream_t s) {
+void launch_dq_v2(const SegBwdParams& p, hipStream_t s) {
     if (g_attn_variant) launch_dq_var<1>(p, s);
     else launch_dq_var<0>(p, s);
 }
 
 template <int VAR>
-static void launch_dkdv_var(const BwdParams& p, hipStream_t s) {
+static void launch_dkdv_var(const SegBwdParams& p, hipStream_t s) {
     constexpr int NW = 12, NSUB = 2;
     static_assert(NSUB * attnb::LDS_DKV <= 160 * 1024, "LDS budget");
     static ttt::OncePerDevice attr;
@@ -78,7 +78,7 @@
     const int nb = (p.S + 32 * NW - 1) / (32 * NW);
     hipLaunchKernelGGL((attn_dkdv2s_kernel<NW, true, 3, NSUB, VAR>), dim3(p.B * p.NH * nb), dim3(64 * NW), NSUB * attnb::LDS_DKV, s, p);
 }
-void launch_dkdv_v2(const BwdParams& p, hipStream_t s) {
+void launch_dkdv_v2(const SegBwdParams& p, hipStream_t s) {
     if (g_attn_variant) launch_dkdv_var<1>(p, s);
     else launch_dkdv_var<0>(p, s);
 }
diff --git a/ttt-video-dit_amd/csrc/capi.hip b/ttt-video-dit_amd/csrc/capi.hip
--- a/ttt-video-dit_amd/csrc/capi.hip
+++ b/ttt-video-dit_amd/csrc/capi.hip
@@ -370,7 +370,8 @@
     if (!q_raw || !k_raw || !wq || !bq || !wk || !bk || !q || !k) return fail("ttt_hip: attn_pre_forward: null pointer");
     if (n_text < S && (!cos_table || !sin_table)) return fail("ttt_hip: attn_pre_forward: null rope table");
     ttt::attn::PreParams p = {(const __bf16*)q_raw, (const __bf16*)k_raw, wq, bq, wk, bk, cos_table, sin_table,
-                              (__bf16*)q, (__bf16*)k, B, S, NH, n_text, eps};
+                              (__bf16*)q, (__bf16*)k, B, S, NH, n_text, eps,
+                              0, 0, (long)S * NH * 64, (long)NH * 64, 0};
     ttt::attn::launch_pre_forward(p, (hipStream_t)stream);
     return post_launch("attn_pre_forward");
 }
@@ -398,9 +399,145 @@
     p.dk_sb = dk->stride_b; p.dk_sh = dk->stride_h; p.dk_ss = dk->stride_s;
     p.wq = wq; p.wk = wk; p.cos = cos_table; p.sin = sin_table;
     p.dq_raw = (__bf16*)dq_raw; p.dk_raw = (__bf16*)dk_raw; p.part = part; p.ld_out = (long)ld_out;
+    p.in_sb = (long)S * NH * 64; p.in_ss = (long)NH * 64; p.out_sb = (long)S * ld_out;
     p.B = B; p.S = S; p.NH = NH; p.n_text = n_text; p.eps = eps;
     ttt::attn::launch_pre_backward(p, (hipStream_t)stream);
     return post_launch("attn_pre_backward");
+}
+
+
+static int check_attn_rows(const ttt_attn_rows& t, const char* name) {
+    if (!t.ptr1 || (t.n_split > 0 && !t.ptr0)) return fail("ttt_hip: attention: null row view %s", name);
+    if (t.n_split < 0) return fail("ttt_hip: attention: negative n_split in %s", name);
+    if (((uintptr_t)t.ptr1 & 15) || ((uintptr_t)t.ptr0 & 15) || (t.stride_b & 7) || (t.stride_h & 7) || (t.stride_s & 7))
+        return fail("ttt_hip: attention: row view %s must be 16-byte aligned with strides that are multiples of 8 elements", name);
+    return 0;
+}
+static __bf16* rows_hi(const ttt_attn_rows& t) { return (__bf16*)t.ptr1 - (long)t.n_split * t.stride_s; }
+static long rows_dlo(const ttt_attn_rows& t) { return t.n_split > 0 ? (long)(((intptr_t)t.ptr0 - (intptr_t)rows_hi(t)) / 2) : 0; }
+static long elem_off(const void* p, const void* base) { return (long)(((intptr_t)p - (intptr_t)base) / 2); }
+static int seg_sides(ttt::attn::SegExt& x, const void* O, const ttt_attn_tensor (&side)[2], const int32_t (&lo)[2], const int32_t (&hi)[2], int S) {
+    for (int i = 0; i < 2; ++i) {
+        if (lo[i] < 0 || hi[i] < lo[i] || hi[i] > S) return fail("ttt_hip: attention: bad side range");
+        if (hi[i] > lo[i] && check_attn_tensor(side[i], "O_side")) return -1;
+    }
+    if (hi[0] > lo[0] && hi[1] > lo[1] && (side[0].stride_b != side[1].stride_b || side[0].stride_h != side[1].stride_h || side[0].stride_s != side[1].stride_s))
+        return fail("ttt_hip: attention: the two side buffers must share their strides");
+    const ttt_attn_tensor& ref = hi[0] > lo[0] ? side[0] : side[1];
+    x.os_sb = ref.stride_b; x.os_sh = ref.stride_h; x.os_ss = ref.stride_s;
+    x.os0_d = hi[0] > lo[0] ? elem_off(side[0].ptr, O) - (long)lo[0] * x.os_ss : 0;
+    x.os1_d = hi[1] > lo[1] ? elem_off(side[1].ptr, O) - (long)lo[1] * x.os_ss : 0;
+    x.s0_lo = lo[0]; x.s0_hi = hi[0]; x.s1_lo = lo[1]; x.s1_hi = hi[1];
+    return 0;
+}
+
+int ttt_hip_attn_forward_seg(const ttt_attn_seg_fwd_args* a, void* stream) {
+    if (!a) return fail("ttt_hip: null args");
+    if (a->D != 64) return fail("ttt_hip: attention: head_dim must be 64");
+    if (a->B <= 0 || a->NH <= 0 || a->S <= 0) return fail("ttt_hip: attention: non-positive dimension");
+    if (check_attn_tensor(a->Q, "Q") || check_attn_tensor(a->K, "K") || check_attn_rows(a->V, "V") || check_attn_rows(a->O, "O")) return -1;
+    if (a->V.n_split != a->O.n_split || a->V.n_split > a->S) return fail("ttt_hip: attention: V and O must split at the same row <= S");
+    ttt::attn::SegFwdParams p = {};
+    p.Q = (const __bf16*)a->Q.ptr; p.K = (const __bf16*)a->K.ptr; p.V = rows_hi(a->V); p.O = rows_hi(a->O);
+    p.LSE = a->LSE;
+    p.q_sb = a->Q.stride_b; p.q_sh = a->Q.stride_h; p.q_ss = a->Q.stride_s;
+    p.k_sb = a->K.stride_b; p.k_sh = a->K.stride_h; p.k_ss = a->K.stride_s;
+    p.v_sb = a->V.stride_b; p.v_sh = a->V.stride_h; p.v_ss = a->V.stride_s;
+    p.o_sb = a->O.stride_b; p.o_sh = a->O.stride_h; p.o_ss = a->O.stride_s;
+    p.B = a->B; p.NH = a->NH; p.S = a->S; p.scale = a->scale;
+    p.x.n_split = a->V.n_split; p.x.v_dlo = rows_dlo(a->V); p.x.o_dlo = rows_dlo(a->O);
+    if (seg_sides(p.x, p.O, a->O_side, a->side_lo, a->side_hi, a->S)) return -1;
+    ttt::attn::launch_forward_seg(p, (hipStream_t)stream);
+    return post_launch("attn_forward_seg");
+}
+
+int ttt_hip_attn_backward_seg(const ttt_attn_seg_bwd_args* a, void* stream) {
+    if (!a) return fail("ttt_hip: null args");
+    if (a->D != 64) return fail("ttt_hip: attention: head_dim must be 64");
+    if (a->B <= 0 || a->NH <= 0 || a->S <= 0) return fail("ttt_hip: attention: non-positive dimension");
+    if (!a->LSE || !a->Delta) return fail("ttt_hip: attention backward: null LSE / Delta");
+    if (check_attn_tensor(a->Q, "Q") || check_attn_tensor(a->K, "K") || check_attn_rows(a->V, "V") || check_attn_rows(a->O, "O") ||
+        check_attn_rows(a->dO, "dO") || check_attn_tensor(a->dQ, "dQ") || check_attn_tensor(a->dK, "dK") || check_attn_rows(a->dV, "dV")) return -1;
+    const int ns = a->V.n_split;
+    if (a->O.n_split != ns || a->dO.n_split != ns || a->dV.n_split != ns || ns > a->S) return fail("ttt_hip: attention: V, O, dO and dV must split at the same row <= S");
+    if (a->acc_lo < 0 || a->acc_hi < a->acc_lo || a->acc_hi > a->S) return fail("ttt_hip: attention: bad accumulate range");
+    for (int i = 0; i < 2; ++i)
+        if (a->half_lo[i] < 0 || a->half_hi[i] < a->half_lo[i] || a->half_hi[i] > a->S) return fail("ttt_hip: attention: bad dO range");
+    ttt::attn::SegBwdParams p = {};
+    p.Q = (const __bf16*)a->Q.ptr; p.K = (const __bf16*)a->K.ptr; p.V = rows_hi(a->V); p.O = rows_hi(a->O);
+    p.dO = rows_hi(a->dO); p.dQ = (__bf16*)a->dQ.ptr; p.dK = (__bf16*)a->dK.ptr; p.dV = rows_hi(a->dV);
+    p.LSE = a->LSE; p.Delta = a->Delta;
+    p.q_sb = a->Q.stride_b; p.q_sh = a->Q.stride_h; p.q_ss = a->Q.stride_s;
+    p.k_sb = a->K.stride_b; p.k_sh = a->K.stride_h; p.k_ss = a->K.stride_s;
+    p.v_sb = a->V.stride_b; p.v_sh = a->V.stride_h; p.v_ss = a->V.stride_s;
+    p.o_sb = a->O.stride_b; p.o_sh = a->O.stride_h; p.o_ss = a->O.stride_s;
+    p.do_sb = a->dO.stride_b; p.do_sh = a->dO.stride_h; p.do_ss = a->dO.stride_s;
+    p.dq_sb = a->dQ.stride_b; p.dq_sh = a->dQ.stride_h; p.dq_ss = a->dQ.stride_s;
+    p.dk_sb = a->dK.stride_b; p.dk_sh = a->dK.stride_h; p.dk_ss = a->dK.stride_s;
+    p.dv_sb = a->dV.stride_b; p.dv_sh = a->dV.stride_h; p.dv_ss = a->dV.stride_s;
+    p.B = a->B; p.NH = a->NH; p.S = a->S; p.scale = a->scale;
+    p.x.n_split = ns; p.x.v_dlo = rows_dlo(a->V); p.x.o_dlo = rows_dlo(a->O); p.x.do_dlo = rows_dlo(a->dO); p.x.dv_dlo = rows_dlo(a->dV);
+    if (seg_sides(p.x, p.O, a->O_side, a->side_lo, a->side_hi, a->S)) return -1;
+    p.x.h0_lo = a->half_lo[0]; p.x.h0_hi = a->half_hi[0]; p.x.h1_lo = a->half_lo[1]; p.x.h1_hi = a->half_hi[1];
+    p.x.acc_lo = a->acc_lo; p.x.acc_hi = a->acc_hi;
+    ttt::attn::launch_backward_seg(p, (hipStream_t)stream);
+    return post_launch("attn_backward_seg");
+}
+
+int ttt_hip_attn_average(int B, int n, int d, const void* a, const void* b, int64_t ab_stride_b, int64_t ab_stride_s,
+                         void* out, int64_t out_stride_b, int64_t out_stride_s, void* stream) {
+    if (B <= 0 || n <= 0 || d <= 0 || (d & 7)) return fail("ttt_hip: attn_average: bad dimension (d must be a multiple of 8)");
+    if (!a || !b || !out) return fail("ttt_hip: attn_average: null pointer");
+    if (((uintptr_t)a & 15) || ((uintptr_t)b & 15) || ((uintptr_t)out & 15) || ((ab_stride_b | ab_stride_s | out_stride_b | out_stride_s) & 7))
+        return fail("ttt_hip: attn_average: tensors must be 16-byte aligned with strides that are multiples of 8 elements");
+    ttt::attn::AvgParams p = {(const __bf16*)a, (const __bf16*)b, (__bf16*)out, (long)ab_stride_b, (long)ab_stride_s, (long)out_stride_b, (long)out_stride_s, B, n, d};
+    ttt::attn::launch_average(p, (hipStream_t)stream);
+    return post_launch("attn_average");
+}
+
+static int check_pre_rows(const ttt_attn_rows* q, const ttt_attn_rows* k, int S, int NH, const char* what) {
+    if (!q || !k) return fail("ttt_hip: attn_pre: null row view");
+    if (check_attn_rows(*q, what) || check_attn_rows(*k, what)) return -1;
+    if (q->stride_h != 64 || k->stride_h != 64 || q->stride_b != k->stride_b || q->stride_s != k->stride_s || q->n_split != k->n_split ||
+        q->n_split > S || q->stride_s < (int64_t)NH * 64)
+        return fail("ttt_hip: attn_pre: the q / k row views must share n_split <= S and strides, with heads 64 elements apart and rows >= NH*64");
+    return 0;
+}
+int ttt_hip_attn_pre_forward_seg(int B, int S, int NH, int n_text, float eps, const ttt_attn_rows* q_raw, const ttt_attn_rows* k_raw,
+                                 const float* wq, const float* bq, const float* wk, const float* bk,
+                                 const float* cos_table, const float* sin_table, void* q, void* k, void* stream) {
+    if (B <= 0 || S <= 0 || NH <= 0 || n_text < 0) return fail("ttt_hip: attn_pre: bad dimension");
+    if (!wq || !bq || !wk || !bk || !q || !k) return fail("ttt_hip: attn_pre_forward: null pointer");
+    if (n_text < S && (!cos_table || !sin_table)) return fail("ttt_hip: attn_pre_forward: null rope table");
+    if (check_pre_rows(q_raw, k_raw, S, NH, "q_raw / k_raw")) return -1;
+    ttt::attn::PreParams p = {rows_hi(*q_raw), rows_hi(*k_raw), wq, bq, wk, bk, cos_table, sin_table, (__bf16*)q, (__bf16*)k, B, S, NH, n_text, eps,
+                              rows_dlo(*q_raw), rows_dlo(*k_raw), (long)q_raw->stride_b, (long)q_raw->stride_s, q_raw->n_split};
+    ttt::attn::launch_pre_forward(p, (hipStream_t)stream);
+    return post_launch("attn_pre_forward_seg");
+}
+int ttt_hip_attn_pre_backward_seg(int B, int S, int NH, int n_text, float eps, const ttt_attn_rows* q_raw, const ttt_attn_rows* k_raw,
+                                  const ttt_attn_tensor* dq, const ttt_attn_tensor* dk, const float* wq, const float* wk,
+                                  const float* cos_table, const float* sin_table, const ttt_attn_rows* dq_raw, const ttt_attn_rows* dk_raw,
+                                  int acc_lo, int acc_hi, float* part, void* stream) {
+    if (B <= 0 || S <= 0 || NH <= 0 || n_text < 0) return fail("ttt_hip: attn_pre: bad dimension");
+    if (!dq || !dk || !wq || !wk || !part) return fail("ttt_hip: attn_pre_backward: null pointer");
+    if (n_text < S && (!cos_table || !sin_table)) return fail("ttt_hip: attn_pre_backward: null rope table");
+    if (check_attn_tensor(*dq, "dq") || check_attn_tensor(*dk, "dk")) return -1;
+    if (check_pre_rows(q_raw, k_raw, S, NH, "q_raw / k_raw") || check_pre_rows(dq_raw, dk_raw, S, NH, "dq_raw / dk_raw")) return -1;
+    if (dq_raw->n_split != q_raw->n_split) return fail("ttt_hip: attn_pre_backward: the raw projections and their gradients must split at the same row");
+    if (acc_lo < 0 || acc_hi < acc_lo || acc_hi > S) return fail("ttt_hip: attn_pre_backward: bad accumulate range");
+    ttt::attn::PreBwdParams p = {};
+    p.q_raw = rows_hi(*q_raw); p.k_raw = rows_hi(*k_raw); p.q_dlo = rows_dlo(*q_raw); p.k_dlo = rows_dlo(*k_raw);
+    p.in_sb = (long)q_raw->stride_b; p.in_ss = (long)q_raw->stride_s; p.n_split = q_raw->n_split;
+    p.dq = (const __bf16*)dq->ptr; p.dk = (const __bf16*)dk->ptr;
+    p.dq_sb = dq->stride_b; p.dq_sh = dq->stride_h; p.dq_ss = dq->stride_s;
+    p.dk_sb = dk->stride_b; p.dk_sh = dk->stride_h; p.dk_ss = dk->stride_s;
+    p.wq = wq; p.wk = wk; p.cos = cos_table; p.sin = sin_table;
+    p.dq_raw = rows_hi(*dq_raw); p.dk_raw = rows_hi(*dk_raw); p.dq_raw_dlo = rows_dlo(*dq_raw); p.dk_raw_dlo = rows_dlo(*dk_raw);
+    p.ld_out = (long)dq_raw->stride_s; p.out_sb = (long)dq_raw->stride_b; p.acc_lo = acc_lo; p.acc_hi = acc_hi;
+    p.part = part; p.B = B; p.S = S; p.NH = NH; p.n_text = n_text; p.eps = eps;
+    ttt::attn::launch_pre_backward(p, (hipStream_t)stream);
+    return post_launch("attn_pre_backward_seg");
 }
 
 
diff --git a/ttt-video-dit_amd/test_time_training/__init__.py b/ttt-video-dit_amd/test_time_training/__init__.py
--- a/ttt-video-dit_amd/test_time_training/__init__.py
+++ b/ttt-video-dit_amd/test_time_training/__init__.py
@@ -56,6 +56,7 @@
     "ttt_hip_post_forward", "ttt_hip_post_backward", "ttt_hip_gate_forward", "ttt_hip_gate_backward_partials",
     "ttt_hip_gate_backward", "ttt_hip_attn_forward", "ttt_hip_attn_backward",
     "ttt_hip_attn_pre_forward", "ttt_hip_attn_pre_partials", "ttt_hip_attn_pre_backward", "ttt_hip_attn_pre_backward_ld",
+    "ttt_hip_attn_forward_seg", "ttt_hip_attn_backward_seg", "ttt_hip_attn_average", "ttt_hip_attn_pre_forward_seg", "ttt_hip_attn_pre_backward_seg",
     "ttt_hip_adaln_forward", "ttt_hip_adaln_backward_partials", "ttt_hip_adaln_backward",
     "ttt_hip_resgate_forward", "ttt_hip_resgate_backward_partials", "ttt_hip_resgate_backward",
 )
@@ -601,6 +602,139 @@
           device=q_raw.device)
 
 
+class _AttnRows(ctypes.Structure):
+    _fields_ = [("ptr0", ctypes.c_void_p), ("ptr1", ctypes.c_void_p), ("stride_b", ctypes.c_int64), ("stride_h", ctypes.c_int64),
+                ("stride_s", ctypes.c_int64), ("n_split", ctypes.c_int32), ("reserved", ctypes.c_int32)]
+
+
+class _AttnSegFwd(ctypes.Structure):
+    _fields_ = [("Q", _AttnTensor), ("K", _AttnTensor), ("V", _AttnRows), ("O", _AttnRows), ("O_side", _AttnTensor * 2),
+                ("side_lo", ctypes.c_int32 * 2), ("side_hi", ctypes.c_int32 * 2), ("LSE", ctypes.c_void_p),
+                ("B", ctypes.c_int32), ("NH", ctypes.c_int32), ("S", ctypes.c_int32), ("D", ctypes.c_int32), ("scale", ctypes.c_float)]
+
+
+class _AttnSegBwd(ctypes.Structure):
+    _fields_ = [("Q", _AttnTensor), ("K", _AttnTensor), ("V", _AttnRows), ("O", _AttnRows), ("dO", _AttnRows), ("O_side", _AttnTensor * 2),
+                ("side_lo", ctypes.c_int32 * 2), ("side_hi", ctypes.c_int32 * 2), ("half_lo", ctypes.c_int32 * 2), ("half_hi", ctypes.c_int32 * 2),
+                ("dQ", _AttnTensor), ("dK", _AttnTensor), ("dV", _AttnRows), ("acc_lo", ctypes.c_int32), ("acc_hi", ctypes.c_int32),
+                ("LSE", ctypes.c_void_p), ("Delta", ctypes.c_void_p),
+                ("B", ctypes.c_int32), ("NH", ctypes.c_int32), ("S", ctypes.c_int32), ("D", ctypes.c_int32), ("scale", ctypes.c_float)]
+
+
+class SegmentRows:
+
+    def __init__(self, t0, n_split, v0, S, side=((0, 0), (0, 0))):
+        self.t0, self.n_split, self.v0, self.S, self.side = int(t0), int(n_split), int(v0), int(S), tuple((int(a), int(b)) for a, b in side)
+
+
+def _attn_rows(t, name, seg, B, NH):
+    if not isinstance(t, torch.Tensor) or not t.is_cuda or t.dtype != torch.bfloat16 or t.dim() != 3:
+        raise RuntimeError(f"{name}: expected a bfloat16 [B, L, NH*64] tensor on a HIP device (there is no CPU path)")
+    L = t.shape[1]
+    if t.shape[0] != B or t.shape[2] != NH * 64 or t.stride(2) != 1:
+        raise RuntimeError(f"{name}: expected shape ({B}, L, {NH * 64}) with a contiguous last dimension, got {tuple(t.shape)}")
+    nv = seg.S - seg.n_split
+    if min(seg.t0, seg.v0, seg.n_split, nv) < 0 or seg.t0 + seg.n_split > L or seg.v0 + nv > L:
+        raise RuntimeError(f"{name}: the segment's rows lie outside the sequence of {L} tokens")
+    es = t.element_size()
+    return _AttnRows(t.data_ptr() + seg.t0 * t.stride(1) * es, t.data_ptr() + seg.v0 * t.stride(1) * es, t.stride(0), 64, t.stride(1),
+                     seg.n_split, 0)
+
+
+def _attn_sides(sides, seg, B, NH):
+    arr, lo, hi = (_AttnTensor * 2)(), (ctypes.c_int32 * 2)(), (ctypes.c_int32 * 2)()
+    for i, (a, b) in enumerate(seg.side):
+        lo[i], hi[i] = a, b
+        if b > a:
+            t = sides[i]
+            if not isinstance(t, torch.Tensor) or not t.is_cuda or t.dtype != torch.bfloat16 or tuple(t.shape) != (B, b - a, NH * 64) or not t.is_contiguous():
+                raise RuntimeError(f"side buffer {i}: expected a contiguous bfloat16 {(B, b - a, NH * 64)} tensor on a HIP device")
+            if not (0 <= a and b <= seg.S):
+                raise RuntimeError("side range outside the segment")
+            arr[i] = _AttnTensor(t.data_ptr(), t.stride(0), 64, t.stride(1))
+    return arr, lo, hi
+
+
+def attn_forward_seg(q, k, v, out, sides, lse, scale, seg):
+    B, NH, S, D = q.shape
+    if S != seg.S:
+        raise RuntimeError("attn_forward_seg: q has a different number of rows than the segment")
+    arr, lo, hi = _attn_sides(sides, seg, B, NH)
+    if lse is not None:
+        _req(lse, "lse", torch.float32)
+        if tuple(lse.shape) != (B, NH, S):
+            raise RuntimeError("lse: expected [B, NH, S]")
+    a = _AttnSegFwd(_attn_tensor(q, "q", (B, NH, S, D)), _attn_tensor(k, "k", (B, NH, S, D)), _attn_rows(v, "v", seg, B, NH),
+                    _attn_rows(out, "out", seg, B, NH), arr, lo, hi, lse.data_ptr() if lse is not None else None, B, NH, S, D, float(scale))
+    _call("ttt_hip_attn_forward_seg", ctypes.byref(a), device=q.device)
+
+
+def attn_backward_seg(q, k, v, out, sides, dout, lse, delta, dq, dk, dv, scale, seg, acc=(0, 0)):
+    B, NH, S, D = q.shape
+    sh = (B, NH, S, D)
+    if S != seg.S:
+        raise RuntimeError("attn_backward_seg: q has a different number of rows than the segment")
+    _req(lse, "lse", torch.float32); _req(delta, "delta", torch.float32)
+    if tuple(lse.shape) != (B, NH, S) or tuple(delta.shape) != (B, NH, S):
+        raise RuntimeError("lse / delta: expected [B, NH, S]")
+    arr, lo, hi = _attn_sides(sides, seg, B, NH)
+    if not (0 <= acc[0] <= acc[1] <= S):
+        raise RuntimeError("attn_backward_seg: bad accumulate range")
+    a = _AttnSegBwd(_attn_tensor(q, "q", sh), _attn_tensor(k, "k", sh), _attn_rows(v, "v", seg, B, NH), _attn_rows(out, "out", seg, B, NH),
+                    _attn_rows(dout, "dout", seg, B, NH), arr, lo, hi, lo, hi, _attn_tensor(dq, "dq", sh), _attn_tensor(dk, "dk", sh),
+                    _attn_rows(dv, "dv", seg, B, NH), int(acc[0]), int(acc[1]), lse.data_ptr(), delta.data_ptr(), B, NH, S, D, float(scale))
+    _call("ttt_hip_attn_backward_seg", ctypes.byref(a), device=q.device)
+
+
+def attn_average(a, b, out):
+    B, n, d = a.shape
+    for t, nm in ((a, "a"), (b, "b")):
+        _req(t, nm, torch.bfloat16)
+    if tuple(b.shape) != (B, n, d) or not isinstance(out, torch.Tensor) or not out.is_cuda or out.dtype != torch.bfloat16 \
+            or tuple(out.shape) != (B, n, d) or out.stride(2) != 1:
+        raise RuntimeError("attn_average: a, b, out must be bf16 [B, n, d] tensors on a HIP device (out: rows of any stride)")
+    _call("ttt_hip_attn_average", B, n, d, _p(a), _p(b), ctypes.c_int64(a.stride(0)), ctypes.c_int64(a.stride(1)), _p(out),
+          ctypes.c_int64(out.stride(0)), ctypes.c_int64(out.stride(1)), device=a.device)
+
+
+def _pre_seg_common(q, k, NH, seg):
+    B, S, D = q.shape
+    if S != seg.S or D != NH * 64:
+        raise RuntimeError("attn_pre_*_seg: q / k must be [B, S, NH*64] with the segment's S")
+    return B, S
+
+
+def attn_pre_forward_seg(q_raw, k_raw, wq, bq, wk, bk, cos, sin, q, k, NH, n_text, eps, seg):
+    B, S = _pre_seg_common(q, k, NH, seg)
+    for t, n in ((q, "q"), (k, "k")):
+        _req(t, n, torch.bfloat16)
+    for t, n in ((wq, "wq"), (bq, "bq"), (wk, "wk"), (bk, "bk"), (cos, "cos"), (sin, "sin")):
+        _req(t, n, torch.float32)
+    if cos.shape[-1] != 64 or cos.shape[0] < S - n_text or tuple(k.shape) != tuple(q.shape):
+        raise RuntimeError("attn_pre_forward_seg: head_dim must be 64 and the rope tables must cover the video tokens")
+    rq, rk = _attn_rows(q_raw, "q_raw", seg, B, NH), _attn_rows(k_raw, "k_raw", seg, B, NH)
+    _call("ttt_hip_attn_pre_forward_seg", B, S, NH, int(n_text), ctypes.c_float(eps), ctypes.byref(rq), ctypes.byref(rk), _p(wq), _p(bq), _p(wk),
+          _p(bk), _p(cos), _p(sin), _p(q), _p(k), device=q.device)
+
+
+def attn_pre_backward_seg(q_raw, k_raw, dq, dk, wq, wk, cos, sin, dq_raw, dk_raw, part, NH, n_text, eps, seg, acc=(0, 0)):
+    B, NH_, S, _ = dq.shape
+    if S != seg.S or NH_ != NH:
+        raise RuntimeError("attn_pre_backward_seg: dq must be [B, NH, S, 64] with the segment's S")
+    for t, n in ((wq, "wq"), (wk, "wk"), (cos, "cos"), (sin, "sin"), (part, "part")):
+        _req(t, n, torch.float32)
+    if cos.shape[-1] != 64 or cos.shape[0] < S - n_text or part.shape[0] < attn_pre_partials(B, S, NH):
+        raise RuntimeError("attn_pre_backward_seg: rope tables / partial buffer too small")
+    if not (0 <= acc[0] <= acc[1] <= S):
+        raise RuntimeError("attn_pre_backward_seg: bad accumulate range")
+    rq, rk = _attn_rows(q_raw, "q_raw", seg, B, NH), _attn_rows(k_raw, "k_raw", seg, B, NH)
+    gq, gk = _attn_rows(dq_raw, "dq_raw", seg, B, NH), _attn_rows(dk_raw, "dk_raw", seg, B, NH)
+    tq, tk = _attn_tensor(dq, "dq", (B, NH, S, 64)), _attn_tensor(dk, "dk", (B, NH, S, 64))
+    _call("ttt_hip_attn_pre_backward_seg", B, S, NH, int(n_text), ctypes.c_float(eps), ctypes.byref(rq), ctypes.byref(rk), ctypes.byref(tq),
+          ctypes.byref(tk), _p(wq), _p(wk), _p(cos), _p(sin), ctypes.byref(gq), ctypes.byref(gk), int(acc[0]), int(acc[1]), _p(part),
+          device=dq.device)
+
+
 def adaln_forward(vid, text, w, b, shift, scale1p, out, eps):
     B, Lv, D = vid.shape
     Lt = text.shape[1]
diff --git a/ttt-video-dit_amd/ttt_amd/models/cogvideo/attention.py b/ttt-video-dit_amd/ttt_amd/models/cogvideo/attention.py
--- a/ttt-video-dit_amd/ttt_amd/models/cogvideo/attention.py
+++ b/ttt-video-dit_amd/ttt_amd/models/cogvideo/attention.py
@@ -138,3 +138,87 @@
         ext.attn_pre_backward(qr, kr, dq, dk, wq32, wk32, cos, sin, dq_raw, dk_raw, part, NH, n_text, eps, ld_out=dq_raw.stride(1))
         g = part.sum(0).to(pdt)
         return dq_raw, dk_raw, dv, g[0], g[1], g[2], g[3], None, None, None, None, None
+
+
+def sequence_segments(n_text, tl, rng, shared):
+    ext = _ext()
+    n = len(rng)
+    segs = []
+    for i, (lo, hi) in enumerate(rng):
+        S = tl + hi - lo
+        side = ((tl, tl + shared) if i > 0 else (0, 0), (S - shared, S) if i + 1 < n else (0, 0))
+        segs.append(ext.SegmentRows(i * tl, tl, n_text + lo, S, side))
+    return segs
+
+
+class FullSequenceAttention(torch.autograd.Function):
+
+    @staticmethod
+    def forward(ctx, q_raw, k_raw, v, wq, bq, wk, bk, cos, sin, NH, n_text, tl, rng, shared, eps):
+        ext = _ext()
+        B, L, D = q_raw.shape
+        Dh = D // NH
+        row = lambda t: t if t.stride(2) == 1 else t.contiguous()
+        q_raw, k_raw, v = row(q_raw), row(k_raw), row(v)
+        f32 = lambda t: t.detach().to(torch.float32).contiguous()
+        p32 = (f32(wq), f32(bq), f32(wk), f32(bk))
+        scale = 1.0 / math.sqrt(Dh)
+        segs = sequence_segments(n_text, tl, rng, shared)
+        heads = lambda t: t.view(B, t.shape[1], NH, Dh).transpose(1, 2)
+
+        def run():
+            out = torch.empty(B, L, D, device=v.device, dtype=v.dtype)
+            sides = torch.empty(max(len(segs) - 1, 1), 2, B, shared, D, device=v.device, dtype=v.dtype)
+            lses = []
+            for i, seg in enumerate(segs):
+                q = torch.empty(B, seg.S, D, device=v.device, dtype=v.dtype)
+                k = torch.empty_like(q)
+                ext.attn_pre_forward_seg(q_raw, k_raw, *p32, cos, sin, q, k, NH, tl, float(eps), seg)
+                lse = torch.empty(B, NH, seg.S, device=v.device, dtype=torch.float32)
+                ext.attn_forward_seg(heads(q), heads(k), v, out, _sides(sides, i, len(segs)), lse, scale, seg)
+                lses.append(lse)
+            for j in range(len(segs) - 1):
+                lo = n_text + rng[j + 1][0]
+                ext.attn_average(sides[j, 0], sides[j, 1], out[:, lo:lo + shared])
+            return (out, sides, *lses)
+
+        out, sides, *lses = kernel_result("attn", run)
+        ctx.save_for_backward(q_raw, k_raw, v, out, sides, *lses, *p32, cos, sin)
+        ctx.meta = (NH, n_text, tl, tuple(rng), shared, float(eps), scale, wq.dtype)
+        return out
+
+    @staticmethod
+    def backward(ctx, dout):
+        ext = _ext()
+        NH, n_text, tl, rng, shared, eps, scale, pdt = ctx.meta
+        n = len(rng)
+        saved = ctx.saved_tensors
+        q_raw, k_raw, v, out, sides = saved[:5]
+        lses = saved[5:5 + n]
+        wq32, bq32, wk32, bk32, cos, sin = saved[5 + n:]
+        B, L, D = q_raw.shape
+        Dh = D // NH
+        if dout.stride(2) != 1 or dout.data_ptr() % 16 or dout.stride(1) % 8 or dout.stride(0) % 8:
+            dout = dout.contiguous()
+        segs = sequence_segments(n_text, tl, rng, shared)
+        heads = lambda t: t.view(B, t.shape[1], NH, Dh).transpose(1, 2)
+        from ttt_amd.models.ssm.fused import qkv_grad_blocks
+        dq_raw, dk_raw, dv = qkv_grad_blocks(q_raw)
+        P = max(ext.attn_pre_partials(B, seg.S, NH) for seg in segs)
+        part = torch.zeros(n, P, 4, 64, device=v.device, dtype=torch.float32)
+        for i, seg in enumerate(segs):
+            q = torch.empty(B, seg.S, D, device=v.device, dtype=v.dtype)
+            k = torch.empty_like(q)
+            ext.attn_pre_forward_seg(q_raw, k_raw, wq32, bq32, wk32, bk32, cos, sin, q, k, NH, tl, eps, seg)
+            dq, dk = heads(torch.empty_like(q)), heads(torch.empty_like(q))
+            delta = torch.empty(B, NH, seg.S, device=v.device, dtype=torch.float32)
+            acc = seg.side[0]
+            ext.attn_backward_seg(heads(q), heads(k), v, out, _sides(sides, i, n), dout, lses[i], delta, dq, dk, dv, scale, seg, acc)
+            del q, k
+            ext.attn_pre_backward_seg(q_raw, k_raw, dq, dk, wq32, wk32, cos, sin, dq_raw, dk_raw, part[i], NH, tl, eps, seg, acc)
+        g = part.sum((0, 1)).to(pdt)
+        return (dq_raw, dk_raw, dv, g[0], g[1], g[2], g[3]) + (None,) * 8
+
+
+def _sides(sides, i, n):
+    return (sides[i - 1, 1] if i > 0 else None, sides[i, 0] if i + 1 < n else None)
diff --git a/ttt-video-dit_amd/ttt_amd/models/cogvideo/dit.py b/ttt-video-dit_amd/ttt_amd/models/cogvideo/dit.py
--- a/ttt-video-dit_amd/ttt_amd/models/cogvideo/dit.py
+++ b/ttt-video-dit_amd/ttt_amd/models/cogvideo/dit.py
@@ -1,6 +1,7 @@
 from __future__ import annotations
 
 import contextlib
+import os
 
 import torch
 import torch.nn.functional as F
@@ -8,8 +9,9 @@
 from torch.utils.checkpoint import checkpoint
 
 from ttt_amd.infra import remat_cache
-from ttt_amd.infra.fused_linear import linear3
-from ttt_amd.models.cogvideo.attention import FusedSegmentAttention, attn_pre_available, segment_attention
+from ttt_amd.infra.fused_linear import linear3, linear3_applies
+from ttt_amd.models.cogvideo.attention import (FullSequenceAttention, FusedSegmentAttention, attn_pre_available,
+                                               segment_attention)
 from ttt_amd.models.cogvideo.utils import (Rotary3DPositionEmbedding, SequenceMetadata, modulate,
                                            timestep_embedding, unpatchify)
 from ttt_amd.models.configs import ModelConfig
@@ -173,6 +175,7 @@
         self.head_dim = config.model_dim // config.num_heads
         self.prefix_temporal_length = config.prefix_temporal_length
         self.attn_length = config.attn_length
+        self.full_sequence_attention = os.environ.get("TTT_FULLSEQ_ATTENTION", "1") != "0"
 
         self.q_norm = nn.LayerNorm(self.head_dim, eps=config.layer_norm_eps).requires_grad_(train)
         self.k_norm = nn.LayerNorm(self.head_dim, eps=config.layer_norm_eps).requires_grad_(train)
@@ -214,6 +217,12 @@
         x = cat if cat is not None else torch.cat((text_emb, vid_emb), dim=1)
         n_text = text_emb.shape[1]
         tl, rng, shared = _segment_geometry(seq_metadata, vid_emb.shape[1], self.attn_length, self.prefix_temporal_length)
+        if self.full_sequence_attention and attn_pre_available(x, self.head_dim) and linear3_applies(self.q, self.k, self.v, x):
+            cos, sin = self.rotary.tables_f32()
+            q, k, v = linear3(self.q, self.k, self.v, x)
+            a = FullSequenceAttention.apply(q, k, v, self.q_norm.weight, self.q_norm.bias, self.k_norm.weight, self.k_norm.bias, cos, sin,
+                                            self.num_heads, n_text, tl, tuple(rng), shared, self.q_norm.eps)
+            return self.o(a)
         segs = SegmentSplit.apply(x, n_text, tl, rng, shared)
         return SegmentMerge.apply(n_text, tl, rng, shared, *(self._segment(seg, tl) for seg in segs))
 
```

Result: no change. 8605 (median of 4 runs) (+0.0%).
